# rwth-i6/rasr

Measured on AMD Instinct MI355X. Metric: acoustic frames scored/sec (1e4-state AM), higher is better.
Workload: dtype f16+mxfp6 (per f32 product: one f16 MFMA product + one block-scaled fp6 x fp6 MFMA product for both cross terms, f32 accumulate)

## Files before the change

rasr_amd/csrc/common.hpp:

```cpp
#pragma once
#include <hip/hip_runtime.h>

#include <cstdarg>
#include <cstdio>
#include <map>
#include <memory>
#include <string>
#include <vector>

#include "../../include/amx.h"

namespace amx {

void set_error(const char* fmt, ...);

#define AMX_HIP(expr)                                                                          \
    do {                                                                                       \
        hipError_t e__ = (expr);                                                               \
        if (e__ != hipSuccess) {                                                               \
            amx::set_error("%s failed: %s (%s:%d)", #expr, hipGetErrorString(e__), __FILE__, __LINE__); \
            return AMX_ERR_DEVICE;                                                             \
        }                                                                                      \
    } while (0)

// ... 92 lines not shown
    const char* name;
    hipEvent_t  a = nullptr, b = nullptr;
    ScopedKernelTimer(amx_ctx* c, const char* n)
            : ctx(c), name(n) {
        if (ctx->profiling) {
            hipEventCreate(&a);
            hipEventCreate(&b);
            hipEventRecord(a, ctx->stream);
        }
    }
    ~ScopedKernelTimer() {
        if (a) {
            hipEventRecord(b, ctx->stream);
            ctx->prof[name].events.emplace_back(a, b);
        }
    }
};

template<class Key>
struct GraphCache {
    enum Ran { kPlain, kRecorded, kReplayed };
    std::map<Key, hipGraphExec_t> graphs;
    int                           use_graphs = 0;
    GraphCache() = default;
    GraphCache(const GraphCache&)            = delete;
    GraphCache& operator=(const GraphCache&) = delete;
    ~GraphCache() { clear(); }
    void clear() {
        for (auto& kv : graphs)
            if (kv.second)
                hipGraphExecDestroy(kv.second);
        graphs.clear();
    }
    template<class Pass>
    int run(const Key& key, hipStream_t stream, Pass&& pass, Ran* ran) {
        *ran    = kPlain;
        auto it = graphs.find(key);
        if (it == graphs.end()) {
            if (graphs.size() >= 64) {
                clear();
                use_graphs = 0;
            }
            else
                graphs[key] = nullptr;
            return pass(false);
        }
        hipGraphExec_t ex = it->second;
        if (ex)
            *ran = kReplayed;
        else {
            hipGraph_t g = nullptr;
            if (hipStreamBeginCapture(stream, hipStreamCaptureModeThreadLocal) != hipSuccess) {
                (void)hipGetLastError();
                use_graphs = 0;
                return pass(false);
            }
            const int  r  = pass(true);
            const bool ok = hipStreamEndCapture(stream, &g) == hipSuccess && r == AMX_OK && g != nullptr;
            if (!ok || hipGraphInstantiate(&ex, g, nullptr, nullptr, 0) != hipSuccess) {
                (void)hipGetLastError();
                if (g)
                    hipGraphDestroy(g);
                use_graphs = 0;
                return pass(false);
            }
            hipGraphDestroy(g);
            graphs[key] = ex;
            *ran        = kRecorded;
        }
        AMX_HIP(hipGraphLaunch(ex, stream));
        return AMX_OK;
    }
};

struct Tuning {
    std::map<std::string, std::string> kv;
    bool parse(const char* s, const char* const* allowed, const char* who);
    bool has(const char* key) const { return kv.count(key) != 0; }
    bool get_int(const char* key, int dflt, long lo, long hi, int* out, const char* who) const;
    bool get_word(const char* key, const char* dflt, const char* const* words, std::string* out, const char* who) const;
};

static const char* const gmm_tuning_keys[] = {"screen", "fused", "screen_all", "screen_kernel", "graph", "tied_prune", "chunk", "fused_waves", "fr",
                                              "simd_mfma", "contract", "dist_list", "near_fused", "fused_pack", nullptr};

template<bool FMA>
__host__ __device__ __forceinline__ float mad(float a, float b, float c) {
    return FMA ? __builtin_fmaf(a, b, c) : a * b + c;
}
template<bool FMA>
__host__ __device__ __forceinline__ double mad(double a, double b, double c) {
    return FMA ? __builtin_fma(a, b, c) : a * b + c;
}

template<class V>
__device__ __forceinline__ void nt_store(V v, V* p) {
#ifdef AMX_PLAIN_STORES
    *p = v;
#else
    __builtin_nontemporal_store(v, p);
#endif
}

inline bool views_alias(const float* in, int in_ld, int in_w, const float* out, int out_ld, int out_w, long long T) {
    if (T <= 0)
        return false;
    const float* in_end  = in + (T - 1) * (long long)in_ld + in_w;
    const float* out_end = out + (T - 1) * (long long)out_ld + out_w;
    if (in_end <= out || out_end <= in)
        return false;
    if (in_ld == out_ld) {
        const long long ld = in_ld, delta = out - in;
        const long long c  = ((delta % ld) + ld) % ld;
        if (c >= in_w && c + out_w <= ld)
            return false;
    }
    return true;
}

inline int ceil_div(long a, long b) {
    return (int)((a + b - 1) / b);
}

}
```

rasr_amd/csrc/ffnn.hip:

```cpp
#include "common.hpp"
#include "gmm_internal.hpp"
#include "ffnn_f32.hpp"

#include <hip/hip_bf16.h>

#include <algorithm>
#include <map>
#include <tuple>
#include <type_traits>
#include <cmath>
#include <cstring>

namespace amx {

typedef __attribute__((ext_vector_type(8))) short bf16x8;
typedef unsigned short                              bf16_t;

typedef float  f32x2 __attribute__((ext_vector_type(2)));
typedef float  f32x4 __attribute__((ext_vector_type(4)));
typedef __bf16 bf16x2 __attribute__((ext_vector_type(2)));

__device__ __forceinline__ unsigned pack_bf16(float lo, float hi) {
    f32x2 v = {lo, hi};
    return __builtin_bit_cast(unsigned, __builtin_convertvector(v, bf16x2));
// ... 1086 lines not shown
            const unsigned i = s_idx[w][lane];
            if (m < bmin || (m == bmin && i < bidx)) {
                bmin = m;
                bidx = i;
            }
        }
        if (best_state)
            best_state[t] = bidx;
        if (bidx != 0xffffffffu)
            sum = (double)bmin;
        my = bidx;
    }
    {
        unsigned long long todo = __ballot(my != 0xffffffffu);
        while (todo) {
            const int      leader = __ffsll((long long)todo) - 1;
            const unsigned key    = (unsigned)__shfl((int)my, leader, 64);
            const unsigned long long same = __ballot(my == key) & todo;
            if (lane == leader)
                atomicAdd(&counts[key], (unsigned long long)__popcll(same));
            todo &= ~same;
        }
    }
#pragma unroll
    for (int off = 32; off > 0; off >>= 1)
        sum += __shfl_xor(sum, off, 64);
    if (lane == 0 && sum != 0.0)
        atomicAdd(score_sum, sum);
}

}


struct OverflowWord {
    unsigned *host = nullptr, *dev = nullptr;
    OverflowWord()                               = default;
    OverflowWord(const OverflowWord&)            = delete;
    OverflowWord& operator=(const OverflowWord&) = delete;
    ~OverflowWord() {
        if (host)
            hipHostFree(host);
    }
    int create() {
        if (hipHostMalloc((void**)&host, 4, hipHostMallocMapped) != hipSuccess || hipHostGetDevicePointer((void**)&dev, host, 0) != hipSuccess) {
            (void)hipGetLastError();
            amx::set_error("amx_ffnn_create: cannot allocate the overflow flag");
            return AMX_ERR_DEVICE;
        }
        *host = 0;
        return AMX_OK;
    }
};

struct amx_ffnn {
    amx_ctx*           ctx = nullptr;
    int                n_layers = 0, precision = AMX_PREC_BF16;
    std::vector<int>   in, out, act, Kpad, Npad;
    std::vector<amx::DevBuf<unsigned char>> d_W;
    std::vector<amx::DevBuf<float>> d_bias;
    amx::DevBuf<unsigned char> d_in, d_act[2];
    std::vector<float> h_Wout, h_bout;
    bool   class_mapped = false;
    amx::DevBuf<float> d_rowstat;
    amx::DevBuf<float> d_Wout, d_bout;
    int    max_hidden_pad = 0;
    int    largest_layer  = 0;
    int    group_t = -1, group_n = -1;
    amx::DevBuf<float>    d_part_min;
    amx::DevBuf<unsigned> d_part_idx;
    struct GraphKey {
        const void *feats, *scores, *best, *counts, *sum;
        hipStream_t stream;
        int         stride, T, stats;
        bool operator<(const GraphKey& o) const {
            return std::tie(feats, scores, best, counts, sum, stream, stride, T, stats) <
                   std::tie(o.feats, o.scores, o.best, o.counts, o.sum, o.stream, o.stride, o.T, o.stats);
        }
    };
    amx::GraphCache<GraphKey> graphs;
    amx::DevBuf<float> d_host_f, d_host_s;
    int    gemm_persistent = 1;
    int    gemm_cfg       = -1;
    int    chunk          = 32768;
    int    mx_stagger     = 0;
    int    mx_dbg         = 0;
    int    mx_ksplit      = 1;
    amx::DevBuf<float> d_ks_ws;
    OverflowWord overflow;
    amx::PreOps         pre{};
    std::vector<amx::DevBuf<float>> d_pre;
    std::vector<int>    mo_groups;
    std::vector<amx::DevBuf<int>> d_mo_off, d_mo_size;
    int    mo_width = 0;
    amx::DevBuf<float> d_mo;
    size_t elt() const { return precision == AMX_PREC_FP32 ? 4 : 2; }
    bool   mfma_bf16() const { return precision != AMX_PREC_FP32; }
    bool   is_mx() const { return precision == AMX_PREC_F16MX; }
    int    requested_precision = 0;
    double mx_block_ratio      = 0.0;
#ifdef AMX_LAB
    int    overflowed() const { return mx_dbg == 0 && overflow.host && *(volatile unsigned*)overflow.host; }
#else
    int    overflowed() const { return overflow.host && *(volatile unsigned*)overflow.host; }
#endif
};

namespace {

int pad_to(int v, int m) {
    return (v + m - 1) / m * m;
}

int operand_stride(const amx_ffnn* h, int width) {
    return h->is_mx() ? width / 32 : (h->precision == AMX_PREC_BF16X3 ? 2 : 1) * width;
}

size_t operand_bytes(const amx_ffnn* h, int Tpad, int width) {
    const size_t stride = (size_t)operand_stride(h, width);
    return h->is_mx() ? (size_t)(Tpad / 256) * stride * amx::mx::BLK : (size_t)Tpad * stride * h->elt();
}

template<class T>
int grow(amx_ffnn* h, amx::DevBuf<T>& buf, size_t n) {
    if (n <= buf.capacity())
        return AMX_OK;
    h->graphs.clear();
    return buf.reserve(n);
}

int ensure_workspace(amx_ffnn* h, int Tpad) {
    if (h->mo_width > 0)
        AMX_TRY(grow(h, h->d_mo, (size_t)Tpad * h->mo_width));
    AMX_TRY(grow(h, h->d_in, operand_bytes(h, Tpad, h->Kpad[0])));
    if (h->max_hidden_pad > 0) {
        AMX_TRY(grow(h, h->d_act[0], operand_bytes(h, Tpad, h->max_hidden_pad)));
        AMX_TRY(grow(h, h->d_act[1], operand_bytes(h, Tpad, h->max_hidden_pad)));
    }
    return AMX_OK;
}

void size_split_k_workspace(amx_ffnn* h) {
    if (!h->is_mx() || h->mx_ksplit <= 1)
        return;
    const long ncu  = std::max(h->ctx->n_cu, 8);
    size_t     need = 0;
    for (int Tpad = amx::PAD_NT;; Tpad += amx::PAD_NT) {
        bool fits = false;
        for (int l = 0; l < h->n_layers; ++l) {
            const long tiles = (long)(h->Npad[l] / 128) * (Tpad / 64);
            if (tiles * h->mx_ksplit > ncu)
                continue;
            fits = true;
            if (h->Kpad[l] / 32 >= 8 * h->mx_ksplit)
                need = std::max(need, (size_t)tiles * h->mx_ksplit * 4 * 2 * 16 * 64);
        }
        if (!fits)
            break;
    }
    if (need != 0 && h->d_ks_ws.reserve(need) != AMX_OK) {
        (void)hipGetLastError();
        h->mx_ksplit = 1;
    }
}

struct ArgminPart {
    float*    min = nullptr;
// ... 205 lines not shown
        AMX_MX_LAUNCH(2048);
    }
    else if (dbg == 128 && C::PIPE == 1 && ACT == AMX_ACT_RELU * (LAST ? 0 : 1)) {
        if constexpr (C::PIPE == 1)
            AMX_MX_LAUNCH(128);
    }
    else
        dbg = 0;
#endif
    if (dbg == 0)
        AMX_MX_LAUNCH(0);
#undef AMX_MX_LAUNCH
    return ntn;
}

template<int ACT, bool LAST>
int launch_mx_cfg(amx_ffnn* h, int l, const void* x, int xkts, void* out, int ldo, int T, int Tpad, int n_valid, ArgminPart part) {
    int cfg = h->gemm_cfg;
    if (cfg < 0) {
        const long ncu = std::max(h->ctx->n_cu, 1), t256 = (long)(h->Npad[l] / 256) * (Tpad / 256), t128 = (long)(h->Npad[l] / 128) * (Tpad / 128);
        const long t64 = (long)(h->Npad[l] / 128) * (Tpad / 64);
        if (t256 >= 2L * ncu)
            cfg = 8;
        else if (LAST && t256 <= ncu && 5 * t256 >= 3 * ncu)
            cfg = 8;
        else if (t128 >= ncu)
            cfg = 0;
        else if (t64 > ncu && t64 <= 2 * ncu)
            cfg = 6;
        else if (!LAST && 2 * t64 <= ncu && h->mx_ksplit <= 1)
            cfg = 14;
        else
            cfg = 3;
    }
    switch (cfg) {
        case 2: return launch_mx<MfgL, ACT, LAST>(h, l, x, xkts, out, ldo, T, Tpad, n_valid, part);
        case 4: return launch_mx<MfgLP, ACT, LAST>(h, l, x, xkts, out, ldo, T, Tpad, n_valid, part);
        case 5: return launch_mx<MfgLH, ACT, LAST>(h, l, x, xkts, out, ldo, T, Tpad, n_valid, part);
        case 7: return launch_mx<MfgLF, ACT, LAST>(h, l, x, xkts, out, ldo, T, Tpad, n_valid, part);
        case 8: return launch_mx<MfgLQ, ACT, LAST>(h, l, x, xkts, out, ldo, T, Tpad, n_valid, part);
        case 9: return launch_mx<MfgLW, ACT, LAST>(h, l, x, xkts, out, ldo, T, Tpad, n_valid, part);
        case 3:
            if constexpr (LAST)
                return launch_mx<MfgS, ACT, LAST>(h, l, x, xkts, out, ldo, T, Tpad, n_valid, part);
            else
                return launch_mx<MfgSP, ACT, LAST>(h, l, x, xkts, out, ldo, T, Tpad, n_valid, part);
        case 6: return launch_mx<MfgS4, ACT, LAST>(h, l, x, xkts, out, ldo, T, Tpad, n_valid, part);
        case 12: return launch_mx<MfgS8, ACT, LAST>(h, l, x, xkts, out, ldo, T, Tpad, n_valid, part);
        case 14:
            if constexpr (LAST)
                return launch_mx<MfgS, ACT, LAST>(h, l, x, xkts, out, ldo, T, Tpad, n_valid, part);
            else
                return launch_mx<Mfg64, ACT, LAST>(h, l, x, xkts, out, ldo, T, Tpad, n_valid, part);
case 11:
            if constexpr (LAST)
                return launch_mx<MfgS, ACT, LAST>(h, l, x, xkts, out, ldo, T, Tpad, n_valid, part);
            else
                return launch_mx<MfgSL, ACT, LAST>(h, l, x, xkts, out, ldo, T, Tpad, n_valid, part);
        default: return launch_mx<MfgA, ACT, LAST>(h, l, x, xkts, out, ldo, T, Tpad, n_valid, part);
    }
}

template<bool NONE_ONLY = false, class F>
void with_act(int act, F&& f) {
    using std::integral_constant;
    if constexpr (NONE_ONLY)
        f(integral_constant<int, AMX_ACT_NONE>());
    else
        switch (act) {
            case AMX_ACT_RELU: f(integral_constant<int, AMX_ACT_RELU>()); break;
            case AMX_ACT_SIGMOID: f(integral_constant<int, AMX_ACT_SIGMOID>()); break;
            case AMX_ACT_TANH: f(integral_constant<int, AMX_ACT_TANH>()); break;
            case AMX_ACT_ELU: f(integral_constant<int, AMX_ACT_ELU>()); break;
            default: f(integral_constant<int, AMX_ACT_NONE>()); break;
        }
}

template<class S>
void pack_operand(amx_ffnn* h, const S& src, int T, int K, void* out, int Kp, int Tpad) {
    hipStream_t st     = h->ctx->stream;
    const int   blocks = (int)std::min<long long>(4096, ((long long)Tpad * Kp + 255) / 256);
    if (h->is_mx()) {
        const int b2 = (int)std::min<long long>(8192, ((long long)Tpad * (Kp / 32) * 2 + 255) / 256);
        hipLaunchKernelGGL(amx::mx::pack_input_mx<S>, dim3(b2), dim3(256), 0, st, src, T, K, (char*)out, Kp / 32, Tpad, h->overflow.dev);
    }
    else if (h->precision == AMX_PREC_BF16X3)
        hipLaunchKernelGGL(amx::pack_input_bf16x3<S>, dim3(blocks), dim3(256), 0, st, src, T, K, (amx::bf16_t*)out, Kp, Tpad);
    else if (h->precision == AMX_PREC_BF16)
        hipLaunchKernelGGL(amx::pack_input_bf16<S>, dim3(blocks), dim3(256), 0, st, src, T, K, (amx::bf16_t*)out, Kp, Tpad);
    else
        hipLaunchKernelGGL(amx::pack_input_f32<S>, dim3(blocks), dim3(256), 0, st, src, T, K, (float*)out, Kp, Tpad);
}

template<bool LAST>
int launch_layer(amx_ffnn* h, int l, const void* x, int ldx, void* out, int ldo, int T, int Tpad, ArgminPart part = {}, int* ntn = nullptr) {
    hipStream_t            st = h->ctx->stream;
    amx::ScopedKernelTimer t_all(h->ctx, "ffnn_gemm");
    hipEvent_t             e0 = nullptr, e1 = nullptr;
    const bool             time_max = h->ctx->profiling && l == h->largest_layer;
    if (time_max) {
        hipEventCreate(&e0);
        hipEventCreate(&e1);
        hipEventRecord(e0, st);
    }
    const int act = LAST ? AMX_ACT_NONE : h->act[l];
    int       tiles = 0;
    if (h->is_mx()) {
        with_act<LAST>(act, [&](auto a) { tiles = launch_mx_cfg<decltype(a)::value, LAST>(h, l, x, ldx, out, ldo, T, Tpad, h->out[l], part); });
    }
    else if (h->mfma_bf16()) {
        with_act<LAST>(act, [&](auto a) { tiles = launch_bf16_cfg<decltype(a)::value, LAST>(h, l, x, ldx, out, ldo, T, Tpad, part); });
    }
    else {
        const int ntn = h->Npad[l] / amx::BN, ntt = Tpad / amx::BT;
        dim3      grid(ntn * ntt), block(256);
        const int nv = h->out[l];
        with_act<LAST>(act, [&](auto a) {
            hipLaunchKernelGGL((amx::gemm_f32_kernel<decltype(a)::value, LAST>), grid, block, 0, st, (const float*)h->d_W[l].get(), (const float*)x,
                               h->d_bias[l].get(), (float*)out, h->Kpad[l], ldx, ldo, nv, T, ntn);
        });
    }
    if (time_max) {
        hipEventRecord(e1, st);
        h->ctx->prof["ffnn_gemm_max"].events.emplace_back(e0, e1);
    }
    AMX_HIP(hipGetLastError());
    if (ntn)
        *ntn = tiles;
    return AMX_OK;
}

int launch_maxout_layer(amx_ffnn* h, int l, const void* x, int ldx, void* dst, int Kp, int T, int Trows, int Tpad, bool export_f32) {
    AMX_TRY(launch_layer<true>(h, l, x, ldx, h->d_mo.get(), h->out[l], T, Tpad));
    const int G = h->mo_groups[l];
    amx::ScopedKernelTimer timer(h->ctx, "ffnn_maxout");
    with_act(h->act[l], [&](auto a) {
        const amx::MaxoutSrc<decltype(a)::value> src{h->d_mo.get(), h->out[l], h->d_mo_off[l].get(), h->d_mo_size[l].get()};
        if (export_f32) {
            const int blocks = (int)std::min<long long>(4096, ((long long)Trows * Kp + 255) / 256);
            hipLaunchKernelGGL(amx::pack_input_f32<decltype(src)>, dim3(blocks), dim3(256), 0, h->ctx->stream, src, T, G, (float*)dst, Kp, Trows);
        }
        else
            pack_operand(h, src, T, G, dst, Kp, Trows);
    });
    AMX_HIP(hipGetLastError());
    return AMX_OK;
}


struct MaxoutSpec {
    std::vector<int>              groups;
    std::vector<std::vector<int>> size;
};

int check_extension(const amx_ffnn_model* m, const amx_ffnn_layers* ext, MaxoutSpec* mo) {
    const int n_pre = ext ? ext->n_pre : 0;
    mo->groups.assign((size_t)m->n_layers, 0);
    mo->size.assign((size_t)m->n_layers, {});
    AMX_REQUIRE(n_pre >= 0 && n_pre <= AMX_NN_MAX_PRE, AMX_ERR_INVALID, "amx_ffnn_create_ex: %d preprocessing layers (0 to %d)", n_pre,
                AMX_NN_MAX_PRE);
    AMX_REQUIRE(n_pre == 0 || ext->pre_type, AMX_ERR_INVALID, "amx_ffnn_create_ex: %d preprocessing layers without pre_type", n_pre);
    for (int i = 0; i < n_pre; ++i) {
        const int ty = ext->pre_type[i];
        AMX_REQUIRE(ty == AMX_NN_PRE_LOGARITHM || ty == AMX_NN_PRE_MEAN_AND_VARIANCE, AMX_ERR_INVALID,
                    "amx_ffnn_create_ex: preprocessing layer %d: unknown type %d", i, ty);
        if (ty == AMX_NN_PRE_MEAN_AND_VARIANCE) {
            AMX_REQUIRE(ext->pre_mean && ext->pre_mean[i], AMX_ERR_INVALID,
// ... 20 lines not shown
                }
                AMX_REQUIRE(sum == m->out_dim[l], AMX_ERR_INVALID,
                            "amx_ffnn_create_ex: layer %d: maxout group sizes add up to %ld, the layer has %d outputs "
                            "(require_eq(getInputDimension(0), inputsize_))", l, sum, m->out_dim[l]);
                v.assign(sz, sz + G);
            }
            else {
                AMX_REQUIRE(m->out_dim[l] % G == 0, AMX_ERR_INVALID,
                            "amx_ffnn_create_ex: layer %d: %d outputs do not split into %d maxout groups of one size "
                            "(require_eq(getInputDimension(0), maxoutSize_ * getOutputDimension()))", l, m->out_dim[l], G);
                v.assign((size_t)G, m->out_dim[l] / G);
            }
            mo->groups[l] = G;
        }
    return AMX_OK;
}

int check_model(const amx_ffnn_model* m, const std::vector<int>& mo_groups) {
    for (int l = 0; l < m->n_layers; ++l) {
        AMX_REQUIRE(m->in_dim[l] > 0 && m->out_dim[l] > 0 && m->W[l], AMX_ERR_INVALID, "amx_ffnn_create: layer %d is empty", l);
        if (l > 0 && mo_groups[l - 1] > 0)
            AMX_REQUIRE(m->in_dim[l] == mo_groups[l - 1], AMX_ERR_INVALID,
                        "amx_ffnn_create_ex: layer %d input dimension %d != %d outputs of the maxout behind layer %d", l, m->in_dim[l],
                        mo_groups[l - 1], l - 1);
        else if (l > 0)
            AMX_REQUIRE(m->in_dim[l] == m->out_dim[l - 1], AMX_ERR_INVALID,
                        "amx_ffnn_create: layer %d input dimension %d != previous output %d", l, m->in_dim[l], m->out_dim[l - 1]);
        AMX_REQUIRE(m->activation[l] >= AMX_ACT_NONE && m->activation[l] <= AMX_ACT_ELU, AMX_ERR_INVALID,
                    "amx_ffnn_create: unknown activation in layer %d", l);
    }
    AMX_REQUIRE(m->activation[m->n_layers - 1] == AMX_ACT_NONE, AMX_ERR_INVALID, "amx_ffnn_create: output layer must be linear (softmax is not evaluated)");
    return AMX_OK;
}

struct LayerParams {
    std::vector<int>          out_dim;
    std::vector<const float*> W, bias;
    const float*              prior = nullptr;
    std::vector<float>        Wmap, bmap, pmap;
};

int remap_classes(const amx_ffnn_model* m, LayerParams* p) {
    const int L0 = m->n_layers - 1;
    p->out_dim.assign(m->out_dim, m->out_dim + m->n_layers);
    p->W.assign(m->W, m->W + m->n_layers);
    p->bias.assign(m->bias, m->bias + m->n_layers);
    p->prior = m->log_prior;
    if (!m->class_to_output)
        return AMX_OK;
    AMX_REQUIRE(m->n_classes > 0, AMX_ERR_INVALID, "amx_ffnn_create: class_to_output without n_classes");
    const int N = m->out_dim[L0], K = m->in_dim[L0];
    std::vector<char> used((size_t)N, 0);
    int               n_targets = 0;
    for (int e = 0; e < m->n_classes; ++e) {
        const int o = m->class_to_output[e];
        AMX_REQUIRE(o >= -1 && o < N, AMX_ERR_INVALID, "amx_ffnn_create: class %d maps to output %d (network has %d outputs)", e, o, N);
        if (o >= 0) {
            AMX_REQUIRE(!used[o], AMX_ERR_INVALID, "amx_ffnn_create: no one-to-one correspondence between network outputs and classes (output %d)", o);
            used[o] = 1;
            ++n_targets;
        }
    }
    AMX_REQUIRE(n_targets == N, AMX_ERR_INVALID, "amx_ffnn_create: %d classes to accumulate, but the output layer has %d units", n_targets, N);
    p->Wmap.assign((size_t)m->n_classes * K, 0.f);
    p->bmap.assign((size_t)m->n_classes, -3.402823466e+38f);
    p->pmap.assign((size_t)m->n_classes, 0.f);
    for (int e = 0; e < m->n_classes; ++e) {
        const int o = m->class_to_output[e];
        if (o < 0)
            continue;
        memcpy(&p->Wmap[(size_t)e * K], m->W[L0] + (size_t)o * K, (size_t)K * 4);
        p->bmap[e] = m->bias[L0] ? m->bias[L0][o] : 0.f;
        p->pmap[e] = m->log_prior ? m->log_prior[o] : 0.f;
    }
    p->out_dim[L0] = m->n_classes;
    p->W[L0]       = p->Wmap.data();
    p->bias[L0]    = p->bmap.data();
    if (m->log_prior)
        p->prior = p->pmap.data();
    return AMX_OK;
}

int parse_tuning(const amx_ffnn_model* m, amx_ffnn* h, bool* mx_fallback_auto) {
    static const char* const keys[]      = {"tile", "graph", "persistent", "group", "chunk", "stagger", "mx_dbg", "mx_fallback", "ksplit", nullptr};
    static const char* const fallbacks[] = {"auto", "off", nullptr};
    const char*              who         = "amx_ffnn_create";
    amx::Tuning              tune;
    std::string              fallback;
    if (!tune.parse(m->tuning, keys, who) || !tune.get_word("mx_fallback", "auto", fallbacks, &fallback, who) ||
        !tune.get_int("ksplit", 1, 1, 4, &h->mx_ksplit, who))
        return AMX_ERR_INVALID;
    *mx_fallback_auto = fallback == "auto";
    AMX_REQUIRE(h->mx_ksplit == 1 || h->mx_ksplit == 4, AMX_ERR_INVALID, "amx_ffnn_create: tuning ksplit=%d: expected 1 | 4", h->mx_ksplit);
    AMX_REQUIRE(h->mx_ksplit == 1 || m->precision == AMX_PREC_F16MX, AMX_ERR_UNSUPPORTED, "amx_ffnn_create: tuning ksplit exists for AMX_PREC_F16MX only");
    if (!tune.get_int("tile", -1, -1, 14, &h->gemm_cfg, who) || !tune.get_int("graph", 0, 0, 1, &h->graphs.use_graphs, who) ||
        !tune.get_int("persistent", 1, 0, 1, &h->gemm_persistent, who) || !tune.get_int("chunk", 32768, 256, 1 << 24, &h->chunk, who) ||
        !tune.get_int("mx_dbg", 0, 0, 1 << 16, &h->mx_dbg, who) || !tune.get_int("stagger", 0, 0, 100000, &h->mx_stagger, who))
        return AMX_ERR_INVALID;
    if (tune.has("group")) {
        const std::string g    = tune.kv["group"];
        char              tail = 0;
        AMX_REQUIRE(sscanf(g.c_str(), "%dx%d%c", &h->group_t, &h->group_n, &tail) == 2 && h->group_t >= 1 && h->group_n >= 1 && h->group_t <= 4096 &&
                            h->group_n <= 4096,
                    AMX_ERR_INVALID, "amx_ffnn_create: tuning group=%s: expected <frame tiles>x<output tiles>, e.g. 16x8", g.c_str());
    }
    return AMX_OK;
}

double block_max_ratio(const float* W, int N, int K) {
    double sum_max2 = 0.0, sum_w2 = 0.0;
    long   n_blocks = 0;
    for (int n = 0; n < N; ++n)
        for (int k0 = 0; k0 < K; k0 += 32) {
            float mx = 0.f;
            for (int k = k0; k < std::min(K, k0 + 32); ++k) {
                const float v = W[(size_t)n * K + k];
                mx            = std::fmax(mx, std::fabs(v));
                sum_w2 += (double)v * (double)v;
            }
            sum_max2 += (double)mx * (double)mx;
            ++n_blocks;
        }
    return sum_w2 > 0.0 ? std::sqrt((sum_max2 / (double)n_blocks) / (sum_w2 / ((double)N * (double)K))) : 0.0;
}

int choose_precision(const amx_ffnn_model* m, const LayerParams& p, bool mx_fallback_auto, amx_ffnn* h) {
    h->precision = h->requested_precision = m->precision;
    if (m->precision != AMX_PREC_F16MX)
        return AMX_OK;
    for (int l = 0; l < m->n_layers; ++l)
        h->mx_block_ratio = std::max(h->mx_block_ratio, block_max_ratio(p.W[l], p.out_dim[l], m->in_dim[l]));
    if (mx_fallback_auto && h->mx_block_ratio > 4.0) {
        AMX_REQUIRE(h->mx_ksplit <= 1, AMX_ERR_INVALID,
                    "amx_ffnn_create: tuning ksplit=%d applies to AMX_PREC_F16MX, but this network's weights are heavy-tailed (block-maximum "
                    "statistic %.2f > 4.0) and the handle would compute in AMX_PREC_BF16X3: drop ksplit, or keep f16mx with mx_fallback=off",
                    h->mx_ksplit, h->mx_block_ratio);
        std::fprintf(stderr, "rasr_amd: amx_ffnn_create: AMX_PREC_F16MX requested, computing in AMX_PREC_BF16X3 (block-maximum statistic of the "
                             "weights %.2f > 4.0; tuning mx_fallback=off keeps f16mx)\n", h->mx_block_ratio);
        h->precision = AMX_PREC_BF16X3;
    }
    return AMX_OK;
}

void set_shapes(amx_ffnn* h, const amx_ffnn_model* m, const LayerParams& p, const MaxoutSpec& mo) {
    const int kmult = h->is_mx() ? amx::mx::TK : h->mfma_bf16() ? amx::BK : amx::FK;
    long      best_flops = -1;
    h->n_layers  = m->n_layers;
    h->mo_groups = mo.groups;
    for (int l = 0; l < m->n_layers; ++l) {
        h->in.push_back(m->in_dim[l]);
        h->out.push_back(p.out_dim[l]);
        h->act.push_back(m->activation[l]);
        if (mo.groups[l] > 0)
            h->mo_width = std::max(h->mo_width, p.out_dim[l]);
        h->Kpad.push_back(pad_to(m->in_dim[l], kmult));
        h->Npad.push_back(pad_to(p.out_dim[l], amx::PAD_NT));
        if (l + 1 < m->n_layers)
            h->max_hidden_pad = std::max(h->max_hidden_pad, h->Npad[l]);
        long fl = (long)m->in_dim[l] * p.out_dim[l];
        if (fl > best_flops) {
            best_flops       = fl;
            h->largest_layer = l;
        }
    }
}

std::vector<unsigned char> pack_weights(int precision, const float* W, int N, int K, int Np, int Kp) {
    std::vector<unsigned char> pk;
    if (precision == AMX_PREC_F16MX) {
        amx::mx::pack_weights_host(W, N, K, K, Np, Kp / 32, pk);
        return pk;
    }
    if (precision == AMX_PREC_FP32) {
        pk.assign((size_t)Np * Kp * 4, 0);
        for (int n = 0; n < N; ++n)
            memcpy(&pk[(size_t)n * Kp * 4], W + (size_t)n * K, (size_t)K * 4);
        return pk;
    }
    const bool   x3 = precision == AMX_PREC_BF16X3;
    const size_t ld = x3 ? 2 * (size_t)Kp : (size_t)Kp;
// ... 422 lines not shown
```

rasr_amd/csrc/ffnn_f32.hpp:

```cpp
#pragma once
#include "common.hpp"

#include <cmath>

namespace amx {

typedef __attribute__((ext_vector_type(16))) float f32x16;

template<int ACT>
__device__ __forceinline__ float activate(float v) {
    if (ACT == AMX_ACT_RELU)
        return v < 0.f ? 0.f : v;
    if (ACT == AMX_ACT_SIGMOID)
        return 1.f / (1.f + expf(-v));
    if (ACT == AMX_ACT_TANH)
        return tanhf(v);
    if (ACT == AMX_ACT_ELU)
        return v < 0.f ? expf(v) - 1.f : v;
    return v;
}

struct PreOps {
    int          n;
    int          type[AMX_NN_MAX_PRE];
    const float* mean[AMX_NN_MAX_PRE];
    const float* rstd[AMX_NN_MAX_PRE];
};

struct RawSrc {
    const float* x;
    int          ldx;
    __device__ __forceinline__ float operator()(int t, int k) const { return x[(size_t)t * ldx + k]; }
};

struct FeatSrc {
    const float* x;
    int          ldx;
    PreOps       pre;
    __device__ __forceinline__ float operator()(int t, int k) const {
        float v = x[(size_t)t * ldx + k];
#pragma unroll
        for (int i = 0; i < AMX_NN_MAX_PRE; ++i) {
            if (i >= pre.n)
                break;
            if (pre.type[i] == AMX_NN_PRE_LOGARITHM)
                v = (float)log((double)v);
            else {
                v = v - pre.mean[i][k];
                v = v * pre.rstd[i][k];
            }
        }
        return v;
    }
};

static __global__ __launch_bounds__(256) void top_negexp_kernel(float* __restrict__ x, int n, float* __restrict__ g_max) {
    __shared__ float s_red[4];
    float*           row = x + (size_t)blockIdx.x * n;
    float            mx  = -__builtin_inff();
    for (int i = threadIdx.x; i < n; i += 256)
        mx = fmaxf(mx, -row[i]);
#pragma unroll
    for (int off = 32; off > 0; off >>= 1)
        mx = fmaxf(mx, __shfl_xor(mx, off, 64));
    if ((threadIdx.x & 63) == 0)
        s_red[threadIdx.x >> 6] = mx;
    __syncthreads();
    mx = fmaxf(fmaxf(s_red[0], s_red[1]), fmaxf(s_red[2], s_red[3]));
    const float value = -1.f * mx;
    for (int i = threadIdx.x; i < n; i += 256) {
        const float a = -row[i];
        row[i]        = (float)exp((double)(a + value));
    }
    if (threadIdx.x == 0)
        g_max[blockIdx.x] = mx;
}

static __global__ __launch_bounds__(64) void top_rowsum_kernel(const float* __restrict__ x, int T, int n, float* __restrict__ g_sum) {
    __shared__ float s_tile[64][65];
    const int        lane = threadIdx.x, t0 = blockIdx.x * 64;
    float            acc = 0.f;
    for (int c0 = 0; c0 < n; c0 += 64) {
        const int w = min(64, n - c0);
        for (int r = 0; r < 64; ++r)
            s_tile[r][lane] = (t0 + r < T && lane < w) ? x[(size_t)(t0 + r) * n + c0 + lane] : 0.f;
        __syncthreads();
        for (int c = 0; c < w; ++c)
            acc = acc + s_tile[lane][c];
        __syncthreads();
    }
    if (t0 + lane < T)
        g_sum[t0 + lane] = acc;
}

static __global__ __launch_bounds__(256) void top_finish_kernel(float* __restrict__ x, long long total, int n, const float* __restrict__ g_sum) {
    for (long long i = (long long)blockIdx.x * 256 + threadIdx.x; i < total; i += (long long)gridDim.x * 256) {
        if (g_sum) {
            const float r = 1.f / g_sum[i / n];
            x[i]          = x[i] * r;
        }
        else
            x[i] = -x[i];
    }
}

template<class S>
__global__ __launch_bounds__(256) void pack_input_f32(S src, int T, int K, float* __restrict__ out, int Kpad, int Tpad) {
    const long long n = (long long)Tpad * Kpad;
    for (long long i = (long long)blockIdx.x * 256 + threadIdx.x; i < n; i += (long long)gridDim.x * 256) {
        int t = (int)(i / Kpad), k = (int)(i - (long long)t * Kpad);
        out[i] = (t < T && k < K) ? src(t, k) : 0.f;
    }
}

constexpr int BN = 128, BT = 128;
constexpr int FK  = 32;
constexpr int FLD = FK + 1;

template<int ACT, bool LAST>
__global__ __launch_bounds__(256) void gemm_f32_kernel(const float* __restrict__ W, const float* __restrict__ X,
                                                      const float* __restrict__ bias, float* __restrict__ out, int Kpad, int ldx, int ldo,
                                                      int n_valid, int t_valid, int n_tiles_n) {
    __shared__ float sW[BN * FLD];
    __shared__ float sX[BT * FLD];
    const int tid = threadIdx.x, lane = tid & 63, wave = tid >> 6;
    const int wn = wave >> 1, wt = wave & 1;
    const int tile_t = blockIdx.x / n_tiles_n, tile_n = blockIdx.x - tile_t * n_tiles_n;
    const int n0 = tile_n * BN, t0 = tile_t * BT;

    f32x16 acc[2][2];
#pragma unroll
    for (int i = 0; i < 2; ++i)
#pragma unroll
        for (int j = 0; j < 2; ++j)
#pragma unroll
            for (int r = 0; r < 16; ++r)
// ... 57 lines not shown
```

rasr_amd/csrc/ffnn_mx.hpp:

```cpp
#pragma once

namespace amx {
namespace mx {

typedef _Float16 f16x8 __attribute__((ext_vector_type(8)));
typedef unsigned u32x4 __attribute__((ext_vector_type(4)));
typedef unsigned u32x2 __attribute__((ext_vector_type(2)));
typedef _Float16 f16x2 __attribute__((ext_vector_type(2)));
typedef _Float16 f16x16 __attribute__((ext_vector_type(16)));
typedef _Float16 f16x32 __attribute__((ext_vector_type(32)));
typedef float    f32v16 __attribute__((ext_vector_type(16)));
typedef unsigned u32x6 __attribute__((ext_vector_type(6)));
typedef int      v8i __attribute__((ext_vector_type(8)));

constexpr int TK    = 32;
constexpr int R_OFF = 16384;
constexpr int BLK   = 24576;

__host__ __device__ constexpr int pos16(int u) {
    return 8 * (2 * (u >> 4) + ((u >> 2) & 1)) + 4 * ((u >> 3) & 1) + (u & 3);
}
__host__ __device__ inline int h_off(int r, int c) {
    return r * 64 + ((c ^ ((r >> 2) & 3)) << 4);
}
// ... 28 lines not shown
            code = (unsigned)(qv / 0.125);
    }
    return code | (std::signbit(v) ? 32u : 0u);
}

static inline void pack_weights_host(const float* W, int n_rows, int K, int ld, int Rpad, int KT, std::vector<unsigned char>& out) {
    out.assign((size_t)(Rpad / 256) * KT * BLK, 0);
    auto block_max = [&](int n, int kt) {
        float m = 0.f;
        if (n < n_rows)
            for (int u = 0; u < 32; ++u) {
                const int k = kt * 32 + u;
                if (k < K)
                    m = std::fmax(m, std::fabs(W[(size_t)n * ld + k]));
            }
        return m;
    };
    for (int n = 0; n < n_rows; ++n) {
        const int rb = n >> 8, r = n & 255;
        for (int kt = 0; kt < KT; ++kt) {
            unsigned char* blk = out.data() + ((size_t)rb * KT + kt) * BLK;
            float          v[32], lo[32];
            _Float16       hi[32];
            for (int u = 0; u < 32; ++u) {
                const int k = kt * 32 + u;
                v[u]        = k < K ? W[(size_t)n * ld + k] : 0.f;
                hi[u]       = (_Float16)v[u];
                lo[u]       = v[u] - (float)hi[u];
            }
            const int ec = block_exponent(std::fmax(block_max(n, kt), block_max(n ^ 32, kt)));
            unsigned  rec[2][4] = {{0, 0, 0, (unsigned)(ec - 2)}, {0, 0, 0, (unsigned)(ec - 2)}};
            for (int u = 0; u < 32; ++u) {
                const int p = pos16(u), chunk = p >> 3, half = chunk & 1, f = 8 * (chunk >> 1) + (p & 7);
                memcpy(blk + h_off(r, chunk) + (p & 7) * 2, &hi[u], 2);
                const unsigned code = fp6_code_host(lo[u], ec - 13);
                const int      bit = 6 * f, d = bit >> 5, sh = bit & 31;
                rec[half][d] |= code << sh;
                if (sh > 26)
                    rec[half][d + 1] |= code >> (32 - sh);
            }
            memcpy(blk + r_off(r, 0), rec[0], 16);
            memcpy(blk + r_off(r, 1), rec[1], 16);
        }
    }
}

struct LanePack {
    uint4 h0, h1, rec;
};

__device__ __forceinline__ unsigned pk_f16(float a, float b) {
    f16x2 v = {(_Float16)a, (_Float16)b};
    return __builtin_bit_cast(unsigned, v);
}

__device__ __forceinline__ LanePack lane_pack(const float (&a)[16], int ec, int sbyte) {
    LanePack o;
    unsigned h[8];
    f32v16   le, lod;
#pragma unroll
    for (int p = 0; p < 8; ++p) {
        h[p]           = pk_f16(a[2 * p], a[2 * p + 1]);
        const f16x2 hv = __builtin_bit_cast(f16x2, h[p]);
        le[p]          = a[2 * p] - (float)hv[0];
        lod[p]         = a[2 * p + 1] - (float)hv[1];
        le[8 + p]      = 0.f;
        lod[8 + p]     = 0.f;
    }
    o.h0 = make_uint4(h[0], h[1], h[2], h[3]);
    o.h1 = make_uint4(h[4], h[5], h[6], h[7]);
    u32x6       r;
    const float scale = __uint_as_float((unsigned)(ec - 13) << 23);
    asm("v_cvt_scalef32_2xpk16_fp6_f32 %0, %1, %2, %3\n\ts_nop 2" : "=&v"(r) : "v"(le), "v"(lod), "v"(scale));
    o.rec = make_uint4(r[0], r[1], r[2], (unsigned)sbyte);
    return o;
}

__device__ __forceinline__ void lane_store(char* blk, int r, int hh, const LanePack& p) {
    *(uint4*)(blk + h_off(r, hh))     = p.h0;
    *(uint4*)(blk + h_off(r, 2 + hh)) = p.h1;
    *(uint4*)(blk + r_off(r, hh))     = p.rec;
}

template<class S>
__global__ __launch_bounds__(256) void pack_input_mx(S src, int T, int K, char* __restrict__ out, int KT, int Tpad, unsigned* __restrict__ overflow) {
    const long long n = (long long)Tpad * KT * 2;
    for (long long i = (long long)blockIdx.x * 256 + threadIdx.x; i < n; i += (long long)gridDim.x * 256) {
        const int       hh = (int)(i & 1);
        const long long j  = i >> 1;
        const int       kt = (int)(j % KT), t = (int)(j / KT);
        float           a[16], m = 0.f;
#pragma unroll
        for (int g = 0; g < 4; ++g)
#pragma unroll
            for (int e = 0; e < 4; ++e) {
                const int   k = kt * 32 + 8 * g + 4 * hh + e;
                const float v = (t < T && k < K) ? src(t, k) : 0.f;
                a[4 * g + e]  = v;
                m             = (v != v) ? __builtin_inff() : fmaxf(m, fabsf(v));
            }
        m = fmaxf(m, __shfl_xor(m, 1, 64));
        if (!(m < 65520.f))
            *overflow = 1u;
        const int ec = block_exponent(m);
        lane_store(out + ((size_t)(t >> 8) * KT + kt) * BLK, t & 255, hh, lane_pack(a, ec, ec - 13));
    }
}

template<int ACT>
__global__ __launch_bounds__(256) void neg_act_kernel(float* __restrict__ x, long long n) {
    for (long long i = (long long)blockIdx.x * 256 + threadIdx.x; i < n; i += (long long)gridDim.x * 256)
        x[i] = activate<ACT>(-x[i]);
}

template<int BN_, int BT_, int WN_, int WT_, int STAGES_, int PF_ = 0, int IW_ = 0, int U_ = 1, int LW_ = 0, int PIPE_ = 0>
struct MxCfg {
    static constexpr int BN = BN_, BT = BT_, WN = WN_, WT = WT_, STAGES = STAGES_;
    static constexpr int PIPE = PIPE_;
    static_assert(PIPE_ == 0 || (PIPE_ == 1 && U_ == 1 && LW_ == 0 && PF_ == 0 && IW_ == 0 && STAGES_ == 3 && WN_ * WT_ == 8) ||
                      (PIPE_ == 2 && U_ == 1 && LW_ == 0 && PF_ == 0 && IW_ == 0 && STAGES_ == 3 && WN_ * WT_ == 4 && BN_ / WN_ == 128 && BT_ / WT_ == 128) ||
                      (PIPE_ == 3 && U_ == 2 && LW_ > 0 && STAGES_ >= 2 * U_ + 1),
                  "ping-pong K loop: eight waves, every one of them issuing, plain three-stage ring; self-pipelined: four waves of 128 x 128; "
                  "read-ahead: loader waves, two K-tiles per barrier, a ring of at least three iterations");
    static constexpr int PF = PF_;
    static constexpr int U = U_;
    static_assert(U_ >= 1 && U_ <= 4 && STAGES_ >= 2 * U_, "ring: U K-tiles being read + at least U in flight");
    static_assert(PF_ == 0 || (BN_ == 256 && BT_ == 256 && WN_ * WT_ == 8), "the prefetch walks whole 256-row blocks with six waves");
    static constexpr int NW = WN * WT, LW = LW_, THREADS = (NW + LW_) * 64, PLANES = 1;
    static_assert(LW_ == 0 || (IW_ == 0 && PF_ == 0), "loader waves replace the issuing-wave variants");
    static constexpr bool SKEW = false, SPREAD = false;
    static constexpr int MI = BN / WN / 32, MJ = BT / WT / 32;
    static constexpr int A_R = BN * 64, A_BYTES = BN * 96;
    static constexpr int B_R = BT * 64, B_BYTES = BT * 96;
    static constexpr int STAGE_BYTES = A_BYTES + B_BYTES, LDS_BYTES = STAGES * STAGE_BYTES;
    static constexpr int A_PIECES = BN / 16 + BN / 32, B_PIECES = BT / 16 + BT / 32;
    static constexpr int TOTAL = A_PIECES + B_PIECES;
    static constexpr int IW  = LW_ > 0 ? LW_ : IW_ > 0 ? IW_ : NW;
    static constexpr int PPW = (TOTAL + IW - 1) / IW;
    static constexpr int NHI = TOTAL % IW;
    static constexpr bool PF_FREE = PF_ > 0 && IW_ > 0;
    static_assert(PF_ == 0 || IW_ == 0 || IW_ * 2 == WN_ * WT_, "free prefetch: half of the waves issue the DMA");
    static_assert(BN % 64 == 0 && BT % 64 == 0 && 256 % BN == 0 && 256 % BT == 0, "tiles are whole record pieces of a 256-row block");
    static_assert(STAGES >= 2 && STAGES <= 8 && (STAGES - 2) * (PPW + (PF_ > 0 ? 1 : 0)) + 1 < 64, "vmcnt immediate");
};

template<class C>
__device__ __forceinline__ void piece_offsets(int p, int ha, int hb, int& src, int& dst, bool& is_b) {
    is_b = p >= C::A_PIECES;
    if (!is_b) {
        if (p < C::BN / 16) {
            src = (ha * (C::BN / 16) + p) * 1024;
            dst = p * 1024;
        }
        else {
            const int j = p - C::BN / 16, half = j / (C::BN / 64), gq = j % (C::BN / 64);
            src = R_OFF + half * 4096 + (ha * (C::BN / 64) + gq) * 1024;
            dst = C::A_R + half * (C::BN * 16) + gq * 1024;
        }
    }
    else {
        const int q = p - C::A_PIECES;
        if (q < C::BT / 16) {
            src = (hb * (C::BT / 16) + q) * 1024;
            dst = C::A_BYTES + q * 1024;
        }
        else {
            const int j = q - C::BT / 16, half = j / (C::BT / 64), gq = j % (C::BT / 64);
            src = R_OFF + half * 4096 + (hb * (C::BT / 64) + gq) * 1024;
            dst = C::A_BYTES + C::B_R + half * (C::BT * 16) + gq * 1024;
        }
    }
}

#ifdef AMX_LAB
__device__ unsigned long long mx_stamps[8 * 48 * 4];
__device__ unsigned long long mx_tile_stamps[4 * 3 * 2];
#endif

__device__ __forceinline__ void keep_alive(const v8i& v) { asm volatile("" ::"v"(v)); }
__device__ __forceinline__ void keep_alive(const f16x8& v) { asm volatile("" ::"v"(v)); }
__device__ __forceinline__ void keep_alive(unsigned v) { asm volatile("" ::"v"(v)); }

template<int N>
// ... 857 lines not shown
```

rasr_amd/csrc/gmm.hip:

```cpp
#include "common.hpp"
#include "gmm_internal.hpp"
#include "gmm_device.hpp"

#include <cfloat>
#include <cmath>
#include <cstring>

namespace amx {

struct GmmParams {
    const float* __restrict__ feats;
    float* __restrict__ scores;
    uint32_t* __restrict__ best;
    const uint32_t* __restrict__ mix_off;
    const uint32_t* __restrict__ k_mean;
    const uint32_t* __restrict__ k_cov;
    const double* __restrict__ k_c64;
    const float* __restrict__ k_c32;
    const float* __restrict__ means;
    const float* __restrict__ isr;
    int T, dim, n_mix, mix_tile;
};

template<int DIM, bool FMA = false>
// ... 149 lines not shown
            p.scores[(size_t)t * p.n_mix + m] = st.result();
            if (p.best)
                p.best[(size_t)t * p.n_mix + m] = st.idx;
        }
    }
}

template<int DIM, bool FMA = false>
__global__ __launch_bounds__(256) void gmm_batch_float_kernel(const float* __restrict__ g_feats, float* __restrict__ g_scores,
                                                             const uint32_t* __restrict__ g_mix_off, const uint32_t* __restrict__ g_k_mean,
                                                             const float* __restrict__ g_k_const, const float* __restrict__ g_smeans,
                                                             const float* __restrict__ g_isr0, GmmDims dims) {
    const int  lane = threadIdx.x & 63;
    const int  wave = threadIdx.x >> 6;
    const int  t    = (blockIdx.y * 4 + wave) * 64 + lane;
    const bool live = t < dims.T;
    const int  tt   = live ? t : (dims.T - 1);
    const int  dim = DIM > 0 ? DIM : dims.dim;
    ScaledRow<DIM> x;
    x.load(g_feats + (size_t)tt * dim, g_isr0, dim);
    const int m0 = blockIdx.x * dims.mix_tile;
    const int m1 = min(m0 + dims.mix_tile, dims.n_mix);
    for (int m = m0; m < m1; ++m) {
        const uint32_t k0 = g_mix_off[m], k1 = g_mix_off[m + 1];
        float          best = FLT_MAX;
        for (uint32_t k = k0; k < k1; ++k) {
            const float* mu = g_smeans + (size_t)g_k_mean[k] * dim;
            const float  r  = batch_float_distance<DIM, FMA>(mu, x, g_k_const[k], dim);
            best           = best < r ? best : r;
        }
        if (live)
            g_scores[(size_t)t * dims.n_mix + m] = best < FLT_MAX ? 0.5f * best : best;
    }
}

template<bool FMA>
__global__ __launch_bounds__(256) void gmm_best_density_kernel(const float* __restrict__ feats, const uint32_t* __restrict__ mixture,
                                                              uint32_t* __restrict__ best, float* __restrict__ score, const uint32_t* __restrict__ mix_off,
                                                              const uint32_t* __restrict__ k_mean, const uint32_t* __restrict__ k_cov,
                                                              const double* __restrict__ k_c64, const float* __restrict__ means,
                                                              const float* __restrict__ isr, int T, int dim, int n_mix) {
    const int t = blockIdx.x * 256 + threadIdx.x;
    if (t >= T)
        return;
    const uint32_t m = mixture[t];
    MaxState       st;
    if (m < (uint32_t)n_mix) {
        const float*   x  = feats + (size_t)t * dim;
        const uint32_t k0 = mix_off[m], k1 = mix_off[m + 1];
        const int      eff = dim & ~3;
        for (uint32_t k = k0; k < k1; ++k) {
            const float* mu = means + (size_t)k_mean[k] * dim;
            const float* is = isr + (size_t)k_cov[k] * dim;
            float        l0 = 0.f, l1 = 0.f, l2 = 0.f, l3 = 0.f;
            for (int i = 0; i < eff; i += 4) {
                const float d0 = (mu[i] - x[i]) * is[i];
                const float d1 = (mu[i + 1] - x[i + 1]) * is[i + 1];
                const float d2 = (mu[i + 2] - x[i + 2]) * is[i + 2];
                const float d3 = (mu[i + 3] - x[i + 3]) * is[i + 3];
                l0             = sq_acc<FMA>(d0, l0);
                l1             = sq_acc<FMA>(d1, l1);
                l2             = sq_acc<FMA>(d2, l2);
                l3             = sq_acc<FMA>(d3, l3);
            }
            float dist = 0.f;
            dist       = dist + ((l0 + l1) + (l2 + l3));
            for (int i = eff; i < dim; ++i) {
                const float df = (mu[i] - x[i]) * is[i];
                dist           = sq_acc<FMA>(df, dist);
            }
            st.add(k_c64[k], 0.f, dist, k - k0);
        }
    }
    best[t] = st.idx;
    if (score)
        score[t] = st.result();
}

__global__ __launch_bounds__(256) void best_narrow_kernel(const uint32_t* __restrict__ in, unsigned char* __restrict__ out, size_t n) {
    for (size_t i = (size_t)blockIdx.x * 256 + threadIdx.x; i < n; i += (size_t)gridDim.x * 256)
        out[i] = (unsigned char)min(in[i], 255u);
}

__global__ __launch_bounds__(256) void gmm_accumulate_kernel(const float* __restrict__ feats, const uint32_t* __restrict__ mixture,
                                                            const uint32_t* __restrict__ best, const unsigned char* __restrict__ best8,
                                                            int best_ld, int T, int dim, int n_mix,
                                                            const uint32_t* __restrict__ mix_off, const uint32_t* __restrict__ k_dens,
                                                            const uint32_t* __restrict__ d_mean, const uint32_t* __restrict__ d_cov,
                                                            double* __restrict__ acc, long long off_mw, long long off_ms,
                                                            long long off_cw, long long off_cs, int pooled) {
    __shared__ uint32_t s_k[256], s_mi[256], s_ci[256];
    __shared__ short    s_next[256];
    __shared__ unsigned char s_lead[256];
    const int tid = threadIdx.x, lane = tid & 63, wave = tid >> 6;
    const int t0 = blockIdx.x * 256;
    {
        const int t = t0 + tid;
        uint32_t  k = 0xffffffffu, mi = 0, ci = 0;
        if (t < T && mixture[t] < (uint32_t)n_mix) {
            const uint32_t m  = mixture[t];
            uint32_t       kk;
            if (best8) {
                const unsigned char b = best_ld > 0 ? best8[(size_t)t * best_ld + m] : best8[t];
                kk                    = b == 0xffu ? 0xffffffffu : (uint32_t)b;
            }
            else
                kk = best_ld > 0 ? best[(size_t)t * best_ld + m] : best[t];
            if (kk < mix_off[m + 1] - mix_off[m]) {
                k                = mix_off[m] + kk;
                const uint32_t d = k_dens[k];
                mi               = d_mean[d];
                ci               = d_cov[d];
            }
        }
        s_k[tid]  = k;
        s_mi[tid] = mi;
        s_ci[tid] = ci;
    }
    __syncthreads();
    {
        const uint32_t k = s_k[tid];
        bool lead = k != 0xffffffffu;
        for (int j = 0; j < tid && lead; ++j)
            lead = s_k[j] != k;
        int next = -1;
        if (k != 0xffffffffu)
            for (int j = tid + 1; j < 256; ++j)
                if (s_k[j] == k) {
                    next = j;
                    break;
                }
        s_lead[tid] = lead ? 1 : 0;
        s_next[tid] = (short)next;
    }
    __syncthreads();
    double pc[4] = {0, 0, 0, 0};
    double pcw   = 0;
    for (int j = wave; j < 256; j += 4) {
        if (!s_lead[j])
            continue;
        const uint32_t k = s_k[j], mi = s_mi[j], ci = s_ci[j];
        double         sx[4] = {0, 0, 0, 0}, sxx[4] = {0, 0, 0, 0};
        int            count = 0;
        for (int m = j; m >= 0; m = s_next[m]) {
            ++count;
            for (int i = lane, c = 0; i < dim && c < 4; i += 64, ++c) {
                const double y = (double)feats[(size_t)(t0 + m) * dim + i];
                sx[c] += y;
                sxx[c] += y * y;
            }
            for (int i = lane + 256; i < dim; i += 64) {
                const double y = (double)feats[(size_t)(t0 + m) * dim + i];
                atomicAdd(&acc[off_ms + (long long)mi * dim + i], y);
                atomicAdd(&acc[off_cs + (pooled ? 0 : (long long)ci * dim) + i], y * y);
            }
        }
        if (lane == 0) {
            atomicAdd(&acc[k], (double)count);
            atomicAdd(&acc[off_mw + mi], (double)count);
            if (!pooled)
                atomicAdd(&acc[off_cw + ci], (double)count);
        }
        pcw += (double)count;
        for (int i = lane, c = 0; i < dim && c < 4; i += 64, ++c) {
            atomicAdd(&acc[off_ms + (long long)mi * dim + i], sx[c]);
            if (pooled)
                pc[c] += sxx[c];
            else
                atomicAdd(&acc[off_cs + (long long)ci * dim + i], sxx[c]);
        }
    }
    if (pooled) {
        for (int i = lane, c = 0; i < dim && c < 4; i += 64, ++c)
            if (pc[c] != 0.0)
                atomicAdd(&acc[off_cs + i], pc[c]);
        if (lane == 0 && pcw != 0.0)
            atomicAdd(&acc[off_cw], pcw);
    }
}

constexpr int kBwMaxDens   = 4096;
constexpr int kBwFramesPerWave = 16;

template<bool FMA>
__global__ __launch_bounds__(256) void gmm_accumulate_weighted_kernel(
        int mode, const float* __restrict__ feats, const uint32_t* __restrict__ mixture, const double* __restrict__ weight,
        const uint32_t* __restrict__ best, int best_ld, int T, int dim, int n_mix, const uint32_t* __restrict__ mix_off,
        const uint32_t* __restrict__ k_dens, const uint32_t* __restrict__ d_mean, const uint32_t* __restrict__ d_cov,
        const float* __restrict__ k_c32, const float* __restrict__ means, const float* __restrict__ isr, double* __restrict__ acc,
        long long off_mw, long long off_ms, long long off_cw, long long off_cs, int pooled) {
    __shared__ float s_p[4][kBwMaxDens];
    const int lane = threadIdx.x & 63, wave = threadIdx.x >> 6;
    float*    sp   = s_p[wave];
    double    pc[4] = {0, 0, 0, 0};
    double    pcw   = 0;
    const int t_begin = (blockIdx.x * 4 + wave) * kBwFramesPerWave;
    for (int t = t_begin; t < min(t_begin + kBwFramesPerWave, T); ++t) {
        const uint32_t m  = mixture[t];
        if (m >= (uint32_t)n_mix)
            continue;
        const uint32_t k0 = mix_off[m], nd = mix_off[m + 1] - k0;
        const float*   x  = feats + (size_t)t * dim;
        const double   w  = weight ? weight[t] : 1.0;
        uint32_t       j_lo = 0, j_hi = nd;
        if (mode == 1) {
            float lmin = FLT_MAX;
            for (uint32_t j = lane; j < nd; j += 64) {
                const uint32_t d  = k_dens[k0 + j];
                const float*   mu = means + (size_t)d_mean[d] * dim;
                const float*   is = isr + (size_t)d_cov[d] * dim;
                float          l0 = 0.f, l1 = 0.f, l2 = 0.f, l3 = 0.f;
                const int      eff = dim & ~3;
                for (int i = 0; i < eff; i += 4) {
                    const float d0 = (mu[i] - x[i]) * is[i], d1 = (mu[i + 1] - x[i + 1]) * is[i + 1];
                    const float d2 = (mu[i + 2] - x[i + 2]) * is[i + 2], d3 = (mu[i + 3] - x[i + 3]) * is[i + 3];
                    l0 = sq_acc<FMA>(d0, l0);
                    l1 = sq_acc<FMA>(d1, l1);
                    l2 = sq_acc<FMA>(d2, l2);
                    l3 = sq_acc<FMA>(d3, l3);
                }
                float dist = 0.f;
                dist       = dist + ((l0 + l1) + (l2 + l3));
                for (int i = eff; i < dim; ++i) {
                    const float df = (mu[i] - x[i]) * is[i];
                    dist           = sq_acc<FMA>(df, dist);
                }
                const float sk = 0.5f * (k_c32[k0 + j] + dist);
                sp[j]          = sk;
                lmin           = fminf(lmin, sk);
            }
// ... 996 lines not shown
        if constexpr (State::kTwoPass)
            for (uint32_t k = k0; k < k1; ++k)
                st.add2(p.k_c32[k], p.dist[(size_t)p.k_dens[k] * p.Tpad + tt]);
        if (live) {
            p.scores[(size_t)t * p.n_mix + m] = st.result();
            if (p.best)
                p.best[(size_t)t * p.n_mix + m] = st.idx;
        }
    }
}

}


struct GraphKey {
    const void *feats, *scores, *best;
    hipStream_t stream;
    int         T;
    bool operator<(const GraphKey& o) const {
        return std::tie(feats, scores, best, stream, T) < std::tie(o.feats, o.scores, o.best, o.stream, o.T);
    }
};

using GraphCache = amx::GraphCache<GraphKey>;

struct amx_gmm {
    amx_ctx* ctx = nullptr;
    int      dim = 0, n_mix = 0, n_dens = 0, n_mean = 0, n_cov = 0;
    size_t   nk = 0;
    std::vector<float>    m2lw, isr, lognorm;
    std::vector<uint32_t> mix_off, h_k_dens, h_d_mean, h_d_cov;
    amx::DevBuf<uint32_t> d_mix_off, d_k_mean, d_k_cov, d_k_dens;
    amx::DevBuf<float>    d_means_t, d_isr_t;
    amx::DevBuf<uint32_t> d_dens_pos;
    amx::DevBuf<uint32_t> d_d_mean, d_d_cov;
    amx::DevBuf<double>   d_k_c64;
    amx::DevBuf<float>    d_k_c32, d_means, d_isr;
    amx::DevBuf<float>    d_smeans, d_k_const, d_isr0;
    bool      pooled = false;
    bool      tied    = false;
    bool      uniform = false;
    int       K = 0, mix_pad = 0;
    amx::DevBuf<float>    d_m2lw_t;
    amx::DevBuf<float>    d_ahat_t, d_amax;
    amx::DevBuf<float>              d_amin;
    amx::DevBuf<unsigned short>     d_aup;
    amx::DevBuf<char>               d_tied_ws;
    amx::DevBuf<unsigned long long> d_tied_surv;
    amx::DevBuf<unsigned long long, true> h_tied_surv;
    unsigned            tied_copy_tick = 0;
    bool                tied_capturing = false;
    bool                tied_keys_clean = false;
    unsigned long long  tied_seen    = 0;
    unsigned long long  tied_triples = 0;
    int                 tied_dense_calls = 0;
    unsigned long long  tied_rep_seen = 0, tied_rep_triples = 0;
    amx::DevBuf<double> d_ln64, d_dist64;
    amx::DevBuf<float>  d_ln32;
    amx::DevBuf<float>  d_dist;
    bool      screen = false;
    int       scr_Kp = 0, scr_Rpad = 0, scr_Mpad16 = 0;
    float     scr_rmax2 = 0.f, scr_na_all = 0.f;
    amx::DevBuf<_Float16> d_scr_A;
    amx::DevBuf<_Float16> d_scr_A2;
    amx::DevBuf<float>    d_scr_c, d_scr_na, d_scr_cabs;
    amx::DevBuf<_Float16> d_scr_X;
    amx::DevBuf<float>    d_scr_nx, d_scr_q;
    amx::DevBuf<uint16_t> d_scr_masks;
    int       scr_cap_T = 0;
    amx::DevBuf<float>    d_host_f, d_host_s;
    amx::DevBuf<uint32_t> d_host_b;
    void*     simd = nullptr;
    std::vector<float>  h_means, h_vars;
    std::vector<double> h_logw;
    double    mws = 1.0, gsc = 1.0;
    int       simd_status = 0;
    void*     presel = nullptr;
    int       presel_clusters = 256, presel_select = 32, presel_iterations = 5;
    float     presel_backoff = 40000.f;
    std::vector<uint32_t> h_k_mean;
    std::vector<float>    h_smeans;
    GraphCache graphs;
    int         tune_screen = 1, tune_fused = 1, tune_screen_all = 0, tune_tied_prune = -1, tune_chunk = 65536, tune_fused_waves = 0, tune_fr = 8,
                tune_simd_mfma = 1, tune_dist_list = 1, tune_near_fused = 1, tune_fused_pack = 1;
    std::string tune_screen_kernel = "rows";
    bool        contract_fma = false;
    amx::DevBuf<char>     d_fus_rec;
    amx::DevBuf<uint32_t> d_best32;
    amx::DevBuf<unsigned long long> d_fus_surv;
    bool      count_survivors = false;
    unsigned long long fus_pairs = 0;
    amx::DevBuf<float>    d_scr_pmin;
    amx::DevBuf<unsigned> d_scr_pidx;
};

namespace {

template<class F>
auto with_dim(int dim, F&& f) {
    switch (dim) {
#define X(D) \
    case D: return f(std::integral_constant<int, D>{});
        AMX_GMM_DIMS(X)
#undef X
        default: return f(std::integral_constant<int, 0>{});
    }
}
template<class F>
auto with_flag(bool flag, F&& f) {
    return flag ? f(std::true_type{}) : f(std::false_type{});
}

bool screen_dim_supported(int dim) {
    return with_dim(dim, [](auto d) { return d.value != 0; });
}

int score_screened(amx_gmm* h, const float* feats_dev, int T, float* scores_dev, uint32_t* best_dev, bool stats, uint32_t* best_state_dev,
                   unsigned long long* counts_dev, double* score_sum_dev, int best_bytes = 4) {
    hipStream_t st = h->ctx->stream;
    const int   chunk = h->tune_chunk;
    const bool fused = h->d_fus_rec.get() && h->tune_fused && !h->tune_screen_all;
    AMX_REQUIRE(best_bytes == 4 || (best_bytes == 1 && fused), AMX_ERR_STATE, "score_screened: byte-sized best densities exist on the fused path only");
    for (int t0 = 0; t0 < T; t0 += chunk) {
        const int Tc = std::min(chunk, T - t0), Tpad = (Tc + 255) / 256 * 256;
        if (Tpad > h->scr_cap_T || (!fused && !h->d_scr_masks.get())) {
            h->graphs.clear();
            h->d_scr_X.release();
            h->d_scr_nx.release();
            h->d_scr_q.release();
            h->d_scr_masks.release();
            h->scr_cap_T = 0;
            AMX_TRY(h->d_scr_X.reserve((size_t)Tpad * h->scr_Kp));
            AMX_TRY(h->d_scr_nx.reserve((size_t)Tpad));
            AMX_TRY(h->d_scr_q.reserve((size_t)Tpad));
            if (!fused)
                AMX_TRY(h->d_scr_masks.reserve((size_t)Tpad * h->scr_Mpad16));
            h->scr_cap_T = Tpad;
        }
        const float*       x = feats_dev + (size_t)t0 * h->dim;
        amx::GmmScreenDims d{Tc, Tpad, h->dim, h->scr_Kp, h->scr_Mpad16, h->pooled ? 1 : 0, h->scr_rmax2,
                             std::sqrt((float)(h->pooled ? h->dim : 2 * h->dim)), h->scr_na_all};
        const bool own_pack = fused && h->tune_fused_pack && h->tune_fused_waves != 13;
        if (!own_pack) {
            amx::ScopedKernelTimer timer(h->ctx, "gmm_screen_pack");
            hipLaunchKernelGGL(amx::gmm_screen_pack_kernel, dim3(Tpad / 4), dim3(256), 0, st, x, h->d_isr.get(), h->d_scr_X.get(), h->d_scr_nx.get(), h->d_scr_q.get(), d);
        }
        if (fused) {
            const int n_tiles = h->scr_Rpad / 256;
            const int split   = amx_internal_gmm_fused_split(h->ctx->n_cu, Tpad, n_tiles, h->tune_fused_waves);
            float*    pmin    = nullptr;
            unsigned* pidx    = nullptr;
            if (stats) {
                const size_t need = (size_t)split * Tpad;
                AMX_TRY(h->d_scr_pmin.reserve(need));
                AMX_TRY(h->d_scr_pidx.reserve(need));
                pmin = h->d_scr_pmin.get();
                pidx = h->d_scr_pidx.get();
            }
            {
                amx::ScopedKernelTimer timer(h->ctx, "gmm");
                int r = amx_internal_gmm_fused_score(h->ctx, h->dim, h->d_fus_rec.get(), h->d_isr.get(), x, own_pack ? nullptr : h->d_scr_X.get(), h->d_scr_nx.get(), h->d_scr_q.get(), Tc, Tpad,
                                                     h->n_mix, n_tiles, split, scores_dev + (size_t)t0 * h->n_mix,
                                                     best_dev ? (uint32_t*)((char*)best_dev + (size_t)t0 * h->n_mix * best_bytes) : nullptr, pmin,
                                                     pidx, Tpad, h->count_survivors ? h->d_fus_surv.get() : nullptr, h->tune_fused_waves, best_bytes,
                                                     h->contract_fma ? 1 : 0, h->scr_na_all);
                if (r != AMX_OK)
                    return r;
                if (h->count_survivors)
                    h->fus_pairs += (unsigned long long)Tc * (unsigned long long)h->n_mix;
            }
            if (stats) {
                amx::ScopedKernelTimer timer(h->ctx, "stats");
                int r = amx_internal_best_state_reduce(h->ctx, pmin, pidx, split, Tpad, Tc, best_state_dev ? best_state_dev + t0 : nullptr,
                                                       counts_dev, score_sum_dev);
                if (r != AMX_OK)
                    return r;
            }
            continue;
        }
        {
            amx::ScopedKernelTimer timer(h->ctx, "gmm_screen");
            const int ntr = h->scr_Rpad / 256, ntt = Tpad / 256;
            const char* variant = h->tune_screen_kernel.c_str();
            if (h->scr_Kp == 64 && !strcmp(variant, "rows")) {
                auto      k   = amx::gmm_screen_rows_kernel;
                const int lds = 2 * 32 * 1024;
                hipFuncSetAttribute((const void*)k, hipFuncAttributeMaxDynamicSharedMemorySize, lds);
                const int split = std::max(1, std::min(ntr, (2 * std::max(h->ctx->n_cu, 8) + ntt - 1) / ntt));
                hipLaunchKernelGGL(k, dim3(ntt * split), dim3(512), lds, st, h->d_scr_A2.get(), h->d_scr_X.get(), h->d_scr_na.get(), h->d_scr_cabs.get(), h->d_scr_nx.get(),
                                   h->d_scr_q.get(), h->d_scr_masks.get(), ntr, split, h->scr_Mpad16);
            }
            else if (h->scr_Kp == 64 && strcmp(variant, "simple")) {
                auto      k   = amx::gmm_screen_persist_kernel;
                const int lds = 3 * 32 * 1024 + 2048;
                hipFuncSetAttribute((const void*)k, hipFuncAttributeMaxDynamicSharedMemorySize, lds);
                const int split = std::max(1, std::min(ntr, (std::max(h->ctx->n_cu, 8) + ntt - 1) / ntt));
                hipLaunchKernelGGL(k, dim3(ntt * split), dim3(512), lds, st, h->d_scr_A.get(), h->d_scr_X.get(), h->d_scr_c.get(), h->d_scr_na.get(), h->d_scr_cabs.get(),
                                   h->d_scr_nx.get(), h->d_scr_q.get(), h->d_scr_masks.get(), ntr, split, d);
            }
            else if (h->scr_Kp == 64) {
                auto k = amx::gmm_screen_kernel<1>;
                hipFuncSetAttribute((const void*)k, hipFuncAttributeMaxDynamicSharedMemorySize, 64 * 1024 + 1024);
                hipLaunchKernelGGL(k, dim3(ntr * ntt), dim3(512), 64 * 1024 + 1024, st, h->d_scr_A.get(), h->d_scr_X.get(), h->d_scr_c.get(), h->d_scr_na.get(),
                                   h->d_scr_cabs.get(), h->d_scr_nx.get(), h->d_scr_q.get(), h->d_scr_masks.get(), ntr, d);
            }
            else {
                auto k = amx::gmm_screen_kernel<2>;
                hipFuncSetAttribute((const void*)k, hipFuncAttributeMaxDynamicSharedMemorySize, 128 * 1024 + 1024);
                hipLaunchKernelGGL(k, dim3(ntr * ntt), dim3(512), 128 * 1024 + 1024, st, h->d_scr_A.get(), h->d_scr_X.get(), h->d_scr_c.get(), h->d_scr_na.get(),
                                   h->d_scr_cabs.get(), h->d_scr_nx.get(), h->d_scr_q.get(), h->d_scr_masks.get(), ntr, d);
            }
        }
        if (h->tune_screen_all)
            hipMemsetAsync(h->d_scr_masks.get(), 0xff, (size_t)Tpad * h->scr_Mpad16 * 2, st);
        float*    pmin = nullptr;
        unsigned* pidx = nullptr;
        if (stats) {
            const size_t need = (size_t)(h->scr_Mpad16 / 16) * Tpad;
            AMX_TRY(h->d_scr_pmin.reserve(need));
            AMX_TRY(h->d_scr_pidx.reserve(need));
            pmin = h->d_scr_pmin.get();
            pidx = h->d_scr_pidx.get();
        }
        {
            amx::ScopedKernelTimer timer(h->ctx, "gmm");
            const int FG = std::max(1, std::min(32, (int)((long)(Tpad / 256) * (h->scr_Mpad16 / 16) / 2500)));
            dim3      grid(h->scr_Mpad16 / 16, (Tpad / 256 + FG - 1) / FG);
            float*    sc = scores_dev + (size_t)t0 * h->n_mix;
            uint32_t* bd = best_dev ? best_dev + (size_t)t0 * h->n_mix : nullptr;
            with_dim(h->dim, [&](auto dc) {
                constexpr int D = decltype(dc)::value;
                if constexpr (D != 0) {
                    const size_t lds = (size_t)256 * amx::gmm_exact_ld(D, h->pooled) * 4 * (h->pooled ? 1 : 2) + 2048 + 2112 + 256 * 17 * 4 + 256 * 20 + 256 * amx::gmm_list_cap(D, h->pooled);
                    with_flag(h->pooled, [&](auto pc) {
                        with_flag(h->contract_fma, [&](auto fc) {
                            auto k = amx::gmm_screen_exact_kernel<D, decltype(pc)::value, decltype(fc)::value>;
                            hipFuncSetAttribute((const void*)k, hipFuncAttributeMaxDynamicSharedMemorySize, (int)lds);
                            hipLaunchKernelGGL(k, grid, dim3(256), lds, st, x, h->d_scr_masks.get(), h->d_mix_off.get(), h->d_k_mean.get(), h->d_k_cov.get(),
                                               h->d_k_c64.get(), h->d_means.get(), h->d_isr.get(), sc, bd, Tc, h->n_mix, h->scr_Mpad16, pmin, pidx, Tpad, FG);
                        });
                    });
                }
            });
        }
        AMX_HIP(hipGetLastError());
// ... 28 lines not shown
    with_dim(h->dim, [&](auto dc) {
        constexpr int D = decltype(dc)::value;
        auto launch = [&](auto k, size_t lds) {
            hipLaunchKernelGGL(k, grid, dim3(256), lds, h->ctx->stream, p.feats, p.dist, dist64, p.d_mean, p.d_cov, p.means, p.isr, dims, dt,
                               (const uint32_t*)h->d_dens_pos.get(), dt_ld);
        };
        if constexpr (D != 0) {
            if (stage)
                return with_flag(h->contract_fma, [&](auto fc) { launch(amx::gmm_dist_kernel<D, true, decltype(fc)::value>, (size_t)256 * (D + 1) * sizeof(float)); });
        }
        with_flag(h->contract_fma, [&](auto fc) { launch(amx::gmm_dist_kernel<D, false, decltype(fc)::value>, D ? 0 : (size_t)4 * 64 * h->dim * sizeof(float)); });
    });
    AMX_HIP(hipGetLastError());
    return AMX_OK;
}

int launch_dist_list(amx_gmm* h, const float* feats, int T, float* dt, unsigned long long* near) {
    const int Kpad = (h->K + 63) & ~63;
    int frames = 16;
    while (frames > 2 && (long)amx::ceil_div(Kpad, 256) * 4 * amx::ceil_div(T, frames) < 8L * std::max(h->ctx->n_cu, 1))
        frames /= 2;
    if (h->tune_dist_list > 1)
        frames = h->tune_dist_list;
    const dim3 grid(amx::ceil_div(Kpad, 256), amx::ceil_div(T, frames));
    const int r = with_dim(h->dim, [&](auto dc) {
        constexpr int D = decltype(dc)::value;
        if constexpr (D == 0 || D == 64)
            return (int)AMX_ERR_STATE;
        else {
            with_flag(near != nullptr, [&](auto nc) {
                with_flag(h->contract_fma, [&](auto fc) {
                    hipLaunchKernelGGL((amx::gmm_dist_list_kernel<D, decltype(fc)::value, decltype(nc)::value>), grid, dim3(256), 0, h->ctx->stream, feats,
                                       h->d_means_t.get(), h->d_isr_t.get(), h->K, Kpad, T, frames, dt, near);
                });
            });
            return (int)AMX_OK;
        }
    });
    if (r != AMX_OK)
        return r;
    AMX_HIP(hipGetLastError());
    return AMX_OK;
}

struct HostTables {
    std::vector<uint32_t> k_mean, k_cov, k_dens;
    std::vector<double>   c64;
    std::vector<float>    c32;
};

int check_model(const amx_gmm_model* m) {
    AMX_REQUIRE(m->dim > 0 && m->n_mix > 0 && m->n_dens > 0 && m->n_mean > 0 && m->n_cov > 0, AMX_ERR_INVALID,
                "amx_gmm_create: empty mixture set");
    AMX_REQUIRE(m->dim <= 1024, AMX_ERR_UNSUPPORTED, "amx_gmm_create: feature dimension %d > 1024", m->dim);
    AMX_REQUIRE(m->mix_offsets && m->dens_index && m->log_weight && m->dens_mean && m->dens_cov && m->means && m->variances,
                AMX_ERR_INVALID, "amx_gmm_create: NULL table");
    const size_t nk = m->mix_offsets[m->n_mix];
    for (int i = 0; i < m->n_mix; ++i)
        AMX_REQUIRE(m->mix_offsets[i] <= m->mix_offsets[i + 1], AMX_ERR_INVALID, "amx_gmm_create: mix_offsets not monotone");
    for (size_t k = 0; k < nk; ++k)
        AMX_REQUIRE(m->dens_index[k] < (uint32_t)m->n_dens, AMX_ERR_INVALID, "amx_gmm_create: density index out of range");
    for (int d = 0; d < m->n_dens; ++d)
        AMX_REQUIRE(m->dens_mean[d] < (uint32_t)m->n_mean && m->dens_cov[d] < (uint32_t)m->n_cov, AMX_ERR_INVALID,
                    "amx_gmm_create: mean/covariance index out of range");
    for (size_t i = 0; i < (size_t)m->n_cov * m->dim; ++i)
        AMX_REQUIRE(m->variances[i] > 0, AMX_ERR_INVALID, "amx_gmm_create: non-positive variance");
    return AMX_OK;
}

int parse_tuning(amx_gmm* h, const amx_ctx* ctx, const char* tuning) {
    amx::Tuning tune;
    const char* who = "amx_gmm_create";
    if (!tune.parse(tuning, amx::gmm_tuning_keys, who))
        return AMX_ERR_INVALID;
    static const char* const screen_kernels[] = {"rows", "persist", "simple", nullptr};
    static const char* const contracts[]      = {"off", "fma", nullptr};
    std::string              contract;
    if (!tune.get_int("screen", 1, 0, 1, &h->tune_screen, who) || !tune.get_int("fused", 1, 0, 1, &h->tune_fused, who) ||
        !tune.get_int("screen_all", 0, 0, 1, &h->tune_screen_all, who) || !tune.get_int("tied_prune", -1, -1, 1, &h->tune_tied_prune, who) ||
        !tune.get_int("chunk", 65536, 256, 1 << 24, &h->tune_chunk, who) || !tune.get_int("fused_waves", 0, 0, 16, &h->tune_fused_waves, who) ||
        !tune.get_int("fr", 8, 2, 16, &h->tune_fr, who) || !tune.get_int("simd_mfma", 1, 0, 1, &h->tune_simd_mfma, who) ||
        !tune.get_int("graph", 0, 0, 1, &h->graphs.use_graphs, who) || !tune.get_int("dist_list", 1, 0, 64, &h->tune_dist_list, who) ||
        !tune.get_int("near_fused", 1, 0, 1, &h->tune_near_fused, who) || !tune.get_int("fused_pack", 1, 0, 1, &h->tune_fused_pack, who) ||
        !tune.get_word("screen_kernel", "rows", screen_kernels, &h->tune_screen_kernel, who) ||
        !tune.get_word("contract", ctx && ctx->contract == AMX_CONTRACT_FMA ? "fma" : "off", contracts, &contract, who))
        return AMX_ERR_INVALID;
    h->contract_fma = contract == "fma";
    AMX_REQUIRE(h->tune_fused_waves == 0 || h->tune_fused_waves == 8 || h->tune_fused_waves == 12 || h->tune_fused_waves == 13 || h->tune_fused_waves == 16,
                AMX_ERR_INVALID, "amx_gmm_create: tuning fused_waves=%d: expected 8 | 12 | 13 | 16", h->tune_fused_waves);
    AMX_REQUIRE(h->tune_fr == 2 || h->tune_fr == 4 || h->tune_fr == 8 || h->tune_fr == 16, AMX_ERR_INVALID,
                "amx_gmm_create: tuning fr=%d: expected 2 | 4 | 8 | 16", h->tune_fr);
    AMX_REQUIRE(!(h->contract_fma && h->tune_fused_waves == 13), AMX_ERR_UNSUPPORTED,
                "amx_gmm_create: tuning contract=fma has no fused_waves=13 kernel (the specialised-wave form exists for contract=off only)");
    return AMX_OK;
}

int upload_pooled_tables(amx_gmm* h, const amx_gmm_model* m, const HostTables& t) {
    const size_t nk = h->nk;
    int          r;
    std::vector<float> isr0(m->dim), smeans((size_t)m->n_mean * m->dim), kc(nk);
    double             lsum = 0;
    for (int i = 0; i < m->dim; ++i) {
        isr0[i] = (float)1 / (float)std::sqrt((double)m->variances[i]);
        lsum += std::log((double)std::fabs(m->variances[i]));
    }
    const float ln = (float)(h->contract_fma ? std::fma((double)m->dim, std::log((double)2 * M_PI), lsum) : (double)m->dim * std::log((double)2 * M_PI) + lsum);
    for (int j = 0; j < m->n_mean; ++j)
        for (int i = 0; i < m->dim; ++i)
            smeans[(size_t)j * m->dim + i] = m->means[(size_t)j * m->dim + i] * isr0[i];
    for (size_t k = 0; k < nk; ++k)
        kc[k] = (float)((double)ln - 2 * m->log_weight[k]);
    h->h_smeans = smeans;
    h->h_k_mean = t.k_mean;
    if ((r = h->d_isr0.upload(isr0.data(), isr0.size())) != AMX_OK || (r = h->d_smeans.upload(smeans.data(), smeans.size())) != AMX_OK ||
        (r = h->d_k_const.upload(kc.data(), kc.size())) != AMX_OK)
        return r;
    return AMX_OK;
}

int upload_tied_tables(amx_gmm* h, const amx_gmm_model* m, const HostTables& t) {
    const auto &k_mean = t.k_mean, &k_cov = t.k_cov, &k_dens = t.k_dens;
    int r;
    h->mix_pad = (h->n_mix + 63) & ~63;
    std::vector<float>  wt((size_t)h->K * h->mix_pad, 0.f);
    std::vector<double> ln64(h->K);
    std::vector<float>  ln32(h->K);
    for (int i = 0; i < h->n_mix; ++i)
        for (int k = 0; k < h->K; ++k)
            wt[(size_t)k * h->mix_pad + i] = h->m2lw[(size_t)i * h->K + k];
    for (int k = 0; k < h->K; ++k) {
        ln32[k] = h->lognorm[k_cov[k]];
        ln64[k] = (double)ln32[k];
    }
    {
        std::vector<uint32_t> pos((size_t)h->n_dens, 0xffffffffu);
        bool                  once = true;
        for (int k = 0; k < h->K && once; ++k) {
            once = k_dens[k] < (uint32_t)h->n_dens && pos[k_dens[k]] == 0xffffffffu;
            if (once)
                pos[k_dens[k]] = (uint32_t)k;
        }
        if (once && (r = h->d_dens_pos.upload(pos.data(), pos.size())) != AMX_OK)
            return r;
        if (once) {
            const int          Kpad = (h->K + 63) & ~63, dim = m->dim;
            std::vector<float> mt((size_t)dim * Kpad, 0.f), it((size_t)dim * Kpad, 0.f);
            for (int k = 0; k < h->K; ++k)
                for (int i = 0; i < dim; ++i) {
                    mt[(size_t)i * Kpad + k] = m->means[(size_t)k_mean[k] * dim + i];
                    it[(size_t)i * Kpad + k] = h->isr[(size_t)k_cov[k] * dim + i];
                }
            if ((r = h->d_means_t.upload(mt.data(), mt.size())) != AMX_OK || (r = h->d_isr_t.upload(it.data(), it.size())) != AMX_OK)
                return r;
        }
    }
    std::vector<float> ahat((size_t)h->K * h->mix_pad, 0.f), amax(h->mix_pad, 0.f);
    for (int k = 0; k < h->K; ++k)
        for (int i = 0; i < h->n_mix; ++i) {
            const float a                    = wt[(size_t)k * h->mix_pad + i] + ln32[k];
            ahat[(size_t)k * h->mix_pad + i] = a;
            amax[i]                          = std::max(amax[i], std::fabs(a));
        }
    if ((r = h->d_m2lw_t.upload(wt.data(), wt.size())) != AMX_OK || (r = h->d_ln64.upload(ln64.data(), ln64.size())) != AMX_OK ||
        (r = h->d_ln32.upload(ln32.data(), ln32.size())) != AMX_OK || (r = h->d_ahat_t.upload(ahat.data(), ahat.size())) != AMX_OK ||
        (r = h->d_amax.upload(amax.data(), amax.size())) != AMX_OK ||
        (r = amx_internal_gmm_tied_create(h->K, h->n_mix, h->mix_pad, ahat.data(), h->d_amin, h->d_aup)) != AMX_OK)
        return r;
    if (h->d_tied_surv.reserve(257) != AMX_OK || hipMemset(h->d_tied_surv.get(), 0, 257 * 8) != hipSuccess || h->h_tied_surv.reserve(257) != AMX_OK) {
        amx::set_error("amx_gmm_create: out of memory (tied-model statistics)");
        return AMX_ERR_DEVICE;
// ... 757 lines not shown
    ok = (fclose(f) == 0) && ok;
    AMX_REQUIRE(ok, AMX_ERR_INVALID, "amx_gmm_accumulator_write: write to '%s' failed", path);
    return AMX_OK;
}

int amx_gmm_accumulator_read(const amx_gmm* h, const char* path, double* acc) {
    AMX_REQUIRE(h && acc && path, AMX_ERR_INVALID, "amx_gmm_accumulator_read: NULL argument");
    FILE* f = fopen(path, "rb");
    AMX_REQUIRE(f, AMX_ERR_INVALID, "amx_gmm_accumulator_read: cannot open '%s'", path);
    const AccLayout l = acc_layout(h);
    char            magic[8] = {0};
    uint32_t        version = 0, dim = 0, n = 0;
    const char*     why = nullptr;
    bool            ok = fread(magic, 1, 8, f) == 8 && get(f, &version) && get(f, &dim);
    if (ok && strncmp(magic, "MIXSET", 7) != 0)
        why = "not a MIXSET estimator file";
    else if (ok && version == 0)
        why = "version 0 files (integer counts) are not supported";
    else if (ok && (int)dim != h->dim)
        why = "dimension differs from the model";
    auto vec = [&](double* sums, double* weight) {
        uint32_t size = 0;
        return get(f, &size) && (int)size == h->dim && fread(sums, 8, (size_t)h->dim, f) == (size_t)h->dim && get(f, weight);
    };
    ok = ok && !why && get(f, &n) && (int)n == h->n_mean;
    for (int i = 0; ok && i < h->n_mean; ++i)
        ok = vec(acc + l.off_ms + (long long)i * h->dim, acc + l.off_mw + i);
    ok = ok && get(f, &n) && (int)n == h->n_cov;
    for (int i = 0; ok && i < h->n_cov; ++i)
        ok = vec(acc + l.off_cs + (long long)i * h->dim, acc + l.off_cw + i);
    ok = ok && get(f, &n) && (int)n == h->n_dens;
    for (int d = 0; ok && d < h->n_dens; ++d) {
        uint32_t mi = 0, ci = 0;
        ok          = get(f, &mi) && get(f, &ci) && mi == h->h_d_mean[d] && ci == h->h_d_cov[d];
    }
    ok = ok && get(f, &n) && (int)n == h->n_mix;
    for (int m = 0; ok && m < h->n_mix; ++m) {
        ok = get(f, &n) && n == h->mix_off[m + 1] - h->mix_off[m];
        for (uint32_t k = h->mix_off[m]; ok && k < h->mix_off[m + 1]; ++k) {
            uint32_t d = 0;
            ok         = get(f, &d) && d == h->h_k_dens[k] && get(f, &acc[k]);
        }
    }
    fclose(f);
    if (why) {
        amx::set_error("amx_gmm_accumulator_read: '%s': %s", path, why);
        return AMX_ERR_INVALID;
    }
    AMX_REQUIRE(ok, AMX_ERR_INVALID, "amx_gmm_accumulator_read: '%s' is truncated or its topology differs from the model", path);
    return AMX_OK;
}

int amx_gmm_best_density_dev(amx_gmm* h, const float* feats_dev, int T, const uint32_t* mixture_dev, uint32_t* best_density_dev,
                             float* scores_dev) {
    AMX_REQUIRE(h, AMX_ERR_INVALID, "amx_gmm_best_density_dev: NULL handle");
    AMX_REQUIRE(h->ctx, AMX_ERR_STATE, "amx_gmm_best_density_dev: host-only handle (created without a context)");
    AMX_REQUIRE(T >= 0, AMX_ERR_INVALID, "amx_gmm_best_density_dev: negative frame count");
    AMX_REQUIRE(h->d_k_mean.get() && h->d_k_cov.get() && h->d_k_c64.get() && h->d_means.get() && h->d_isr.get(), AMX_ERR_UNSUPPORTED,
                "amx_gmm_best_density_dev: the model's scorer keeps no diagonal-maximum tables on the device");
    if (T == 0)
        return AMX_OK;
    AMX_REQUIRE(feats_dev && mixture_dev && best_density_dev, AMX_ERR_INVALID, "amx_gmm_best_density_dev: NULL buffer");
    AMX_HIP(hipSetDevice(h->ctx->device));
    amx::ScopedKernelTimer timer(h->ctx, "gmm_best_density");
    hipLaunchKernelGGL((h->contract_fma ? amx::gmm_best_density_kernel<true> : amx::gmm_best_density_kernel<false>), dim3((T + 255) / 256), dim3(256), 0, h->ctx->stream, feats_dev, mixture_dev, best_density_dev,
                       scores_dev, h->d_mix_off.get(), h->d_k_mean.get(), h->d_k_cov.get(), h->d_k_c64.get(), h->d_means.get(), h->d_isr.get(), T, h->dim, h->n_mix);
    AMX_HIP(hipGetLastError());
    return AMX_OK;
}

int amx_gmm_accumulate_dev(amx_gmm* h, const float* feats_dev, int T, const uint32_t* mixture_dev, const uint32_t* best_density_dev,
                           int best_density_ld, double* acc_dev) {
    AMX_REQUIRE(h, AMX_ERR_INVALID, "amx_gmm_accumulate_dev: NULL handle");
    AMX_REQUIRE(h->ctx, AMX_ERR_STATE, "amx_gmm_accumulate_dev: host-only handle (created without a context)");
    AMX_REQUIRE(T >= 0 && (best_density_ld == 0 || best_density_ld >= h->n_mix), AMX_ERR_INVALID, "amx_gmm_accumulate_dev: bad shape");
    if (T == 0)
        return AMX_OK;
    AMX_REQUIRE(feats_dev && mixture_dev && best_density_dev && acc_dev, AMX_ERR_INVALID, "amx_gmm_accumulate_dev: NULL buffer");
    AMX_HIP(hipSetDevice(h->ctx->device));
    const AccLayout        l = acc_layout(h);
    const int              pooled = (h->n_cov == 1 && h->dim <= 256) ? 1 : 0;
    const int              blocks = (T + 255) / 256;
    amx::ScopedKernelTimer timer(h->ctx, "gmm_accumulate");
    hipLaunchKernelGGL(amx::gmm_accumulate_kernel, dim3(blocks), dim3(256), 0, h->ctx->stream, feats_dev, mixture_dev, best_density_dev,
                       (const unsigned char*)nullptr, best_density_ld, T, h->dim, h->n_mix, h->d_mix_off.get(), h->d_k_dens.get(), h->d_d_mean.get(), h->d_d_cov.get(), acc_dev,
                       l.off_mw, l.off_ms, l.off_cw, l.off_cs, pooled);
    AMX_HIP(hipGetLastError());
    return AMX_OK;
}

int amx_gmm_accumulate_u8_dev(amx_gmm* h, const float* feats_dev, int T, const uint32_t* mixture_dev, const uint8_t* best_density_dev,
                              int best_density_ld, double* acc_dev) {
    AMX_REQUIRE(h, AMX_ERR_INVALID, "amx_gmm_accumulate_u8_dev: NULL handle");
    AMX_REQUIRE(h->ctx, AMX_ERR_STATE, "amx_gmm_accumulate_u8_dev: host-only handle (created without a context)");
    AMX_REQUIRE(T >= 0 && (best_density_ld == 0 || best_density_ld >= h->n_mix), AMX_ERR_INVALID, "amx_gmm_accumulate_u8_dev: bad shape");
    if (T == 0)
        return AMX_OK;
    AMX_REQUIRE(feats_dev && mixture_dev && best_density_dev && acc_dev, AMX_ERR_INVALID, "amx_gmm_accumulate_u8_dev: NULL buffer");
    AMX_HIP(hipSetDevice(h->ctx->device));
    const AccLayout        l = acc_layout(h);
    const int              pooled = (h->n_cov == 1 && h->dim <= 256) ? 1 : 0;
    const int              blocks = (T + 255) / 256;
    amx::ScopedKernelTimer timer(h->ctx, "gmm_accumulate");
    hipLaunchKernelGGL(amx::gmm_accumulate_kernel, dim3(blocks), dim3(256), 0, h->ctx->stream, feats_dev, mixture_dev, (const uint32_t*)nullptr,
                       (const unsigned char*)best_density_dev, best_density_ld, T, h->dim, h->n_mix, h->d_mix_off.get(), h->d_k_dens.get(), h->d_d_mean.get(), h->d_d_cov.get(),
                       acc_dev, l.off_mw, l.off_ms, l.off_cw, l.off_cs, pooled);
    AMX_HIP(hipGetLastError());
    return AMX_OK;
}

int amx_gmm_accumulate_weighted_dev(amx_gmm* h, int mode, const float* feats_dev, int T, const uint32_t* mixture_dev,
                                    const double* weight_dev, const uint32_t* best_density_dev, int best_density_ld, double* acc_dev) {
    AMX_REQUIRE(h, AMX_ERR_INVALID, "amx_gmm_accumulate_weighted_dev: NULL handle");
    AMX_REQUIRE(h->ctx, AMX_ERR_STATE, "amx_gmm_accumulate_weighted_dev: host-only handle (created without a context)");
    AMX_REQUIRE(mode == AMX_GMM_VITERBI || mode == AMX_GMM_BAUM_WELCH, AMX_ERR_INVALID, "amx_gmm_accumulate_weighted_dev: unknown mode %d", mode);
    AMX_REQUIRE(T >= 0 && (best_density_ld == 0 || best_density_ld >= h->n_mix), AMX_ERR_INVALID, "amx_gmm_accumulate_weighted_dev: bad shape");
    if (T == 0)
        return AMX_OK;
    AMX_REQUIRE(feats_dev && mixture_dev && acc_dev && (mode == AMX_GMM_BAUM_WELCH || best_density_dev), AMX_ERR_INVALID,
                "amx_gmm_accumulate_weighted_dev: NULL buffer");
    if (mode == AMX_GMM_BAUM_WELCH) {
        uint32_t kmax = 0;
        for (int m = 0; m < h->n_mix; ++m)
            kmax = std::max(kmax, h->mix_off[m + 1] - h->mix_off[m]);
        AMX_REQUIRE(kmax <= (uint32_t)amx::kBwMaxDens, AMX_ERR_UNSUPPORTED,
                    "amx_gmm_accumulate_weighted_dev: Baum-Welch statistics support up to %d densities per mixture (model has %u)",
                    amx::kBwMaxDens, kmax);
    }
    AMX_HIP(hipSetDevice(h->ctx->device));
    const AccLayout        l = acc_layout(h);
    const int              pooled = (h->n_cov == 1) ? 1 : 0;
    const int              per_block = 4 * amx::kBwFramesPerWave;
    const int              blocks = (T + per_block - 1) / per_block;
    amx::ScopedKernelTimer timer(h->ctx, "gmm_accumulate_weighted");
    hipLaunchKernelGGL((h->contract_fma ? amx::gmm_accumulate_weighted_kernel<true> : amx::gmm_accumulate_weighted_kernel<false>), dim3(blocks), dim3(256), 0, h->ctx->stream, mode, feats_dev, mixture_dev,
                       weight_dev, best_density_dev, best_density_ld, T, h->dim, h->n_mix, h->d_mix_off.get(), h->d_k_dens.get(), h->d_d_mean.get(), h->d_d_cov.get(),
                       h->d_k_c32.get(), h->d_means.get(), h->d_isr.get(), acc_dev, l.off_mw, l.off_ms, l.off_cw, l.off_cs, pooled);
    AMX_HIP(hipGetLastError());
    return AMX_OK;
}

int amx_gmm_score(amx_gmm* h, int mode, const float* feats_host, int T, float* scores_host, uint32_t* best_host) {
    AMX_REQUIRE(h, AMX_ERR_INVALID, "amx_gmm_score: NULL handle");
    AMX_REQUIRE(h->ctx, AMX_ERR_STATE, "amx_gmm_score: host-only handle (created without a context)");
    AMX_REQUIRE(T >= 0, AMX_ERR_INVALID, "amx_gmm_score: negative frame count");
    if (T == 0)
        return AMX_OK;
    AMX_REQUIRE(feats_host && scores_host, AMX_ERR_INVALID, "amx_gmm_score: NULL buffer");
    AMX_HIP(hipSetDevice(h->ctx->device));
    hipStream_t  st = h->ctx->stream;
    const size_t nf = (size_t)T * h->dim, ns = (size_t)T * h->n_mix;
    if (nf > h->d_host_f.capacity() || ns > h->d_host_s.capacity() || (best_host && ns > h->d_host_b.capacity()))
        h->graphs.clear();
    if (h->d_host_f.reserve(nf) != AMX_OK || h->d_host_s.reserve(ns) != AMX_OK || (best_host && h->d_host_b.reserve(ns) != AMX_OK)) {
        (void)hipGetLastError();
        amx::set_error("amx_gmm_score: out of device memory");
        return AMX_ERR_DEVICE;
    }
    float*    d_f = h->d_host_f.get();
    float*    d_s = h->d_host_s.get();
    uint32_t* d_b = best_host ? h->d_host_b.get() : nullptr;
    if (hipMemcpyAsync(d_f, feats_host, nf * 4, hipMemcpyHostToDevice, st) != hipSuccess) {
        amx::set_error("amx_gmm_score: H2D copy failed");
        return AMX_ERR_DEVICE;
    }
    int r = amx_gmm_score_dev(h, mode, d_f, T, d_s, d_b);
    if (r != AMX_OK)
        return r;
    if (hipMemcpyAsync(scores_host, d_s, ns * 4, hipMemcpyDeviceToHost, st) != hipSuccess ||
        (best_host && hipMemcpyAsync(best_host, d_b, ns * 4, hipMemcpyDeviceToHost, st) != hipSuccess) ||
        hipStreamSynchronize(st) != hipSuccess) {
        amx::set_error("amx_gmm_score: D2H copy / kernel execution failed: %s", hipGetErrorString(hipGetLastError()));
        return AMX_ERR_DEVICE;
    }
    return AMX_OK;
}

}
```

rasr_amd/csrc/gmm_fused.hip:

```cpp
#include "common.hpp"
#include "gmm_internal.hpp"
#include "gmm_device.hpp"

#include <cfloat>
#include <cmath>
#include <cstring>
#include <limits>
#include <type_traits>
#include <vector>

namespace amx {

typedef _Float16 fus_f16x8 __attribute__((ext_vector_type(8)));
typedef float    fus_f32x16 __attribute__((ext_vector_type(16)));
typedef unsigned fus_u32x2 __attribute__((ext_vector_type(2)));

__host__ __device__ constexpr int fused_ld(int dim) {
    return 4 * (((dim + 3) / 4) | 1);
}
constexpr int kFusedABytes = 256 * 128;
constexpr int kFusedAStage = kFusedABytes + 1024;
__host__ __device__ constexpr int fused_mu_stage(int dim) {
    return 256 * fused_ld(dim) * 4;
}
__host__ __device__ constexpr int fused_rec_bytes(int dim) {
    return kFusedAStage + fused_mu_stage(dim);
}

__device__ __forceinline__ void fused_dma16(const void* gsrc, unsigned lds_byte_addr) {
    asm volatile("s_mov_b32 m0, %1\n\ts_nop 0\n\tglobal_load_lds_dwordx4 %0, off" ::"v"(gsrc), "s"(lds_byte_addr) : "memory");
}

#ifdef AMX_LAB
__device__ unsigned long long fused_stamps[16 * 64 * 6];
#define FUSED_STAMP(phase)                                                                                             \
    do {                                                                                                               \
        if (blockIdx.x == 0 && lane == 0 && (r - r_begin) < 64)                                                        \
            fused_stamps[(wave * 64 + (r - r_begin)) * 6 + (phase)] = __builtin_amdgcn_s_memtime();                    \
    } while (0)
#else
#define FUSED_STAMP(phase) \
    do {                   \
    } while (0)
#endif

template<int DIM, int BEST, int NW, bool FMA = false>
__global__ __launch_bounds__(NW * 64) void gmm_fused_kernel(const float* __restrict__ g_feats, const _Float16* __restrict__ g_X,
                                                        const float* __restrict__ g_nx, const float* __restrict__ g_q,
                                                        const char* __restrict__ g_rec, const float* __restrict__ g_isr,
                                                        float* __restrict__ g_scores, uint32_t* __restrict__ g_best, int T, int Tpad,
                                                        int n_mix, int n_tiles, int r_split, float* __restrict__ g_part_min,
                                                        unsigned* __restrict__ g_part_idx, int part_ld,
                                                        unsigned long long* __restrict__ g_survivors, float na_all) {
    extern __shared__ __attribute__((aligned(16))) char lds[];
    constexpr int LD = fused_ld(DIM), REC = fused_rec_bytes(DIM), NP = REC / 1024;
#ifdef FUSED_ISSUE_ALL
    constexpr bool ISSUE4 = false;
#else
    constexpr bool ISSUE4 = true;
#endif
    const int tid = threadIdx.x, lane = tid & 63;
    const int wave = __builtin_amdgcn_readfirstlane(tid >> 6);
    const int tile_t = blockIdx.x / r_split, part = blockIdx.x % r_split;
    const int per = (n_tiles + r_split - 1) / r_split;
    const int r_begin = part * per, r_end = min(n_tiles, r_begin + per);
    if (r_begin >= r_end)
        return;
    const unsigned lds_base = (unsigned)(uintptr_t)lds;
    constexpr int IW = (NW == 12 && ISSUE4) ? 4 : NW;
    auto load_tile = [&](int r, int buf) {
        if (wave >= IW)
            return;
        const char*    src = g_rec + (size_t)r * REC + lane * 16;
        const unsigned dst = lds_base + buf * REC;
        for (int p = wave; p < NP; p += IW)
            fused_dma16(src + p * 1024, (unsigned)__builtin_amdgcn_readfirstlane((int)(dst + p * 1024)));
    };
    load_tile(r_begin, 0);
#ifdef FUSED_PRIO
    if (NW == 12) {
        if ((wave >> 2) == 2)
            __builtin_amdgcn_s_setprio(2);
        else if ((wave >> 2) == 1)
            __builtin_amdgcn_s_setprio(1);
    }
#endif
    const int  frow = lane & 31, fk = lane >> 5;
    const int  t    = tile_t * (NW * 32) + wave * 32 + frow;
    const bool live = t < T;
    const int  tt   = live ? t : T - 1;
    const int  tx   = min(t, Tpad - 1);
    const bool wave_live = tile_t * (NW * 32) + wave * 32 < T;
    float      x[DIM];
#pragma unroll
    for (int i = 0; i < DIM; ++i)
        x[i] = g_feats[(size_t)tt * DIM + i];
    constexpr int KS = (DIM + 2 + 15) / 16;
    static_assert(KS >= 1 && KS <= 4, "screen operand rows hold 64 columns");
    fus_f16x8 bx[KS];
    float     nx, q;
    if (g_X) {
#pragma unroll
        for (int ks = 0; ks < KS; ++ks)
            bx[ks] = *(const fus_f16x8*)(g_X + (size_t)tx * 64 + (ks * 2 + fk) * 8);
        nx = g_nx[tx];
        q  = g_q[tx];
    }
    else {
        float n2 = 0.f, qq = 0.f, r2 = 0.f;
        bool  fits = true;
        _Float16 hv[KS * 16];
#pragma unroll
        for (int i = 0; i < KS * 16; ++i) {
            float v = 0.f;
            if (i < DIM)
                v = live ? x[i] * g_isr[i] : 0.f;
            fits &= fabsf(v) <= 65504.f;
            const _Float16 h = (_Float16)v;
            const float    r = (float)h;
            n2 += r * r;
            r2 += (v - r) * (v - r);
            qq += v * v;
            hv[i] = (i == DIM || i == DIM + 1) ? (_Float16)(live ? 1.f : 0.f) : h;
        }
#pragma unroll
        for (int ks = 0; ks < KS; ++ks)
#pragma unroll
            for (int e = 0; e < 8; ++e)
                bx[ks][e] = fk ? hv[(ks * 2 + 1) * 8 + e] : hv[ks * 16 + e];
        nx = fits ? sqrtf(n2) : __builtin_inff();
        q  = 1.6e-5f * qq + na_all * (sqrtf(r2) * 1.00001f);
    }
    const bool  all = !(nx < __builtin_inff());
    const bool wide_ok = (n_mix & (BEST == 2 ? 7 : 3)) == 0 && ((uintptr_t)g_scores & 15) == 0 &&
                         (!BEST || ((uintptr_t)g_best & (BEST == 2 ? 7 : 15)) == 0);
    const bool counted = wide_ok && wave_live && NW < 16;
    __builtin_amdgcn_s_waitcnt(0);
    float    run_min = 3.402823466e+38f;
    unsigned run_idx = 0xffffffffu;
    unsigned n_surv  = 0;

    for (int r = r_begin; r < r_end; ++r) {
        const int buf = (r - r_begin) & 1;
        if (wave >= IW)
            asm volatile("s_waitcnt lgkmcnt(0)" ::: "memory");
        else if (r == r_begin || !counted)
            asm volatile("s_waitcnt vmcnt(0) lgkmcnt(0)" ::: "memory");
// ... 152 lines not shown
            so[2 * j + 1]      = __uint_as_float(rs.y);
            if (BEST == 1) {
                const unsigned  bj = (bvalid >> j) & 1u ? (bpack >> (4 * j)) & 15u : 0xffffffffu;
                const unsigned  bk = (bvalid >> (4 + j)) & 1u ? (bpack >> (4 * (4 + j))) & 15u : 0xffffffffu;
                const fus_u32x2 rb = __builtin_amdgcn_permlane32_swap(bj, bk, false, false);
                bo[2 * j]          = rb.x;
                bo[2 * j + 1]      = rb.y;
            }
        }
        unsigned b8[2] = {0, 0};
        if (BEST == 2) {
            auto nib2byte = [](unsigned n) {
                const unsigned x = (n | (n << 8)) & 0x00ff00ffu;
                return (x | (x << 4)) & 0x0f0f0f0fu;
            };
            auto bit2byte = [](unsigned v) { return ((v | (v << 7) | (v << 14) | (v << 21)) & 0x01010101u) * 0xffu; };
            const unsigned  wa = nib2byte(bpack & 0xffffu) | ~bit2byte(bvalid & 15u);
            const unsigned  wb = nib2byte(bpack >> 16) | ~bit2byte((bvalid >> 4) & 15u);
            const fus_u32x2 rb = __builtin_amdgcn_permlane32_swap(wa, wb, false, false);
            b8[0]              = __builtin_amdgcn_perm(rb.y, rb.x, 0x05010400u);
            b8[1]              = __builtin_amdgcn_perm(rb.y, rb.x, 0x07030602u);
        }
        const int mb = m0 + fk * 8;
        if (live) {
            float*    gs = g_scores + (size_t)t * n_mix + mb;
            uint32_t* gb = BEST == 1 ? g_best + (size_t)t * n_mix + mb : nullptr;
            unsigned char* gb8 = BEST == 2 ? (unsigned char*)g_best + (size_t)t * n_mix + mb : nullptr;
            if (wide_ok && m0 + 16 <= n_mix) {
                typedef float    nt_f4 __attribute__((ext_vector_type(4)));
                typedef unsigned nt_u4 __attribute__((ext_vector_type(4)));
                amx::nt_store(nt_f4{so[0], so[1], so[2], so[3]}, (nt_f4*)gs);
                amx::nt_store(nt_f4{so[4], so[5], so[6], so[7]}, (nt_f4*)(gs + 4));
                if (BEST == 1) {
                    amx::nt_store(nt_u4{bo[0], bo[1], bo[2], bo[3]}, (nt_u4*)gb);
                    amx::nt_store(nt_u4{bo[4], bo[5], bo[6], bo[7]}, (nt_u4*)(gb + 4));
                }
                if (BEST == 2) {
                    typedef unsigned nt_u2 __attribute__((ext_vector_type(2)));
                    amx::nt_store(nt_u2{b8[0], b8[1]}, (nt_u2*)gb8);
                }
            }
            else {
#pragma unroll
                for (int e = 0; e < 8; ++e)
                    if (mb + e < n_mix) {
                        gs[e] = so[e];
                        if (BEST == 1)
                            gb[e] = bo[e];
                        if (BEST == 2)
                            gb8[e] = (unsigned char)(b8[e >> 2] >> (8 * (e & 3)));
                    }
            }
        }
        FUSED_STAMP(4);
    }
    if (g_survivors) {
        unsigned long long n = live ? n_surv : 0u;
#pragma unroll
        for (int off = 32; off > 0; off >>= 1)
            n += __shfl_xor(n, off, 64);
        if (lane == 0 && n)
            atomicAdd(g_survivors + ((blockIdx.x * NW + wave) & 255), n);
    }
    if (g_part_min) {
        const float    om = __shfl_xor(run_min, 32, 64);
        const unsigned oi = (unsigned)__shfl_xor((int)run_idx, 32, 64);
        if (om < run_min || (om == run_min && oi < run_idx)) {
            run_min = om;
            run_idx = oi;
        }
        if (fk == 0 && live) {
            g_part_min[(size_t)part * part_ld + t] = run_min;
            g_part_idx[(size_t)part * part_ld + t] = run_idx;
        }
    }
}


template<int DIM, bool BEST, int NE>
__global__ __launch_bounds__((4 + NE) * 64) void gmm_fused_spec_kernel(const float* __restrict__ g_feats, const _Float16* __restrict__ g_X,
                                                             const float* __restrict__ g_nx, const float* __restrict__ g_q,
                                                             const char* __restrict__ g_rec, const float* __restrict__ g_isr,
                                                             float* __restrict__ g_scores, uint32_t* __restrict__ g_best, int T, int Tpad,
                                                             int n_mix, int n_tiles, int r_split, float* __restrict__ g_part_min,
                                                             unsigned* __restrict__ g_part_idx, int part_ld,
                                                             unsigned long long* __restrict__ g_survivors) {
    extern __shared__ __attribute__((aligned(16))) char lds[];
    constexpr int LD = fused_ld(DIM), REC = fused_rec_bytes(DIM), A_ST = kFusedAStage, MU_ST = fused_mu_stage(DIM);
    constexpr int NS = 4, G = NE / NS, FPW = NE * 32;
    static_assert(NE % NS == 0, "every screen wave serves the same number of exact waves");
    static_assert(2 * REC == 2 * A_ST + 2 * MU_ST && A_ST % 1024 == 0 && MU_ST % 1024 == 0, "two rings out of two records");
    const int tid = threadIdx.x, lane = tid & 63;
    const int wave = __builtin_amdgcn_readfirstlane(tid >> 6);
    const int tile_t = blockIdx.x / r_split, part = blockIdx.x % r_split;
    const int per = (n_tiles + r_split - 1) / r_split;
    const int r_begin = part * per, r_end = min(n_tiles, r_begin + per);
    if (r_begin >= r_end)
        return;
    const unsigned lds_base = (unsigned)(uintptr_t)lds;
    auto a_slot  = [&](int q) { return lds + (q & 1) * A_ST; };
    auto mu_slot = [&](int q) { return lds + 2 * A_ST + (q & 1) * MU_ST; };
    const int frow = lane & 31, fk = lane >> 5;
    const int t_wg = tile_t * FPW;

    if (wave < NS) {
        auto dma = [&](const char* src, unsigned dst, int n_pieces) {
            for (int p = wave; p < n_pieces; p += NS)
                fused_dma16(src + p * 1024 + lane * 16, (unsigned)__builtin_amdgcn_readfirstlane((int)(dst + p * 1024)));
        };
        auto load_a = [&](int r) {
            if (r < r_end)
                dma(g_rec + (size_t)r * REC, lds_base + (r & 1) * A_ST, A_ST / 1024);
        };
        auto load_mu = [&](int r) {
            if (r < r_end)
                dma(g_rec + (size_t)r * REC + A_ST, lds_base + 2 * A_ST + (r & 1) * MU_ST, MU_ST / 1024);
        };
        load_a(r_begin);
        load_mu(r_begin);
        load_a(r_begin + 1);
        fus_f16x8 bx[G][4];
        float     nx[G], qq[G];
        bool      live[G], all[G];
#pragma unroll
        for (int g = 0; g < G; ++g) {
            const int t  = t_wg + (G * wave + g) * 32 + frow;
            const int tx = min(t, Tpad - 1);
#pragma unroll
            for (int ks = 0; ks < 4; ++ks)
                bx[g][ks] = *(const fus_f16x8*)(g_X + (size_t)tx * 64 + (ks * 2 + fk) * 8);
            nx[g]   = g_nx[tx];
            qq[g]   = g_q[tx];
            live[g] = t < T;
            all[g]  = !(nx[g] < __builtin_inff());
        }
        unsigned M[G][4];
        auto     screen = [&](int r) {
            const char*  stage = a_slot(r);
            const float* s_p   = (const float*)(stage + kFusedABytes);
#pragma unroll
            for (int g = 0; g < G; ++g) {
#pragma unroll
                for (int w = 0; w < 4; ++w)
                    M[g][w] = 0;
#pragma unroll
                for (int i = 0; i < 8; ++i) {
                    const int  rr = i * 32 + frow;
                    fus_f32x16 c;
#pragma unroll
                    for (int e = 0; e < 16; ++e)
                        c[e] = 0.f;
#pragma unroll
                    for (int ks = 0; ks < 4; ++ks) {
                        const fus_f16x8 a = *(const fus_f16x8*)(stage + rr * 128 + (((ks * 2 + fk) ^ ((rr >> 1) & 7)) << 4));
                        c                 = __builtin_amdgcn_mfma_f32_32x32x16_f16(a, bx[g][ks], c, 0, 0, 0);
                    }
                    float mn = min3_first(c[0], c[1], c[2]);
                    mn       = min3_raw(mn, c[3], c[4]);
                    mn       = min3_raw(mn, c[5], c[6]);
                    mn       = min3_raw(mn, c[7], c[8]);
                    mn       = min3_raw(mn, c[9], c[10]);
                    mn       = min3_raw(mn, c[11], c[12]);
                    mn       = min3_raw(mn, c[13], c[14]);
                    mn       = min3_raw(mn, c[15], c[15]);
                    const float p1 = s_p[i * 2 + fk], p2 = s_p[16 + i * 2 + fk];
                    const int   nd = ((const int*)s_p)[32 + i * 2 + fk];
                    const float thr = mn + fmaf(nx[g], p1, fmaf(fabsf(mn), 1.6e-5f, p2 + qq[g])) + 1e-30f;
                    unsigned    bits = 0;
#pragma unroll
                    for (int e = 15; e >= 0; --e)
                        bits = __builtin_amdgcn_alignbit(bits, __float_as_uint(thr - c[e]), 31);
                    const unsigned valid = (1u << nd) - 1u;
                    const unsigned m16   = live[g] ? ((all[g] ? 0xffffu : (~bits & 0xffffu)) & valid) : 0u;
                    M[g][i >> 1] |= m16 << (16 * (i & 1));
                }
            }
        };
        asm volatile("s_waitcnt vmcnt(0) lgkmcnt(0)" ::: "memory");
// ... 193 lines not shown


extern "C" int amx_internal_gmm_fused_supported(int dim, int pooled, int Kp) {
    if (!pooled || Kp != 64)
        return 0;
    switch (dim) {
        case 16: case 24: case 32: case 33: case 39: case 40: return 1;
        default: return 0;
    }
}

extern "C" int amx_internal_gmm_fused_create(int dim, int n_mix, int n_tiles, const void* A2_host, const uint32_t* mix_off,
                                             const uint32_t* k_mean, const double* c64, const float* means, const float* p1, const float* p2,
                                             amx::DevBuf<char>& rec_dev) {
    const int    LD = amx::fused_ld(dim), REC = amx::fused_rec_bytes(dim);
    const size_t total = (size_t)n_tiles * REC;
    std::vector<char> rec(total, 0);
    const char*       A2 = (const char*)A2_host;
    for (int r = 0; r < n_tiles; ++r) {
        char* base = rec.data() + (size_t)r * REC;
        for (int row = 0; row < 256; ++row)
            for (int c = 0; c < 8; ++c)
                memcpy(base + row * 128 + ((c ^ ((row >> 1) & 7)) << 4), A2 + ((size_t)r * 256 + row) * 128 + c * 16, 16);
        float* pp = (float*)(base + amx::kFusedABytes);
        float* mu = (float*)(base + amx::kFusedAStage);
        for (int j = 0; j < 16; ++j) {
            const int m = r * 16 + j;
            int       nd = 0;
            if (m < n_mix) {
                nd = (int)(mix_off[m + 1] - mix_off[m]);
                for (int s = 0; s < nd; ++s) {
                    const uint32_t k   = mix_off[m] + s;
                    float*         dst = mu + (size_t)(j * 16 + s) * LD;
                    memcpy(dst, means + (size_t)k_mean[k] * dim, (size_t)dim * 4);
                    memcpy(dst + LD - 2, &c64[k], 8);
                }
            }
            pp[j]      = p1[m];
            pp[16 + j] = p2[m];
            ((int*)pp)[32 + j] = nd;
        }
    }
    return rec_dev.upload(rec.data(), total);
}

static int fused_waves(int Tpad, int forced) {
    if (forced == 8 || forced == 12 || forced == 16 || forced == 13)
        return forced;
    return Tpad >= 4096 ? 12 : 8;
}
static int fused_frames(int Tpad, int forced) {
    const int w = fused_waves(Tpad, forced);
    return w == 13 ? 256 : w * 32;
}

static int fused_split_raw(int n_cu, int Tpad, int n_tiles, int forced) {
    const int fpw = fused_frames(Tpad, forced);
    const int ntt = (Tpad + fpw - 1) / fpw, cus = std::max(n_cu, 8);
    if (fused_waves(Tpad, forced) != 8) {
        int best = 1;
        double best_eff = 0;
        for (int sp = 1; sp <= std::min(n_tiles, 8); ++sp) {
            const int    wgs = ntt * sp;
            const double eff = (double)wgs / (double)(((wgs + cus - 1) / cus) * cus);
            if (eff > best_eff + 0.02) {
                best_eff = eff;
                best     = sp;
            }
        }
        return best;
    }
    int split = (cus + ntt - 1) / ntt;
    if (ntt * 4 >= 3 * cus)
        split = 1;
    else if (ntt * split > cus && split > 1 && ntt * (split - 1) * 8 >= cus * 7)
        --split;
    return std::max(1, std::min(split, n_tiles));
}

extern "C" int amx_internal_gmm_fused_waves(int Tpad, int forced_waves) {
    return fused_waves(Tpad, forced_waves);
}

extern "C" int amx_internal_gmm_fused_split(int n_cu, int Tpad, int n_tiles, int forced_waves) {
    const int split = fused_split_raw(n_cu, Tpad, n_tiles, forced_waves);
    const int per   = (n_tiles + split - 1) / split;
    return (n_tiles + per - 1) / per;
}

extern "C" int amx_internal_gmm_fused_score(amx_ctx* ctx, int dim, const void* rec_dev, const float* isr_dev, const float* feats,
                                            const void* X, const float* nx, const float* q, int T, int Tpad, int n_mix, int n_tiles,
                                            int split, float* scores, uint32_t* best, float* pmin, unsigned* pidx, int part_ld,
                                            unsigned long long* survivors, int forced_waves, int best_bytes, int contract_fma, float na_all) {
    const int   nw = fused_waves(Tpad, forced_waves), fpw = fused_frames(Tpad, forced_waves), ntt = (Tpad + fpw - 1) / fpw;
    const int   lds = 2 * amx::fused_rec_bytes(dim);
    const char* rec = (const char*)rec_dev;
    hipStream_t st  = ctx->stream;
#define AMX_FUSED_LAUNCH(D, B, W)                                                                                               \
    {                                                                                                                           \
        auto k = contract_fma ? amx::gmm_fused_kernel<D, B, W, true> : amx::gmm_fused_kernel<D, B, W, false>;                   \
        hipFuncSetAttribute((const void*)k, hipFuncAttributeMaxDynamicSharedMemorySize, lds);                                   \
        hipLaunchKernelGGL(k, dim3(ntt * split), dim3(W * 64), lds, st, feats, (const _Float16*)X, nx, q, rec, isr_dev, scores,  \
                           best, T, Tpad, n_mix, n_tiles, split, pmin, pidx, part_ld, survivors, na_all);                  \
    }
#define AMX_FUSED_SPEC(D, B, E)                                                                                                 \
    {                                                                                                                           \
        auto k = amx::gmm_fused_spec_kernel<D, B, E>;                                                                           \
        hipFuncSetAttribute((const void*)k, hipFuncAttributeMaxDynamicSharedMemorySize, lds);                                   \
        hipLaunchKernelGGL(k, dim3(ntt * split), dim3((4 + E) * 64), lds, st, feats, (const _Float16*)X, nx, q, rec, isr_dev, scores,    \
                           best, T, Tpad, n_mix, n_tiles, split, pmin, pidx, part_ld, survivors);                          \
    }
#define AMX_FUSED(D)                                                                                                            \
    case D: {                                                                                                                   \
        if (nw == 13 && best) AMX_FUSED_SPEC(D, true, 8)                                                                        \
        else if (nw == 13) AMX_FUSED_SPEC(D, false, 8)                                                                          \
        else if (best && nw == 16) AMX_FUSED_LAUNCH(D, 1, 16)                                                                   \
        else if (best && nw == 12 && best_bytes == 1) AMX_FUSED_LAUNCH(D, 2, 12)                                                \
        else if (best && best_bytes == 1) AMX_FUSED_LAUNCH(D, 2, 8)                                                             \
        else if (best && nw == 12) AMX_FUSED_LAUNCH(D, 1, 12)                                                                   \
        else if (best) AMX_FUSED_LAUNCH(D, 1, 8)                                                                                \
        else if (nw == 16) AMX_FUSED_LAUNCH(D, 0, 16)                                                                           \
        else if (nw == 12) AMX_FUSED_LAUNCH(D, 0, 12)                                                                           \
        else AMX_FUSED_LAUNCH(D, 0, 8)                                                                                          \
    } break;
    if (nw == 13 && !X) {
        amx::set_error("gmm fused scorer: the specialised-wave kernel (fused_waves=13) reads packed operand rows (fused_pack=0)");
        return AMX_ERR_UNSUPPORTED;
    }
    if (nw == 13 && contract_fma) {
        amx::set_error("gmm fused scorer: the specialised-wave kernel (fused_waves=13) exists for contract=off only");
        return AMX_ERR_UNSUPPORTED;
    }
    if (best && best_bytes == 1 && nw != 8 && nw != 12) {
        amx::set_error("gmm fused scorer: byte-sized best densities exist for the 8- and 12-wave kernels only (fused_waves=%d)", nw);
        return AMX_ERR_UNSUPPORTED;
    }
    switch (dim) {
        AMX_FUSED(16)
        AMX_FUSED(24)
        AMX_FUSED(32)
        AMX_FUSED(33)
        AMX_FUSED(39)
        AMX_FUSED(40)
        default:
            amx::set_error("gmm fused scorer: no kernel for dimension %d", dim);
            return AMX_ERR_UNSUPPORTED;
    }
#undef AMX_FUSED
#undef AMX_FUSED_SPEC
#undef AMX_FUSED_LAUNCH
    AMX_HIP(hipGetLastError());
    return AMX_OK;
}

#ifdef AMX_LAB
extern "C" int amx_lab_fused_stamps(unsigned long long* out ) {
    return hipMemcpyFromSymbol(out, HIP_SYMBOL(amx::fused_stamps), sizeof(amx::fused_stamps)) == hipSuccess ? AMX_OK : AMX_ERR_DEVICE;
}
#endif
```

rasr_amd/csrc/gmm_internal.hpp:

```cpp
#pragma once
#include "common.hpp"

#define AMX_GMM_DIMS(X) X(16) X(24) X(32) X(33) X(39) X(40) X(45) X(48) X(64)

extern "C" {

int  amx_internal_gmm_presel_create(amx_ctx* ctx, int dim, size_t nk, const uint32_t* k_mean_host, const float* smeans_host, const float* d_smeans,
                                    const uint32_t* d_k_mean, int n_clusters, int n_select, int iterations, float backoff, int contract_fma,
                                    void** out);
void amx_internal_gmm_presel_destroy(void* p);
int  amx_internal_gmm_presel_info(const void* p, int* n_clusters, uint32_t* cluster_of, float* cluster_means);
int  amx_internal_gmm_presel_score(void* p, amx_ctx* ctx, const float* feats_dev, int T, float* scores_dev, const uint32_t* d_mix_off,
                                   const uint32_t* d_k_mean, const float* d_k_const, const float* d_smeans, const float* d_isr0, int n_mix);

int   amx_internal_gmm_simd_create(const amx_gmm_model* m, int contract_fma, void** out, float* scaling_out);
void  amx_internal_gmm_simd_destroy(void* p);
float amx_internal_gmm_simd_scaling(const void* p);
int   amx_internal_gmm_simd_score(void* p, amx_ctx* ctx, int variant, const float* feats_dev, int T, float* scores_dev, uint32_t* best_dev);
int   amx_internal_gmm_simd_presel_build(void* p, amx_ctx* ctx, int n_clusters, int n_select, int iterations);
int   amx_internal_gmm_simd_presel_info(const void* p, int* n_clusters, uint32_t* cluster_of, float* cluster_means);
int   amx_internal_gmm_simd_presel_score(void* p, amx_ctx* ctx, const float* feats_dev, int T, float* scores_dev);

int    amx_internal_gmm_tied_create(int K, int n_mix, int mix_pad, const float* ahat_t_host, amx::DevBuf<float>& amin,
                                    amx::DevBuf<unsigned short>& aup);
size_t amx_internal_gmm_tied_workspace(int K, int T, int mix_pad);
int    amx_internal_gmm_tied_score(amx_ctx* ctx, const float* dist_dev, const uint32_t* k_dens_dev, int K, int T, int Tpad, int n_mix, int mix_pad,
                                   const unsigned short* aup, const float* amax, const float* m2lw_t, const float* ahat_t, const double* ln64,
                                   const float* ln32, const float* amin, void* workspace, float* scores, uint32_t* best,
                                   unsigned long long* survivors_dev, int dt_written, int near_written);
float* amx_internal_gmm_tied_dt(void* workspace, int K, int T, int have_positions);
unsigned long long* amx_internal_gmm_tied_near(void* workspace);
int                 amx_internal_gmm_tied_near_init(amx_ctx* ctx, void* workspace);

int amx_internal_gmm_fused_supported(int dim, int pooled, int Kp);
int amx_internal_gmm_fused_create(int dim, int n_mix, int n_tiles, const void* A2_host, const uint32_t* mix_off, const uint32_t* k_mean,
                                  const double* c64, const float* means, const float* p1, const float* p2, amx::DevBuf<char>& rec);
int amx_internal_gmm_fused_split(int n_cu, int Tpad, int n_tiles, int forced_waves);
int amx_internal_gmm_fused_score(amx_ctx* ctx, int dim, const void* rec_dev, const float* isr_dev, const float* feats, const void* X,
                                 const float* nx, const float* q, int T, int Tpad, int n_mix, int n_tiles, int split, float* scores, uint32_t* best,
                                 float* pmin, unsigned* pidx, int part_ld, unsigned long long* survivors, int forced_waves, int best_bytes,
                                 int contract_fma, float na_all);
int amx_internal_gmm_fused_waves(int Tpad, int forced_waves);

struct amx_internal_gmm_view {
    amx_ctx*        ctx;
    int             dim, n_mix, n_dens, n_mean, n_cov;
    const uint32_t *d_mix_off, *d_k_dens, *d_d_mean, *d_d_cov;
    const float*    d_means;
    const float*    h_vars;
};
int amx_internal_gmm_view_get(const amx_gmm* h, amx_internal_gmm_view* out);

int amx_internal_best_state_reduce(amx_ctx* ctx, const float* part_min, const unsigned* part_idx, int n_tiles, int part_ld, int T,
                                   uint32_t* best_state_dev, unsigned long long* counts_dev, double* score_sum_dev);

}
```

rasr_amd/csrc/mfcc.hip:

```cpp
#include "common.hpp"
#include "mfcc_tables.hpp"

#include <algorithm>
#include <cmath>
#include <cstdlib>
#include <cstring>
#include <type_traits>

namespace amx {

struct MfccTile {
    long long sample_base;
    long long out_frame;
    int       n_samples;
    int       frame0;
    int       n_frames;
    int       pad_;
};

struct MfccParams {
    const void*     pcm;
    float*          ceps;
    const MfccTile* tiles;
    const float*    window;
// ... 743 lines not shown
        }
        };
        if (!R16 && p.front_end)
            bank(std::true_type{});
        else
            bank(std::false_type{});
        if (p.eql)
            acc = (float)((double)acc * p.eql[flt]);
        if (f < tile.n_frames)
            s_lm[f * L.lm_ld + flt] = (!R16 && p.front_end) ? power_node(acc, p.plp_power)
                                                            : __log10f(acc);
    }
    MFCC_STAMP(3);
    __syncthreads();
    MFCC_STAMP(4);
    if constexpr (BPT) {
        const int next = tile_id + (int)gridDim.x;
        if (next < p.n_tiles) {
            const int nb = __builtin_amdgcn_readfirstlane(p.tiles[next].pad_);
            if (nb != cur_bank) {
                stage_bank(nb);
                cur_bank = nb;
            }
        }
    }

    {
        const int n_tiles = L.dct_ld / 16;
        const int arow = lane & 15, akq = lane >> 4;
        for (int nt = wave; nt < n_tiles; nt += MW) {
            f32x4 acc = {0.f, 0.f, 0.f, 0.f};
            for (int kk = 0; kk < L.kpad / 4; ++kk) {
                const float a = s_lm[arow * L.lm_ld + 4 * kk + akq];
                const float b = s_dct[(4 * kk + akq) * L.dct_ld + nt * 16 + arow];
                acc           = __builtin_amdgcn_mfma_f32_16x16x4f32(a, b, acc, 0, 0, 0);
            }
            const int cep = nt * 16 + (lane & 15);
#pragma unroll
            for (int r = 0; r < 4; ++r) {
                const int f = (lane >> 4) * 4 + r;
                if (f < tile.n_frames && cep < p.n_ceps) {
                    float v = acc[r];
                    if (p.dct_normalize)
                        v = v / p.norm_div;
                    p.ceps[(tile.out_frame + f) * (long long)p.n_ceps + cep] = v;
                }
            }
        }
    }
    MFCC_STAMP(5);
    __syncthreads();
    MFCC_STAMP(6);
  }
}

__global__ __launch_bounds__(256) void context_window_kernel(const float* __restrict__ feats, const long long* __restrict__ frame_off,
                                                            int n_seg, int dim, int left, int right,
                                                            float* __restrict__ out, int out_stride, long long total) {
    const long long t = blockIdx.x;
    if (t >= total)
        return;
    int lo = 0, hi = n_seg;
    while (hi - lo > 1) {
        int mid = (lo + hi) >> 1;
        if (frame_off[mid] <= t)
            lo = mid;
        else
            hi = mid;
    }
    const long long s0 = frame_off[lo], s1 = frame_off[lo + 1];
    const int       w  = (left + right + 1) * dim;
    for (int i = threadIdx.x; i < out_stride; i += blockDim.x) {
        float v = 0.f;
        if (i < w) {
            int       c  = i / dim, d = i - c * dim;
            long long tt = t - left + c;
            tt           = tt < s0 ? s0 : (tt >= s1 ? s1 - 1 : tt);
            v            = feats[tt * dim + d];
        }
        out[t * (long long)out_stride + i] = v;
    }
}

}


struct amx_mfcc {
    amx_ctx*        ctx = nullptr;
    bool            tune_fft_mfma = false, tune_lpc_lds = false, tune_prefetch = false;
    bool            fft_r16 = false;
    int             tune_wgs = 0;
    amx::MfccTables tab;
    int             frames_per_tile = 16;
    amx::DevBuf<float>  d_window, d_fw, d_dct_t;
    amx::DevBuf<int>    d_fs, d_fe, d_fo;
    amx::DevBuf<float2> d_tw, d_stw;
    amx::DevBuf<double> d_eql;
    size_t              lds_bytes = 0;
    amx::DevBuf<float>  d_ac;
    std::vector<double>          vtln_factors;
    std::vector<amx::MfccTables> banks;
    int                          bank_weights = 0;
    amx::DevBuf<unsigned>        d_banks;
    size_t                       bank_rec = 0, bank_nw = 0;

    int n_weights() const { return banks.empty() ? (int)tab.filter_weights.size() : bank_weights; }
};

struct amx_mfcc_plan {
    amx_mfcc*              owner = nullptr;
    int                    n_seg = 0;
    bool                   vtln  = false;
    int                    uniform_bank = 0;
    std::vector<long>      sample_off, frame_off;
    std::vector<amx::MfccTile> tiles;
    amx::DevBuf<amx::MfccTile> d_tiles;
    amx::DevBuf<long long>     d_frame_off;
};

namespace {

size_t mfcc_lds_bytes(const amx::MfccTables& t, bool r16, int n_weights) {
    amx::MfccLds L(t.frame_len, t.frame_shift, t.fft_len, t.n_inputs, t.n_transform, n_weights, r16);
    return (size_t)L.total * 4;
}

void input_filters(const amx::MfccTables& t, std::vector<int>& in_start, std::vector<int>& in_end, std::vector<int>& in_off) {
    in_start.assign((size_t)t.n_inputs, 0);
    in_end.assign((size_t)t.n_inputs, 0);
    in_off.assign((size_t)t.n_inputs, 0);
    for (int i = 0; i < t.n_inputs; ++i) {
        const int src = t.n_inputs == t.n_filters ? i : std::min(std::max(i - 1, 0), t.n_filters - 1);
        in_start[(size_t)i] = t.filter_start[(size_t)src];
        in_end[(size_t)i]   = t.filter_end[(size_t)src];
        in_off[(size_t)i]   = t.filter_offset[(size_t)src];
    }
}

__host__ __device__ constexpr size_t lpc_lds_bytes(int n_ac) {
    return (size_t)64 * n_ac * (8 + 8 + 4 + 4 + 4);
}
__global__ __launch_bounds__(64) void lpc_cepstrum_kernel(const float* __restrict__ ac, int n_ac, float* __restrict__ out, int n_out,
                                                         long long n_frames) {
    extern __shared__ __attribute__((aligned(16))) char lpc_lds[];
    const int lane  = threadIdx.x;
    double*   prev  = (double*)lpc_lds + lane;
    double*   cur   = prev + (size_t)64 * n_ac;
    float*    R     = (float*)(cur - lane + (size_t)64 * n_ac) + lane;
    float*    a     = R + (size_t)64 * n_ac;
    float*    c     = a + (size_t)64 * n_ac;
    const long long t  = (long long)blockIdx.x * 64 + lane;
    const long long tt = t < n_frames ? t : n_frames - 1;
    for (int i = 0; i < n_ac; ++i)
        R[i * 64] = ac[tt * n_ac + i];
    const int N = n_ac - 1;
    auto almost_zero = [](double e) {
        return fabs(e) < (fabs(e) + 0.0 + 2.2250738585072014e-308) * 2.2204460492503131e-16 * 1.0;
    };
    bool   ok = true;
    double E  = (double)R[0];
    if (almost_zero(E))
        ok = false;
    if (ok) {
        const double k1 = (double)(-R[64] / R[0]);
        prev[64]        = k1;
        E               = (double)R[0] + (double)R[64] * k1;
    }
    for (int i = 2; i <= N; ++i) {
        double k = (double)R[i * 64];
        for (int j = 1; j <= i - 1; ++j)
            k += prev[j * 64] * (double)R[(i - j) * 64];
        if (ok && almost_zero(E))
            ok = false;
        if (ok) {
            k           = -k / E;
            cur[i * 64] = k;
            for (int j = 1; j <= i - 1; ++j)
                cur[j * 64] = prev[j * 64] + k * prev[(i - j) * 64];
            E = (1.0 - k * k) * E;
            for (int j = 1; j <= i; ++j)
                prev[j * 64] = cur[j * 64];
        }
    }
    if (t >= n_frames)
        return;
    float* o = out + t * n_out;
    if (!ok) {
        for (int n = 0; n < n_out; ++n)
            o[n] = __builtin_nanf("");
        return;
    }
    const float gain = (float)sqrt(E);
    for (int j = 1; j <= N; ++j)
        a[(j - 1) * 64] = (float)prev[j * 64];
    c[0]  = (float)(2 * log((double)gain));
// ... 53 lines not shown
                for (int j = 1; j <= i - 1; ++j)
                    cur[j] = prev[j] + k * prev[i - j];
                E = (1.0 - k * k) * E;
#pragma unroll
                for (int j = 1; j <= i; ++j)
                    prev[j] = cur[j];
            }
        }
    }
    if (t >= n_frames)
        return;
    float* o = out + t * n_out;
    if (!ok) {
        for (int n = 0; n < n_out; ++n)
            o[n] = __builtin_nanf("");
        return;
    }
    const float gain = (float)sqrt(E);
    float       a[MAXA], c[MAXA];
#pragma unroll
    for (int j = 1; j < MAXA; ++j)
        a[j - 1] = (float)prev[j];
    a[MAXA - 1] = 0.f;
    c[0] = (float)(2 * log((double)gain));
    c[1] = -a[0];
#pragma unroll
    for (int n = 2; n < MAXA; ++n) {
        c[n] = 0.f;
        if (n < n_out) {
            float v = (float)n * a[n - 1];
#pragma unroll
            for (int k = 1; k < n; ++k) {
                float tt2 = (float)(n - k) * c[n - k];
                tt2       = tt2 * a[k - 1];
                v         = v + tt2;
            }
            c[n] = v / (-(float)n);
        }
    }
#pragma unroll
    for (int n = 0; n < MAXA; ++n)
        if (n < n_out)
            o[n] = c[n];
}

template<int NC, int VAR>
int launch_mfcc_var(amx_mfcc* h, const amx::MfccParams& p, int n_tiles) {
    auto kern = amx::mfcc_kernel<NC, VAR>;
    if (h->lds_bytes > 48 * 1024)
        AMX_HIP(hipFuncSetAttribute((const void*)kern, hipFuncAttributeMaxDynamicSharedMemorySize, (int)h->lds_bytes));
    int per_cu = (int)std::max<size_t>(1, std::min<size_t>((VAR & 16) ? 2 : (VAR & 8) ? 3 : 4, (160 * 1024) / std::max<size_t>(h->lds_bytes, 1)));
    if (h->tune_wgs > 0)
        per_cu = std::max(1, std::min(per_cu, h->tune_wgs));
    int grid   = std::min(n_tiles, per_cu * std::max(h->ctx->n_cu, 1));
    amx::ScopedKernelTimer timer(h->ctx, "mfcc");
    hipLaunchKernelGGL(kern, dim3(grid), dim3(amx::mfcc_waves(NC) * 64), h->lds_bytes, h->ctx->stream, p);
    AMX_HIP(hipGetLastError());
    return AMX_OK;
}

template<int NC, int VAR>
int launch_mfcc_bank(amx_mfcc* h, const amx::MfccParams& p, int n_tiles, bool bpt) {
    return bpt ? launch_mfcc_var<NC, VAR | 32>(h, p, n_tiles) : launch_mfcc_var<NC, VAR>(h, p, n_tiles);
}

template<int NC>
int launch_mfcc(amx_mfcc* h, const amx::MfccParams& p, int n_tiles, bool s16, bool bpt) {
    if (n_tiles <= 0)
        return AMX_OK;
    if constexpr (NC == 256) {
        if (h->fft_r16)
            return s16 ? launch_mfcc_bank<NC, 18>(h, p, n_tiles, bpt) : launch_mfcc_bank<NC, 16>(h, p, n_tiles, bpt);
        if (h->tune_fft_mfma)
            return s16 ? launch_mfcc_bank<NC, 3>(h, p, n_tiles, bpt) : launch_mfcc_bank<NC, 1>(h, p, n_tiles, bpt);
        if (h->tune_prefetch)
            return s16 ? launch_mfcc_bank<NC, 6>(h, p, n_tiles, bpt) : launch_mfcc_bank<NC, 4>(h, p, n_tiles, bpt);
    }
    return s16 ? launch_mfcc_bank<NC, 2>(h, p, n_tiles, bpt) : launch_mfcc_bank<NC, 0>(h, p, n_tiles, bpt);
}

int parse_tuning(amx_mfcc* h, const amx_mfcc_cfg* cfg, bool* fma, bool* r16) {
    amx::Tuning tune;
    {
        static const char* const keys[] = {"fft", "wgs", "lpc", "prefetch", "contract", nullptr};
        if (!tune.parse(cfg->tuning, keys, "amx_mfcc_create"))
            return AMX_ERR_INVALID;
    }
    std::string t_fft, t_lpc, t_contract;
    int         t_wgs, t_prefetch;
    {
        static const char* const ffts[] = {"stockham", "mfma", "r16", nullptr};
        static const char* const lpcs[] = {"regs", "lds", nullptr};
        static const char* const cons[] = {"off", "fma", nullptr};
        const char*              who    = "amx_mfcc_create";
        if (!tune.get_word("fft", "stockham", ffts, &t_fft, who) || !tune.get_word("lpc", "regs", lpcs, &t_lpc, who) ||
            !tune.get_int("wgs", 0, 0, 64, &t_wgs, who) || !tune.get_int("prefetch", 1, 0, 1, &t_prefetch, who) ||
            !tune.get_word("contract", h->ctx && h->ctx->contract == AMX_CONTRACT_FMA ? "fma" : "off", cons, &t_contract, who))
            return AMX_ERR_INVALID;
    }
    h->tune_fft_mfma = t_fft == "mfma";
    h->tune_lpc_lds  = t_lpc == "lds";
    h->tune_wgs      = t_wgs;
    h->tune_prefetch = t_prefetch != 0;
    *fma             = t_contract == "fma";
    *r16             = t_fft == "r16";
    return AMX_OK;
}

int build_banks(amx_mfcc* h, const amx_mfcc_cfg& cfg, const amx_mfcc_vtln* vtln, bool fma) {
    if (!vtln)
        return h->tab.build(cfg, fma);
    h->vtln_factors.assign(vtln->factors, vtln->factors + vtln->n_factors);
    h->banks.resize((size_t)vtln->n_factors);
    for (int i = 0; i < vtln->n_factors; ++i) {
        const amx::MfccTables::Vtln v{vtln->factors[i], vtln->limit};
        AMX_TRY(h->banks[(size_t)i].build(cfg, fma, &v));
        AMX_REQUIRE(h->banks[(size_t)i].n_filters == h->banks[0].n_filters, AMX_ERR_INVALID,
                    "amx_mfcc_create_vtln: warping factor %g gives %d filters, warping factor %g gives %d", vtln->factors[0],
                    h->banks[0].n_filters, vtln->factors[i], h->banks[(size_t)i].n_filters);
        h->bank_weights = std::max(h->bank_weights, (int)h->banks[(size_t)i].filter_weights.size());
    }
    h->tab = h->banks[0];
    return AMX_OK;
}

int check_limits(amx_mfcc* h, const amx_mfcc_cfg& cfg, bool r16) {
    const amx::MfccTables& t = h->tab;
    AMX_REQUIRE(t.fft_len >= 8 && t.fft_len <= 2048, AMX_ERR_UNSUPPORTED,
                "amx_mfcc_create: FFT length %d not supported by the gfx950 kernel (8..2048)", t.fft_len);
    if (!h->ctx)
        return AMX_OK;
    h->frames_per_tile = amx::FT;
    h->fft_r16         = r16 && t.fft_len == 512 && cfg.front_end == AMX_FRONT_END_MFCC;
    h->lds_bytes       = mfcc_lds_bytes(t, h->fft_r16, h->n_weights());
    AMX_REQUIRE(h->lds_bytes <= 160 * 1024, AMX_ERR_UNSUPPORTED,
                "amx_mfcc_create: configuration needs %zu bytes of LDS per workgroup (> 160 KiB)", h->lds_bytes);
    return AMX_OK;
}

std::vector<unsigned> pack_bank_records(amx_mfcc* h) {
    const amx::MfccTables& t = h->tab;
    const amx::MfccLds     L(t.frame_len, t.frame_shift, t.fft_len, t.n_inputs, t.n_transform, h->n_weights(), h->fft_r16);
    const size_t           nw = (size_t)(L.fidx - L.fw), rec = nw + 3 * (size_t)t.n_inputs;
    h->bank_rec = rec, h->bank_nw = nw;
    std::vector<unsigned> recs(rec * h->banks.size(), 0u);
    for (size_t k = 0; k < h->banks.size(); ++k) {
        const amx::MfccTables& b = h->banks[k];
        unsigned*              o = recs.data() + k * rec;
        std::vector<int>       bs, be, bo;
        input_filters(b, bs, be, bo);
        memcpy(o, b.filter_weights.data(), b.filter_weights.size() * 4);
        memcpy(o + nw, bs.data(), bs.size() * 4);
        memcpy(o + nw + bs.size(), be.data(), be.size() * 4);
        memcpy(o + nw + 2 * bs.size(), bo.data(), bo.size() * 4);
    }
    return recs;
}

int upload_tables(amx_mfcc* h) {
    const amx::MfccTables& t = h->tab;
    AMX_HIP(hipSetDevice(h->ctx->device));
    std::vector<float> dct_t((size_t)t.n_inputs * t.n_transform);
    for (int k = 0; k < t.n_transform; ++k)
        for (int n = 0; n < t.n_inputs; ++n)
            dct_t[(size_t)n * t.n_transform + k] = t.dct[(size_t)k * t.n_inputs + n];
    std::vector<int> in_start, in_end, in_off;
    input_filters(t, in_start, in_end, in_off);
    if (!h->banks.empty()) {
        const std::vector<unsigned> recs = pack_bank_records(h);
        AMX_TRY(h->d_banks.upload(recs.data(), recs.size()));
    }
    AMX_TRY(h->d_window.upload(t.window.data(), t.window.size()));
    AMX_TRY(h->d_fw.upload(t.filter_weights.data(), t.filter_weights.size()));
    AMX_TRY(h->d_dct_t.upload(dct_t.data(), dct_t.size()));
    AMX_TRY(h->d_fs.upload(in_start.data(), in_start.size()));
    AMX_TRY(h->d_fe.upload(in_end.data(), in_end.size()));
    AMX_TRY(h->d_fo.upload(in_off.data(), in_off.size()));
    if (!t.eql.empty())
        AMX_TRY(h->d_eql.upload(t.eql.data(), t.eql.size()));
    AMX_TRY(h->d_tw.upload((const float2*)t.twiddle.data(), t.twiddle.size() / 2));
    return h->d_stw.upload((const float2*)t.split_twiddle.data(), t.split_twiddle.size() / 2);
}

int mfcc_create(amx_ctx* ctx, const amx_mfcc_cfg* cfg, const amx_mfcc_vtln* vtln, amx_mfcc** out) {
    AMX_REQUIRE(cfg && out, AMX_ERR_INVALID, "amx_mfcc_create: NULL argument");
    *out = nullptr;
    std::unique_ptr<amx_mfcc> h(new amx_mfcc);
    h->ctx   = ctx;
    bool fma = false, r16 = false;
    AMX_TRY(parse_tuning(h.get(), cfg, &fma, &r16));
    AMX_TRY(build_banks(h.get(), *cfg, vtln, fma));
    AMX_TRY(check_limits(h.get(), *cfg, r16));
    if (ctx)
        AMX_TRY(upload_tables(h.get()));
    *out = h.release();
    return AMX_OK;
}

int mfcc_tables(const amx::MfccTables& t, float* window, int* fs, int* fe, int* fo, float* fw, float* dct) {
    if (window)
        memcpy(window, t.window.data(), t.window.size() * 4);
    if (fs)
        memcpy(fs, t.filter_start.data(), t.filter_start.size() * 4);
    if (fe)
        memcpy(fe, t.filter_end.data(), t.filter_end.size() * 4);
    if (fo)
        memcpy(fo, t.filter_offset.data(), t.filter_offset.size() * 4);
    if (fw)
        memcpy(fw, t.filter_weights.data(), t.filter_weights.size() * 4);
    if (dct)
        memcpy(dct, t.dct.data(), t.dct.size() * 4);
    return AMX_OK;
}

int mfcc_bank_of(const amx_mfcc* h, double factor) {
    if (h->vtln_factors.empty())
        return factor == 1.0 ? 0 : -1;
    for (size_t k = 0; k < h->vtln_factors.size(); ++k)
        if (h->vtln_factors[k] == factor)
            return (int)k;
    return -1;
}

int mfcc_plan_create(amx_mfcc* h, int n_seg, const long* sample_offsets, const std::vector<int>* bank, amx_mfcc_plan** out) {
    AMX_REQUIRE(h && out && n_seg >= 0 && (n_seg == 0 || sample_offsets), AMX_ERR_INVALID, "amx_mfcc_plan_create: bad argument");
    AMX_REQUIRE(h->ctx, AMX_ERR_STATE, "amx_mfcc_plan_create: host-only handle (created without a context)");
    *out = nullptr;
    std::unique_ptr<amx_mfcc_plan> p(new amx_mfcc_plan);
    p->owner = h;
    p->n_seg = n_seg;
    p->vtln  = bank != nullptr;
    p->sample_off.assign(sample_offsets, sample_offsets + n_seg + (n_seg ? 1 : 0));
    if (n_seg == 0)
        p->sample_off.assign(1, 0);
    p->frame_off.assign((size_t)n_seg + 1, 0);
    const int ft = h->frames_per_tile;
    for (int u = 0; u < n_seg; ++u) {
        long len = p->sample_off[u + 1] - p->sample_off[u];
        AMX_REQUIRE(len >= 0 && len <= 0x7fffffffL, AMX_ERR_INVALID, "amx_mfcc_plan_create: segment %d has invalid length %ld", u, len);
        long T              = h->tab.n_frames(len);
        p->frame_off[u + 1] = p->frame_off[u] + T;
        for (long f0 = 0; f0 < T; f0 += ft) {
            amx::MfccTile t;
            t.sample_base = p->sample_off[u];
            t.out_frame   = p->frame_off[u] + f0;
            t.n_samples   = (int)len;
            t.frame0      = (int)f0;
            t.n_frames    = (int)std::min<long>(ft, T - f0);
            t.pad_        = bank ? (*bank)[(size_t)u] : 0;
            if (!p->tiles.empty() && t.pad_ != p->tiles[0].pad_)
                p->uniform_bank = -1;
            else if (p->tiles.empty())
                p->uniform_bank = t.pad_;
            p->tiles.push_back(t);
        }
    }
    hipSetDevice(h->ctx->device);
    AMX_TRY(p->d_tiles.upload(p->tiles.data(), p->tiles.size()));
    const std::vector<long long> fo(p->frame_off.begin(), p->frame_off.end());
    AMX_TRY(p->d_frame_off.upload(fo.data(), fo.size()));
    *out = p.release();
    return AMX_OK;
}

amx::MfccParams mfcc_params(const amx_mfcc* h, const amx_mfcc_plan* p, const void* pcm_dev, float* ceps_dev, bool bpt) {
    const amx::MfccTables& t = h->tab;
    amx::MfccParams        k;
    k.pcm             = pcm_dev;
    k.ceps            = ceps_dev;
    k.tiles           = p->d_tiles.get();
    k.window          = h->d_window.get();
    k.fstart          = h->d_fs.get();
    k.fend            = h->d_fe.get();
    k.foff            = h->d_fo.get();
    k.fweights        = bpt ? (const float*)h->d_banks.get() : h->d_fw.get();
    if (!h->banks.empty() && !bpt) {
        const unsigned* rec = h->d_banks.get() + (size_t)p->uniform_bank * h->bank_rec;
        k.fweights          = (const float*)rec;
        k.fstart            = (const int*)(rec + h->bank_nw);
        k.fend              = k.fstart + t.n_inputs;
        k.foff              = k.fend + t.n_inputs;
    }
    k.dct_t           = h->d_dct_t.get();
    k.tw              = h->d_tw.get();
    k.stw             = h->d_stw.get();
    k.frame_len       = t.frame_len;
    k.frame_shift     = t.frame_shift;
    k.n_filters       = t.n_inputs;
    k.eql             = h->d_eql.get();
    k.n_ceps          = t.n_transform;
    k.n_weights       = h->n_weights();
    k.front_end       = t.cfg.front_end != AMX_FRONT_END_MFCC ? 1 : 0;
    k.norm_div        = t.norm_div;
    k.plp_power       = (float)t.cfg.plp_power;
    k.frames_per_tile = h->frames_per_tile;
    k.alpha           = (float)t.cfg.preemph_alpha;
    k.fft_scale       = t.fft_scale;
    k.n_tiles         = (int)p->tiles.size();
    k.apply_scale     = (t.cfg.apply_scale && t.cfg.sample_rate != 1) ? 1 : 0;
    k.dct_normalize   = t.cfg.dct_normalize;
    return k;
}

int mfcc_run_plan(amx_mfcc* h, const amx_mfcc_plan* p, const void* pcm_dev, bool s16, float* ceps_dev) {
    AMX_REQUIRE(h && p, AMX_ERR_INVALID, "amx_mfcc_run_plan_dev: NULL handle");
    AMX_REQUIRE(p->owner == h, AMX_ERR_STATE, "amx_mfcc_run_plan_dev: plan belongs to another front-end handle");
    if (p->tiles.empty())
        return AMX_OK;
    AMX_REQUIRE(pcm_dev && ceps_dev, AMX_ERR_INVALID, "amx_mfcc_run_plan_dev: NULL buffer");
    AMX_HIP(hipSetDevice(h->ctx->device));
    const amx::MfccTables& t = h->tab;
    const bool      bpt = !h->banks.empty() && p->uniform_bank < 0;
    amx::MfccParams k   = mfcc_params(h, p, pcm_dev, ceps_dev, bpt);
    const long long total_frames = p->frame_off.back();
// ... 197 lines not shown
    memcpy(factors, h->tab.eql.data(), h->tab.eql.size() * sizeof(double));
    return AMX_OK;
}

int amx_mfcc_plan_create(amx_mfcc* h, int n_seg, const long* sample_offsets, amx_mfcc_plan** out) {
    return mfcc_plan_create(h, n_seg, sample_offsets, nullptr, out);
}

int amx_mfcc_plan_create_vtln(amx_mfcc* h, int n_seg, const long* sample_offsets, const double* warping_factor, amx_mfcc_plan** out) {
    AMX_REQUIRE(h && out && n_seg >= 0 && (n_seg == 0 || (sample_offsets && warping_factor)), AMX_ERR_INVALID,
                "amx_mfcc_plan_create_vtln: bad argument");
    *out = nullptr;
    std::vector<int> bank((size_t)n_seg, 0);
    for (int u = 0; u < n_seg; ++u) {
        bank[(size_t)u] = mfcc_bank_of(h, warping_factor[u]);
        AMX_REQUIRE(bank[(size_t)u] >= 0, AMX_ERR_INVALID, "amx_mfcc_plan_create_vtln: segment %d: warping factor %.17g is not one of the handle's",
                    u, warping_factor[u]);
    }
    return mfcc_plan_create(h, n_seg, sample_offsets, &bank, out);
}

void amx_mfcc_plan_destroy(amx_mfcc_plan* p) {
    delete p;
}

long amx_mfcc_plan_total_frames(const amx_mfcc_plan* p) {
    return p ? p->frame_off.back() : 0;
}

int amx_mfcc_plan_frame_offsets(const amx_mfcc_plan* p, long* frame_offsets) {
    AMX_REQUIRE(p && frame_offsets, AMX_ERR_INVALID, "amx_mfcc_plan_frame_offsets: NULL argument");
    std::copy(p->frame_off.begin(), p->frame_off.end(), frame_offsets);
    return AMX_OK;
}

int amx_mfcc_run_plan_dev(amx_mfcc* h, const amx_mfcc_plan* p, const float* pcm_dev, float* ceps_dev) {
    return mfcc_run_plan(h, p, pcm_dev, false, ceps_dev);
}

int amx_mfcc_run_plan_dev_s16(amx_mfcc* h, const amx_mfcc_plan* p, const int16_t* pcm_dev, float* ceps_dev) {
    return mfcc_run_plan(h, p, pcm_dev, true, ceps_dev);
}

int amx_mfcc_run_batch(amx_mfcc* h, int n_seg, const float* const* pcm_host, const long* n_samples, float* const* ceps_host) {
    return mfcc_run_batch(h, n_seg, (const void* const*)pcm_host, false, n_samples, ceps_host);
}

int amx_mfcc_run_batch_s16(amx_mfcc* h, int n_seg, const int16_t* const* pcm_host, const long* n_samples, float* const* ceps_host) {
    return mfcc_run_batch(h, n_seg, (const void* const*)pcm_host, true, n_samples, ceps_host);
}

int amx_mfcc_run(amx_mfcc* h, const float* pcm_host, long n_samples, float* ceps_host) {
    const float* in[1]  = {pcm_host};
    float*       out[1] = {ceps_host};
    long         n[1]   = {n_samples};
    return amx_mfcc_run_batch(h, 1, in, n, out);
}

int amx_mfcc_run_s16(amx_mfcc* h, const int16_t* pcm_host, long n_samples, float* ceps_host) {
    const int16_t* in[1]  = {pcm_host};
    float*         out[1] = {ceps_host};
    long           n[1]   = {n_samples};
    return amx_mfcc_run_batch_s16(h, 1, in, n, out);
}

int amx_internal_plan_view(const amx_mfcc_plan* p, const long long** d_frame_off, int* n_seg, long long* total) {
    AMX_REQUIRE(p && d_frame_off && n_seg && total, AMX_ERR_INVALID, "plan view: NULL argument");
    *d_frame_off = p->d_frame_off.get();
    *n_seg       = p->n_seg;
    *total       = p->frame_off.back();
    return AMX_OK;
}

int amx_context_window_dev(amx_ctx* ctx, const amx_mfcc_plan* p, const float* feats_dev, int dim, int left, int right,
                           float* out_dev, int out_stride) {
    AMX_REQUIRE(ctx && p && feats_dev && out_dev, AMX_ERR_INVALID, "amx_context_window_dev: NULL argument");
    AMX_REQUIRE(dim > 0 && left >= 0 && right >= 0 && out_stride >= (left + right + 1) * dim, AMX_ERR_INVALID,
                "amx_context_window_dev: out_stride %d < window %d", out_stride, (left + right + 1) * dim);
    const long long total = p->frame_off.back();
    if (total == 0)
        return AMX_OK;
    AMX_HIP(hipSetDevice(ctx->device));
    amx::ScopedKernelTimer timer(ctx, "context_window");
    hipLaunchKernelGGL(amx::context_window_kernel, dim3((unsigned)total), dim3(256), 0, ctx->stream, feats_dev,
                       p->d_frame_off.get(), p->n_seg, dim, left, right, out_dev, out_stride, total);
    AMX_HIP(hipGetLastError());
    return AMX_OK;
}

}

#ifdef AMX_LAB
extern "C" int amx_lab_mfcc_r16_stamps(unsigned long long* out ) {
    return hipMemcpyFromSymbol(out, HIP_SYMBOL(amx::mfcc_r16_stamps), sizeof(amx::mfcc_r16_stamps)) == hipSuccess ? AMX_OK : AMX_ERR_DEVICE;
}
extern "C" int amx_lab_mfcc_stamps(unsigned long long* out ) {
    return hipMemcpyFromSymbol(out, HIP_SYMBOL(amx::mfcc_stamps), sizeof(amx::mfcc_stamps)) == hipSuccess ? AMX_OK : AMX_ERR_DEVICE;
}
#endif
```

Measured before the change: 5.031 million.

## Vectorize input packing, context window, stage accumulate feats in LDS, plan fused splits

Several unrelated changes land together. The MX input pack gets a row-major index order with float4 loads. A vectorised context-window kernel handles several frames per wave. The GMM accumulate kernel stages features in LDS and uses a fixed-trip leader scan. A new fused-score plan allows uneven part sizes (per, n_long) instead of an equal split. These mainly target memory coalescing and load balance across CUs, and they add new kernels and tuning keys that could hurt for some shapes.

Result: no change. 5.073 million (median of 6 runs) (+0.8%).

```diff
diff --git a/rasr_amd/csrc/common.hpp b/rasr_amd/csrc/common.hpp
--- a/rasr_amd/csrc/common.hpp
+++ b/rasr_amd/csrc/common.hpp
@@ -198,7 +198,7 @@
 };
 
 static const char* const gmm_tuning_keys[] = {"screen", "fused", "screen_all", "screen_kernel", "graph", "tied_prune", "chunk", "fused_waves", "fr",
-                                              "simd_mfma", "contract", "dist_list", "near_fused", "fused_pack", nullptr};
+                                              "simd_mfma", "contract", "dist_list", "near_fused", "fused_pack", "acc_lds", "fused_plan", nullptr};
 
 template<bool FMA>
 __host__ __device__ __forceinline__ float mad(float a, float b, float c) {
diff --git a/rasr_amd/csrc/ffnn.hip b/rasr_amd/csrc/ffnn.hip
--- a/rasr_amd/csrc/ffnn.hip
+++ b/rasr_amd/csrc/ffnn.hip
@@ -1192,6 +1192,7 @@
     int    gemm_persistent = 1;
     int    gemm_cfg       = -1;
     int    chunk          = 32768;
+    int    mx_pack_rows   = 1;
     int    mx_stagger     = 0;
     int    mx_dbg         = 0;
     int    mx_ksplit      = 1;
@@ -1563,7 +1564,8 @@
     const int   blocks = (int)std::min<long long>(4096, ((long long)Tpad * Kp + 255) / 256);
     if (h->is_mx()) {
         const int b2 = (int)std::min<long long>(8192, ((long long)Tpad * (Kp / 32) * 2 + 255) / 256);
-        hipLaunchKernelGGL(amx::mx::pack_input_mx<S>, dim3(b2), dim3(256), 0, st, src, T, K, (char*)out, Kp / 32, Tpad, h->overflow.dev);
+        hipLaunchKernelGGL(amx::mx::pack_input_mx<S>, dim3(b2), dim3(256), 0, st, src, T, K, (char*)out, Kp / 32, Tpad, h->overflow.dev,
+                           h->mx_pack_rows);
     }
     else if (h->precision == AMX_PREC_BF16X3)
         hipLaunchKernelGGL(amx::pack_input_bf16x3<S>, dim3(blocks), dim3(256), 0, st, src, T, K, (amx::bf16_t*)out, Kp, Tpad);
@@ -1750,7 +1752,7 @@
 }
 
 int parse_tuning(const amx_ffnn_model* m, amx_ffnn* h, bool* mx_fallback_auto) {
-    static const char* const keys[]      = {"tile", "graph", "persistent", "group", "chunk", "stagger", "mx_dbg", "mx_fallback", "ksplit", nullptr};
+    static const char* const keys[]      = {"tile", "graph", "persistent", "group", "chunk", "stagger", "mx_dbg", "mx_fallback", "ksplit", "pack_rows", nullptr};
     static const char* const fallbacks[] = {"auto", "off", nullptr};
     const char*              who         = "amx_ffnn_create";
     amx::Tuning              tune;
@@ -1763,7 +1765,8 @@
     AMX_REQUIRE(h->mx_ksplit == 1 || m->precision == AMX_PREC_F16MX, AMX_ERR_UNSUPPORTED, "amx_ffnn_create: tuning ksplit exists for AMX_PREC_F16MX only");
     if (!tune.get_int("tile", -1, -1, 14, &h->gemm_cfg, who) || !tune.get_int("graph", 0, 0, 1, &h->graphs.use_graphs, who) ||
         !tune.get_int("persistent", 1, 0, 1, &h->gemm_persistent, who) || !tune.get_int("chunk", 32768, 256, 1 << 24, &h->chunk, who) ||
-        !tune.get_int("mx_dbg", 0, 0, 1 << 16, &h->mx_dbg, who) || !tune.get_int("stagger", 0, 0, 100000, &h->mx_stagger, who))
+        !tune.get_int("mx_dbg", 0, 0, 1 << 16, &h->mx_dbg, who) || !tune.get_int("stagger", 0, 0, 100000, &h->mx_stagger, who) ||
+        !tune.get_int("pack_rows", 1, 0, 1, &h->mx_pack_rows, who))
         return AMX_ERR_INVALID;
     if (tune.has("group")) {
         const std::string g    = tune.kv["group"];
diff --git a/rasr_amd/csrc/ffnn_f32.hpp b/rasr_amd/csrc/ffnn_f32.hpp
--- a/rasr_amd/csrc/ffnn_f32.hpp
+++ b/rasr_amd/csrc/ffnn_f32.hpp
@@ -31,6 +31,8 @@
     const float* x;
     int          ldx;
     __device__ __forceinline__ float operator()(int t, int k) const { return x[(size_t)t * ldx + k]; }
+    __device__ __forceinline__ bool   quads() const { return ldx % 4 == 0 && ((uintptr_t)x & 15) == 0; }
+    __device__ __forceinline__ float4 quad(int t, int k) const { return *(const float4*)(x + (size_t)t * ldx + k); }
 };
 
 struct FeatSrc {
@@ -52,6 +54,8 @@
         }
         return v;
     }
+    __device__ __forceinline__ bool   quads() const { return pre.n == 0 && ldx % 4 == 0 && ((uintptr_t)x & 15) == 0; }
+    __device__ __forceinline__ float4 quad(int t, int k) const { return *(const float4*)(x + (size_t)t * ldx + k); }
 };
 
 static __global__ __launch_bounds__(256) void top_negexp_kernel(float* __restrict__ x, int n, float* __restrict__ g_max) {
diff --git a/rasr_amd/csrc/ffnn_mx.hpp b/rasr_amd/csrc/ffnn_mx.hpp
--- a/rasr_amd/csrc/ffnn_mx.hpp
+++ b/rasr_amd/csrc/ffnn_mx.hpp
@@ -134,23 +134,51 @@
     *(uint4*)(blk + r_off(r, hh))     = p.rec;
 }
 
+template<class S, class = void>
+struct has_quads : std::false_type {};
 template<class S>
-__global__ __launch_bounds__(256) void pack_input_mx(S src, int T, int K, char* __restrict__ out, int KT, int Tpad, unsigned* __restrict__ overflow) {
+struct has_quads<S, std::void_t<decltype(std::declval<const S&>().quads())>> : std::true_type {};
+
+template<class S>
+__global__ __launch_bounds__(256) void pack_input_mx(S src, int T, int K, char* __restrict__ out, int KT, int Tpad, unsigned* __restrict__ overflow,
+                                                     int by_rows) {
     const long long n = (long long)Tpad * KT * 2;
     for (long long i = (long long)blockIdx.x * 256 + threadIdx.x; i < n; i += (long long)gridDim.x * 256) {
         const int       hh = (int)(i & 1);
         const long long j  = i >> 1;
-        const int       kt = (int)(j % KT), t = (int)(j / KT);
+        int             kt, t;
+        if (by_rows) {
+            const long long w = j >> 5;
+            kt                = (int)(w % KT);
+            t                 = (int)(w / KT) * 32 + (int)(j & 31);
+        }
+        else {
+            kt = (int)(j % KT);
+            t  = (int)(j / KT);
+        }
         float           a[16], m = 0.f;
-#pragma unroll
-        for (int g = 0; g < 4; ++g)
+        bool            quads = false;
+        if constexpr (has_quads<S>::value)
+            quads = by_rows && src.quads();
+#pragma unroll
+        for (int g = 0; g < 4; ++g) {
+            const int k0 = kt * 32 + 8 * g + 4 * hh;
+            bool      loaded = false;
+            if constexpr (has_quads<S>::value)
+                if (quads && t < T && k0 + 4 <= K) {
+                    const float4 q = src.quad(t, k0);
+                    a[4 * g] = q.x, a[4 * g + 1] = q.y, a[4 * g + 2] = q.z, a[4 * g + 3] = q.w;
+                    loaded = true;
+                }
 #pragma unroll
             for (int e = 0; e < 4; ++e) {
-                const int   k = kt * 32 + 8 * g + 4 * hh + e;
-                const float v = (t < T && k < K) ? src(t, k) : 0.f;
-                a[4 * g + e]  = v;
+                const int k = k0 + e;
+                if (!loaded)
+                    a[4 * g + e] = (t < T && k < K) ? src(t, k) : 0.f;
+                const float v = a[4 * g + e];
                 m             = (v != v) ? __builtin_inff() : fmaxf(m, fabsf(v));
             }
+        }
         m = fmaxf(m, __shfl_xor(m, 1, 64));
         if (!(m < 65520.f))
             *overflow = 1u;
diff --git a/rasr_amd/csrc/gmm.hip b/rasr_amd/csrc/gmm.hip
--- a/rasr_amd/csrc/gmm.hip
+++ b/rasr_amd/csrc/gmm.hip
@@ -255,6 +255,9 @@
         out[i] = (unsigned char)min(in[i], 255u);
 }
 
+constexpr int kAccLdsMaxDim = 60;
+
+template<bool LDS>
 __global__ __launch_bounds__(256) void gmm_accumulate_kernel(const float* __restrict__ feats, const uint32_t* __restrict__ mixture,
                                                             const uint32_t* __restrict__ best, const unsigned char* __restrict__ best8,
                                                             int best_ld, int T, int dim, int n_mix,
@@ -267,6 +270,16 @@
     __shared__ unsigned char s_lead[256];
     const int tid = threadIdx.x, lane = tid & 63, wave = tid >> 6;
     const int t0 = blockIdx.x * 256;
+    extern __shared__ __align__(16) float s_x[];
+    if constexpr (LDS) {
+        const float* src = feats + (size_t)t0 * dim;
+        const int    n   = min(256, T - t0) * dim;
+        const int    n4  = ((uintptr_t)src & 15) == 0 ? n >> 2 : 0;
+        for (int i = tid; i < n4; i += 256)
+            ((float4*)s_x)[i] = ((const float4*)src)[i];
+        for (int i = n4 * 4 + tid; i < n; i += 256)
+            s_x[i] = src[i];
+    }
     {
         const int t = t0 + tid;
         uint32_t  k = 0xffffffffu, mi = 0, ci = 0;
@@ -291,7 +304,22 @@
         s_ci[tid] = ci;
     }
     __syncthreads();
-    {
+    if constexpr (LDS) {
+        const uint32_t k = s_k[tid];
+        bool lead = k != 0xffffffffu;
+        int  next = -1;
+#pragma unroll 16
+        for (int j = 255; j >= 0; --j) {
+            const bool same = s_k[j] == k && k != 0xffffffffu;
+            if (same && j < tid)
+                lead = false;
+            if (same && j > tid)
+                next = j;
+        }
+        s_lead[tid] = lead ? 1 : 0;
+        s_next[tid] = (short)next;
+    }
+    else {
         const uint32_t k = s_k[tid];
         bool lead = k != 0xffffffffu;
         for (int j = 0; j < tid && lead; ++j)
@@ -318,7 +346,7 @@
         for (int m = j; m >= 0; m = s_next[m]) {
             ++count;
             for (int i = lane, c = 0; i < dim && c < 4; i += 64, ++c) {
-                const double y = (double)feats[(size_t)(t0 + m) * dim + i];
+                const double y = (double)(LDS ? s_x[m * dim + i] : feats[(size_t)(t0 + m) * dim + i]);
                 sx[c] += y;
                 sxx[c] += y * y;
             }
@@ -1481,8 +1509,9 @@
     std::vector<float>    h_smeans;
     GraphCache graphs;
     int         tune_screen = 1, tune_fused = 1, tune_screen_all = 0, tune_tied_prune = -1, tune_chunk = 65536, tune_fused_waves = 0, tune_fr = 8,
-                tune_simd_mfma = 1, tune_dist_list = 1, tune_near_fused = 1, tune_fused_pack = 1;
+                tune_simd_mfma = 1, tune_dist_list = 1, tune_near_fused = 1, tune_fused_pack = 1, tune_acc_lds = 1;
     std::string tune_screen_kernel = "rows";
+    std::string tune_fused_plan;
     bool        contract_fma = false;
     amx::DevBuf<char>     d_fus_rec;
     amx::DevBuf<uint32_t> d_best32;
@@ -1546,7 +1575,8 @@
         }
         if (fused) {
             const int n_tiles = h->scr_Rpad / 256;
-            const int split   = amx_internal_gmm_fused_split(h->ctx->n_cu, Tpad, n_tiles, h->tune_fused_waves);
+            int       split = 0, per = 0, n_long = 0;
+            AMX_TRY(amx_internal_gmm_fused_plan(h->ctx->n_cu, Tpad, n_tiles, h->tune_fused_waves, h->tune_fused_plan.c_str(), &split, &per, &n_long));
             float*    pmin    = nullptr;
             unsigned* pidx    = nullptr;
             if (stats) {
@@ -1559,7 +1589,7 @@
             {
                 amx::ScopedKernelTimer timer(h->ctx, "gmm");
                 int r = amx_internal_gmm_fused_score(h->ctx, h->dim, h->d_fus_rec.get(), h->d_isr.get(), x, own_pack ? nullptr : h->d_scr_X.get(), h->d_scr_nx.get(), h->d_scr_q.get(), Tc, Tpad,
-                                                     h->n_mix, n_tiles, split, scores_dev + (size_t)t0 * h->n_mix,
+                                                     h->n_mix, n_tiles, split, per, n_long, scores_dev + (size_t)t0 * h->n_mix,
                                                      best_dev ? (uint32_t*)((char*)best_dev + (size_t)t0 * h->n_mix * best_bytes) : nullptr, pmin,
                                                      pidx, Tpad, h->count_survivors ? h->d_fus_surv.get() : nullptr, h->tune_fused_waves, best_bytes,
                                                      h->contract_fma ? 1 : 0, h->scr_na_all);
@@ -1754,10 +1784,18 @@
         !tune.get_int("fr", 8, 2, 16, &h->tune_fr, who) || !tune.get_int("simd_mfma", 1, 0, 1, &h->tune_simd_mfma, who) ||
         !tune.get_int("graph", 0, 0, 1, &h->graphs.use_graphs, who) || !tune.get_int("dist_list", 1, 0, 64, &h->tune_dist_list, who) ||
         !tune.get_int("near_fused", 1, 0, 1, &h->tune_near_fused, who) || !tune.get_int("fused_pack", 1, 0, 1, &h->tune_fused_pack, who) ||
+        !tune.get_int("acc_lds", 1, 0, 1, &h->tune_acc_lds, who) ||
         !tune.get_word("screen_kernel", "rows", screen_kernels, &h->tune_screen_kernel, who) ||
         !tune.get_word("contract", ctx && ctx->contract == AMX_CONTRACT_FMA ? "fma" : "off", contracts, &contract, who))
         return AMX_ERR_INVALID;
     h->contract_fma = contract == "fma";
+    if (tune.has("fused_plan")) {
+        h->tune_fused_plan = tune.kv["fused_plan"];
+        int  a = 0, b = 0;
+        char tail = 0;
+        AMX_REQUIRE(h->tune_fused_plan == "equal" || (sscanf(h->tune_fused_plan.c_str(), "%dx%d%c", &a, &b, &tail) == 2 && a >= 1 && b >= 1),
+                    AMX_ERR_INVALID, "amx_gmm_create: tuning fused_plan=%s: expected equal | <parts>x<per>, e.g. 4x204", h->tune_fused_plan.c_str());
+    }
     AMX_REQUIRE(h->tune_fused_waves == 0 || h->tune_fused_waves == 8 || h->tune_fused_waves == 12 || h->tune_fused_waves == 13 || h->tune_fused_waves == 16,
                 AMX_ERR_INVALID, "amx_gmm_create: tuning fused_waves=%d: expected 8 | 12 | 13 | 16", h->tune_fused_waves);
     AMX_REQUIRE(h->tune_fr == 2 || h->tune_fr == 4 || h->tune_fr == 8 || h->tune_fr == 16, AMX_ERR_INVALID,
@@ -2681,7 +2719,9 @@
     const int              pooled = (h->n_cov == 1 && h->dim <= 256) ? 1 : 0;
     const int              blocks = (T + 255) / 256;
     amx::ScopedKernelTimer timer(h->ctx, "gmm_accumulate");
-    hipLaunchKernelGGL(amx::gmm_accumulate_kernel, dim3(blocks), dim3(256), 0, h->ctx->stream, feats_dev, mixture_dev, best_density_dev,
+    const bool             lds = h->tune_acc_lds && h->dim <= amx::kAccLdsMaxDim;
+    hipLaunchKernelGGL((lds ? amx::gmm_accumulate_kernel<true> : amx::gmm_accumulate_kernel<false>), dim3(blocks), dim3(256),
+                       lds ? (size_t)256 * h->dim * sizeof(float) : 0, h->ctx->stream, feats_dev, mixture_dev, best_density_dev,
                        (const unsigned char*)nullptr, best_density_ld, T, h->dim, h->n_mix, h->d_mix_off.get(), h->d_k_dens.get(), h->d_d_mean.get(), h->d_d_cov.get(), acc_dev,
                        l.off_mw, l.off_ms, l.off_cw, l.off_cs, pooled);
     AMX_HIP(hipGetLastError());
@@ -2701,7 +2741,9 @@
     const int              pooled = (h->n_cov == 1 && h->dim <= 256) ? 1 : 0;
     const int              blocks = (T + 255) / 256;
     amx::ScopedKernelTimer timer(h->ctx, "gmm_accumulate");
-    hipLaunchKernelGGL(amx::gmm_accumulate_kernel, dim3(blocks), dim3(256), 0, h->ctx->stream, feats_dev, mixture_dev, (const uint32_t*)nullptr,
+    const bool             lds = h->tune_acc_lds && h->dim <= amx::kAccLdsMaxDim;
+    hipLaunchKernelGGL((lds ? amx::gmm_accumulate_kernel<true> : amx::gmm_accumulate_kernel<false>), dim3(blocks), dim3(256),
+                       lds ? (size_t)256 * h->dim * sizeof(float) : 0, h->ctx->stream, feats_dev, mixture_dev, (const uint32_t*)nullptr,
                        (const unsigned char*)best_density_dev, best_density_ld, T, h->dim, h->n_mix, h->d_mix_off.get(), h->d_k_dens.get(), h->d_d_mean.get(), h->d_d_cov.get(),
                        acc_dev, l.off_mw, l.off_ms, l.off_cw, l.off_cs, pooled);
     AMX_HIP(hipGetLastError());
diff --git a/rasr_amd/csrc/gmm_fused.hip b/rasr_amd/csrc/gmm_fused.hip
--- a/rasr_amd/csrc/gmm_fused.hip
+++ b/rasr_amd/csrc/gmm_fused.hip
@@ -5,7 +5,12 @@
 #include <cfloat>
 #include <cmath>
 #include <cstring>
+#include <functional>
 #include <limits>
+#include <map>
+#include <mutex>
+#include <queue>
+#include <tuple>
 #include <type_traits>
 #include <vector>
 
@@ -49,7 +54,7 @@
                                                         const float* __restrict__ g_nx, const float* __restrict__ g_q,
                                                         const char* __restrict__ g_rec, const float* __restrict__ g_isr,
                                                         float* __restrict__ g_scores, uint32_t* __restrict__ g_best, int T, int Tpad,
-                                                        int n_mix, int n_tiles, int r_split, float* __restrict__ g_part_min,
+                                                        int n_mix, int n_tiles, int r_split, int per, int n_long, float* __restrict__ g_part_min,
                                                         unsigned* __restrict__ g_part_idx, int part_ld,
                                                         unsigned long long* __restrict__ g_survivors, float na_all) {
     extern __shared__ __attribute__((aligned(16))) char lds[];
@@ -61,8 +66,9 @@
 #endif
     const int tid = threadIdx.x, lane = tid & 63;
     const int wave = __builtin_amdgcn_readfirstlane(tid >> 6);
-    const int tile_t = blockIdx.x / r_split, part = blockIdx.x % r_split;
-    const int per = (n_tiles + r_split - 1) / r_split;
+    const int n_front = (int)(gridDim.x / r_split) * n_long;
+    const bool front  = n_long == r_split || (int)blockIdx.x < n_front;
+    const int tile_t = front ? blockIdx.x / n_long : blockIdx.x - n_front, part = front ? blockIdx.x % n_long : n_long;
     const int r_begin = part * per, r_end = min(n_tiles, r_begin + per);
     if (r_begin >= r_end)
         return;
@@ -381,7 +387,7 @@
                                                              const float* __restrict__ g_nx, const float* __restrict__ g_q,
                                                              const char* __restrict__ g_rec, const float* __restrict__ g_isr,
                                                              float* __restrict__ g_scores, uint32_t* __restrict__ g_best, int T, int Tpad,
-                                                             int n_mix, int n_tiles, int r_split, float* __restrict__ g_part_min,
+                                                             int n_mix, int n_tiles, int r_split, int per, int n_long, float* __restrict__ g_part_min,
                                                              unsigned* __restrict__ g_part_idx, int part_ld,
                                                              unsigned long long* __restrict__ g_survivors) {
     extern __shared__ __attribute__((aligned(16))) char lds[];
@@ -391,8 +397,9 @@
     static_assert(2 * REC == 2 * A_ST + 2 * MU_ST && A_ST % 1024 == 0 && MU_ST % 1024 == 0, "two rings out of two records");
     const int tid = threadIdx.x, lane = tid & 63;
     const int wave = __builtin_amdgcn_readfirstlane(tid >> 6);
-    const int tile_t = blockIdx.x / r_split, part = blockIdx.x % r_split;
-    const int per = (n_tiles + r_split - 1) / r_split;
+    const int n_front = (int)(gridDim.x / r_split) * n_long;
+    const bool front  = n_long == r_split || (int)blockIdx.x < n_front;
+    const int tile_t = front ? blockIdx.x / n_long : blockIdx.x - n_front, part = front ? blockIdx.x % n_long : n_long;
     const int r_begin = part * per, r_end = min(n_tiles, r_begin + per);
     if (r_begin >= r_end)
         return;
@@ -752,15 +759,135 @@
     return fused_waves(Tpad, forced_waves);
 }
 
-extern "C" int amx_internal_gmm_fused_split(int n_cu, int Tpad, int n_tiles, int forced_waves) {
+constexpr int    kFusedMaxParts   = 8;
+constexpr double kFusedStartTiles = 1.5;
+
+struct FusedPlan {
+    int parts, per, n_long;
+};
+
+static FusedPlan fused_plan_of(int n_tiles, int per, bool numbered_as_equal) {
+    FusedPlan p;
+    p.per    = per;
+    p.parts  = (n_tiles + per - 1) / per;
+    p.n_long = (numbered_as_equal || n_tiles % per == 0) ? p.parts : p.parts - 1;
+    return p;
+}
+
+static double fused_makespan(int n_slots, int ntt, int n_tiles, const FusedPlan& p) {
+    std::priority_queue<double, std::vector<double>, std::greater<double>> free_at;
+    for (int i = 0; i < n_slots; ++i)
+        free_at.push(0.0);
+    double    end  = 0.0;
+    const int last = n_tiles - (p.parts - 1) * p.per;
+    auto      run  = [&](int tiles) {
+        const double t = free_at.top() + kFusedStartTiles + tiles;
+        free_at.pop();
+        free_at.push(t);
+        end = std::max(end, t);
+    };
+    if (p.n_long == p.parts) {
+        for (int t = 0; t < ntt; ++t)
+            for (int q = 0; q < p.parts; ++q)
+                run(q == p.parts - 1 ? last : p.per);
+    }
+    else {
+        for (int i = 0; i < ntt * p.n_long; ++i)
+            run(p.per);
+        for (int t = 0; t < ntt; ++t)
+            run(last);
+    }
+    return end;
+}
+
+static FusedPlan fused_plan_equal(int n_cu, int Tpad, int n_tiles, int forced_waves) {
     const int split = fused_split_raw(n_cu, Tpad, n_tiles, forced_waves);
-    const int per   = (n_tiles + split - 1) / split;
-    return (n_tiles + per - 1) / per;
+    return fused_plan_of(n_tiles, (n_tiles + split - 1) / split, true);
+}
+
+static int fused_plan(int n_cu, int Tpad, int n_tiles, int forced_waves, const char* forced, FusedPlan* out) {
+    const FusedPlan eq = fused_plan_equal(n_cu, Tpad, n_tiles, forced_waves);
+    *out               = eq;
+    if (forced && !strcmp(forced, "equal"))
+        return AMX_OK;
+    if (forced && *forced) {
+        int  parts = 0, per = 0;
+        char tail  = 0;
+        if (sscanf(forced, "%dx%d%c", &parts, &per, &tail) != 2 || parts < 1 || per < 1) {
+            amx::set_error("gmm fused scorer: tuning fused_plan=%s: expected equal | <parts>x<per>, e.g. 4x204", forced);
+            return AMX_ERR_INVALID;
+        }
+        per = std::min(per, n_tiles);
+        const FusedPlan p = fused_plan_of(n_tiles, per, false);
+        if (p.parts != parts) {
+            amx::set_error("gmm fused scorer: tuning fused_plan=%s: %d ranges of %d tiles do not cover %d tiles exactly once", forced, parts,
+                           per, n_tiles);
+            return AMX_ERR_INVALID;
+        }
+        *out = p;
+        return AMX_OK;
+    }
+    const int w = fused_waves(Tpad, forced_waves);
+    if (w != 12 && w != 16)
+        return AMX_OK;
+    struct Key {
+        int  n_cu, ntt, n_tiles;
+        bool operator<(const Key& o) const { return std::tie(n_cu, ntt, n_tiles) < std::tie(o.n_cu, o.ntt, o.n_tiles); }
+    };
+    static std::mutex               mu;
+    static std::map<Key, FusedPlan> known;
+    const int                       fpw = fused_frames(Tpad, forced_waves), ntt = (Tpad + fpw - 1) / fpw, slots = std::max(n_cu, 8);
+    const Key                       key{slots, ntt, n_tiles};
+    std::lock_guard<std::mutex>     lock(mu);
+    auto                            it = known.find(key);
+    if (it == known.end()) {
+        const double m_eq = fused_makespan(slots, ntt, n_tiles, eq);
+        FusedPlan    best = eq;
+        double       m_best = m_eq;
+        for (int per = (n_tiles + kFusedMaxParts - 1) / kFusedMaxParts; per <= n_tiles; ++per) {
+            const FusedPlan p = fused_plan_of(n_tiles, per, false);
+            const double    m = fused_makespan(slots, ntt, n_tiles, p);
+            if (m < m_best) {
+                m_best = m;
+                best   = p;
+            }
+        }
+        const int extra = ntt * (best.parts - eq.parts);
+        if (!(m_eq - m_best > kFusedStartTiles * std::max(0, (extra + slots - 1) / slots)))
+            best = eq;
+        it = known.emplace(key, best).first;
+    }
+    *out = it->second;
+    return AMX_OK;
+}
+
+extern "C" int amx_internal_gmm_fused_plan(int n_cu, int Tpad, int n_tiles, int forced_waves, const char* forced, int* parts, int* per,
+                                           int* n_long) {
+    FusedPlan p;
+    const int r = fused_plan(n_cu, Tpad, n_tiles, forced_waves, forced, &p);
+    if (r != AMX_OK)
+        return r;
+    *parts  = p.parts;
+    *per    = p.per;
+    *n_long = p.n_long;
+    return AMX_OK;
+}
+
+extern "C" double amx_internal_gmm_fused_makespan(int n_cu, int Tpad, int n_tiles, int forced_waves, int per, int n_long) {
+    const int fpw = fused_frames(Tpad, forced_waves), ntt = (Tpad + fpw - 1) / fpw;
+    FusedPlan p   = fused_plan_of(n_tiles, per, false);
+    p.n_long      = n_long;
+    return fused_makespan(std::max(n_cu, 8), ntt, n_tiles, p);
+}
+
+extern "C" int amx_internal_gmm_fused_split(int n_cu, int Tpad, int n_tiles, int forced_waves, const char* forced) {
+    FusedPlan p;
+    return fused_plan(n_cu, Tpad, n_tiles, forced_waves, forced, &p) == AMX_OK ? p.parts : -1;
 }
 
 extern "C" int amx_internal_gmm_fused_score(amx_ctx* ctx, int dim, const void* rec_dev, const float* isr_dev, const float* feats,
                                             const void* X, const float* nx, const float* q, int T, int Tpad, int n_mix, int n_tiles,
-                                            int split, float* scores, uint32_t* best, float* pmin, unsigned* pidx, int part_ld,
+                                            int split, int per, int n_long, float* scores, uint32_t* best, float* pmin, unsigned* pidx, int part_ld,
                                             unsigned long long* survivors, int forced_waves, int best_bytes, int contract_fma, float na_all) {
     const int   nw = fused_waves(Tpad, forced_waves), fpw = fused_frames(Tpad, forced_waves), ntt = (Tpad + fpw - 1) / fpw;
     const int   lds = 2 * amx::fused_rec_bytes(dim);
@@ -771,14 +898,14 @@
         auto k = contract_fma ? amx::gmm_fused_kernel<D, B, W, true> : amx::gmm_fused_kernel<D, B, W, false>;                   \
         hipFuncSetAttribute((const void*)k, hipFuncAttributeMaxDynamicSharedMemorySize, lds);                                   \
         hipLaunchKernelGGL(k, dim3(ntt * split), dim3(W * 64), lds, st, feats, (const _Float16*)X, nx, q, rec, isr_dev, scores,  \
-                           best, T, Tpad, n_mix, n_tiles, split, pmin, pidx, part_ld, survivors, na_all);                  \
+                           best, T, Tpad, n_mix, n_tiles, split, per, n_long, pmin, pidx, part_ld, survivors, na_all);                  \
     }
 #define AMX_FUSED_SPEC(D, B, E)                                                                                                 \
     {                                                                                                                           \
         auto k = amx::gmm_fused_spec_kernel<D, B, E>;                                                                           \
         hipFuncSetAttribute((const void*)k, hipFuncAttributeMaxDynamicSharedMemorySize, lds);                                   \
         hipLaunchKernelGGL(k, dim3(ntt * split), dim3((4 + E) * 64), lds, st, feats, (const _Float16*)X, nx, q, rec, isr_dev, scores,    \
-                           best, T, Tpad, n_mix, n_tiles, split, pmin, pidx, part_ld, survivors);                          \
+                           best, T, Tpad, n_mix, n_tiles, split, per, n_long, pmin, pidx, part_ld, survivors);                          \
     }
 #define AMX_FUSED(D)                                                                                                            \
     case D: {                                                                                                                   \
diff --git a/rasr_amd/csrc/gmm_internal.hpp b/rasr_amd/csrc/gmm_internal.hpp
--- a/rasr_amd/csrc/gmm_internal.hpp
+++ b/rasr_amd/csrc/gmm_internal.hpp
@@ -35,9 +35,11 @@
 int amx_internal_gmm_fused_supported(int dim, int pooled, int Kp);
 int amx_internal_gmm_fused_create(int dim, int n_mix, int n_tiles, const void* A2_host, const uint32_t* mix_off, const uint32_t* k_mean,
                                   const double* c64, const float* means, const float* p1, const float* p2, amx::DevBuf<char>& rec);
-int amx_internal_gmm_fused_split(int n_cu, int Tpad, int n_tiles, int forced_waves);
+int    amx_internal_gmm_fused_plan(int n_cu, int Tpad, int n_tiles, int forced_waves, const char* forced, int* parts, int* per, int* n_long);
+double amx_internal_gmm_fused_makespan(int n_cu, int Tpad, int n_tiles, int forced_waves, int per, int n_long);
+int    amx_internal_gmm_fused_split(int n_cu, int Tpad, int n_tiles, int forced_waves, const char* forced);
 int amx_internal_gmm_fused_score(amx_ctx* ctx, int dim, const void* rec_dev, const float* isr_dev, const float* feats, const void* X,
-                                 const float* nx, const float* q, int T, int Tpad, int n_mix, int n_tiles, int split, float* scores, uint32_t* best,
+                                 const float* nx, const float* q, int T, int Tpad, int n_mix, int n_tiles, int split, int per, int n_long, float* scores, uint32_t* best,
                                  float* pmin, unsigned* pidx, int part_ld, unsigned long long* survivors, int forced_waves, int best_bytes,
                                  int contract_fma, float na_all);
 int amx_internal_gmm_fused_waves(int Tpad, int forced_waves);
diff --git a/rasr_amd/csrc/mfcc.hip b/rasr_amd/csrc/mfcc.hip
--- a/rasr_amd/csrc/mfcc.hip
+++ b/rasr_amd/csrc/mfcc.hip
@@ -849,6 +849,54 @@
     }
 }
 
+constexpr int kWinFramesPerWave = 4;
+
+__global__ __launch_bounds__(256) void context_window_vec_kernel(const float4* __restrict__ feats, const long long* __restrict__ frame_off,
+                                                                int n_seg, int dim4, int left, int right, float4* __restrict__ out,
+                                                                int stride4, long long total) {
+    const int lane = threadIdx.x & 63;
+    long long t    = ((long long)blockIdx.x * 4 + __builtin_amdgcn_readfirstlane(threadIdx.x >> 6)) * kWinFramesPerWave;
+    if (t >= total)
+        return;
+    const long long t_end = t + kWinFramesPerWave < total ? t + kWinFramesPerWave : total;
+    int             lo = 0, hi = n_seg;
+    while (hi - lo > 1) {
+        int mid = (lo + hi) >> 1;
+        if (frame_off[mid] <= t)
+            lo = mid;
+        else
+            hi = mid;
+    }
+    long long s0 = frame_off[lo], s1 = frame_off[lo + 1];
+    const int w4 = (left + right + 1) * dim4;
+    const int c0 = lane / dim4, d0 = lane - c0 * dim4;
+    const int cstep = 64 / dim4, dstep = 64 - cstep * dim4;
+    for (; t < t_end; ++t) {
+        while (t >= s1) {
+            ++lo;
+            s0 = s1;
+            s1 = frame_off[lo + 1];
+        }
+        float4* o = out + t * (long long)stride4;
+        int     c = c0, d = d0;
+        for (int q = lane; q < stride4; q += 64) {
+            float4 v = make_float4(0.f, 0.f, 0.f, 0.f);
+            if (q < w4) {
+                long long tt = t - left + c;
+                tt           = tt < s0 ? s0 : (tt >= s1 ? s1 - 1 : tt);
+                v            = feats[tt * dim4 + d];
+            }
+            o[q] = v;
+            c += cstep;
+            d += dstep;
+            if (d >= dim4) {
+                d -= dim4;
+                ++c;
+            }
+        }
+    }
+}
+
 }
 
 
@@ -857,6 +905,7 @@
     bool            tune_fft_mfma = false, tune_lpc_lds = false, tune_prefetch = false;
     bool            fft_r16 = false;
     int             tune_wgs = 0;
+    int             tune_win_vec = 1;
     amx::MfccTables tab;
     int             frames_per_tile = 16;
     amx::DevBuf<float>  d_window, d_fw, d_dct_t;
@@ -878,6 +927,7 @@
     amx_mfcc*              owner = nullptr;
     int                    n_seg = 0;
     bool                   vtln  = false;
+    bool                   win_vec = true;
     int                    uniform_bank = 0;
     std::vector<long>      sample_off, frame_off;
     std::vector<amx::MfccTile> tiles;
@@ -1097,12 +1147,12 @@
 int parse_tuning(amx_mfcc* h, const amx_mfcc_cfg* cfg, bool* fma, bool* r16) {
     amx::Tuning tune;
     {
-        static const char* const keys[] = {"fft", "wgs", "lpc", "prefetch", "contract", nullptr};
+        static const char* const keys[] = {"fft", "wgs", "lpc", "prefetch", "contract", "win_vec", nullptr};
         if (!tune.parse(cfg->tuning, keys, "amx_mfcc_create"))
             return AMX_ERR_INVALID;
     }
     std::string t_fft, t_lpc, t_contract;
-    int         t_wgs, t_prefetch;
+    int         t_wgs, t_prefetch, t_win_vec;
     {
         static const char* const ffts[] = {"stockham", "mfma", "r16", nullptr};
         static const char* const lpcs[] = {"regs", "lds", nullptr};
@@ -1110,12 +1160,14 @@
         const char*              who    = "amx_mfcc_create";
         if (!tune.get_word("fft", "stockham", ffts, &t_fft, who) || !tune.get_word("lpc", "regs", lpcs, &t_lpc, who) ||
             !tune.get_int("wgs", 0, 0, 64, &t_wgs, who) || !tune.get_int("prefetch", 1, 0, 1, &t_prefetch, who) ||
+            !tune.get_int("win_vec", 1, 0, 1, &t_win_vec, who) ||
             !tune.get_word("contract", h->ctx && h->ctx->contract == AMX_CONTRACT_FMA ? "fma" : "off", cons, &t_contract, who))
             return AMX_ERR_INVALID;
     }
     h->tune_fft_mfma = t_fft == "mfma";
     h->tune_lpc_lds  = t_lpc == "lds";
     h->tune_wgs      = t_wgs;
+    h->tune_win_vec  = t_win_vec;
     h->tune_prefetch = t_prefetch != 0;
     *fma             = t_contract == "fma";
     *r16             = t_fft == "r16";
@@ -1245,6 +1297,7 @@
     p->owner = h;
     p->n_seg = n_seg;
     p->vtln  = bank != nullptr;
+    p->win_vec = h->tune_win_vec != 0;
     p->sample_off.assign(sample_offsets, sample_offsets + n_seg + (n_seg ? 1 : 0));
     if (n_seg == 0)
         p->sample_off.assign(1, 0);
@@ -1608,8 +1661,16 @@
         return AMX_OK;
     AMX_HIP(hipSetDevice(ctx->device));
     amx::ScopedKernelTimer timer(ctx, "context_window");
-    hipLaunchKernelGGL(amx::context_window_kernel, dim3((unsigned)total), dim3(256), 0, ctx->stream, feats_dev,
-                       p->d_frame_off.get(), p->n_seg, dim, left, right, out_dev, out_stride, total);
+    const bool vec = p->win_vec && dim % 4 == 0 && out_stride % 4 == 0 &&
+                     ((uintptr_t)feats_dev | (uintptr_t)out_dev) % 16 == 0;
+    if (vec) {
+        const long long per_wg = 4 * amx::kWinFramesPerWave;
+        hipLaunchKernelGGL(amx::context_window_vec_kernel, dim3((unsigned)((total + per_wg - 1) / per_wg)), dim3(256), 0, ctx->stream,
+                           (const float4*)feats_dev, p->d_frame_off.get(), p->n_seg, dim / 4, left, right, (float4*)out_dev, out_stride / 4, total);
+    }
+    else
+        hipLaunchKernelGGL(amx::context_window_kernel, dim3((unsigned)total), dim3(256), 0, ctx->stream, feats_dev,
+                           p->d_frame_off.get(), p->n_seg, dim, left, right, out_dev, out_stride, total);
     AMX_HIP(hipGetLastError());
     return AMX_OK;
 }
```
